# ethz-asl/voxgraph

Hardware: AMD Instinct MI355X
Metric: Mresiduals+Jacobians/s per GPU; full pose-graph solve ms (200 submaps) (higher is better)
Workload: dtype f32

## Files before the change

voxgraph_amd/csrc/vgx_context.hip:

```cpp
#include <algorithm>
#include <atomic>
#include <cmath>
#include <cstring>
#include <numeric>

#include <cstdlib>

#include "vgx_internal.h"

namespace vgx {

static std::mutex g_err_mu;
static std::string g_global_error = "no error";

void set_global_error(const std::string& msg) {
  std::lock_guard<std::mutex> lk(g_err_mu);
  g_global_error = msg;
}

int set_error(vgx_ctx ctx, int code, const std::string& msg) {
  if (ctx) {
    std::lock_guard<std::mutex> lk(ctx->err_mu);
    ctx->last_error = msg;
  } else {
// ... 29 lines not shown
    float v = __builtin_nanf("");
    if (slot >= 0) {
      int vx = ox ? 0 : cx, vy = oy ? 0 : cy, vz = oz ? 0 : cz;
      size_t at = (size_t)slot * VOX + vx + VPS * (vy + VPS * vz);
      bool ok = weight ? (weight[at] > 0.0f) : (observed[at] != 0);
      if (ok) v = distance[at];
    }
    out[cell] = v;
  }
}

int launch_brickify(vgx_submap sm, int which) {
  vgx_ctx ctx = sm->ctx;
  const float* dist = which == 0 ? sm->d_tsdf_distance : sm->d_esdf_distance;
  const float* w = which == 0 ? sm->d_tsdf_weight.get() : nullptr;
  const uint8_t* obs = which == 0 ? nullptr : sm->d_esdf_observed.get();
  const int layout = ctx->brick_layout;
  const size_t cells = brick_cells(sm->vps, layout);
  if ((unsigned long long)sm->n_blocks * cells >= (1ull << 32))
    return set_error(ctx, VGX_ERR_UNSUPPORTED,
                     "submap too large for 32-bit brick addressing: " + std::to_string(sm->n_blocks) + " blocks x " +
                         std::to_string(cells) + " cells per brick");
  size_t bytes = (size_t)sm->n_blocks * cells * sizeof(float);
  VGX_HIP(ctx, sm->grid[which].d_bricks.alloc(bytes));
  sm->grid[which].layout = layout;
  int3 mn = make_int3(sm->lut_min[0], sm->lut_min[1], sm->lut_min[2]);
  int3 dm = make_int3(sm->lut_dim[0], sm->lut_dim[1], sm->lut_dim[2]);
  dispatch_brick(sm->vps, layout, [&](auto V, auto L) {
    hipLaunchKernelGGL((brickify_kernel<V(), L()>), dim3(sm->n_blocks), dim3(256), 0, ctx->stream, sm->d_block_index, sm->d_lut, mn, dm,
                       dist, w, obs, sm->grid[which].d_bricks);
  });
  VGX_HIP(ctx, hipGetLastError());
  sm->grid[which].present = true;
  return VGX_OK;
}

template <int VPS>
__global__ __launch_bounds__(256) void requad_kernel(const float* __restrict__ apron, float* __restrict__ quad) {
  constexpr int CA = BrickLayout<VPS, 0>::cells, CQ = BrickLayout<VPS, 1>::cells, B = VPS + 1;
  const float* in = apron + (size_t)blockIdx.x * CA;
  float* out = quad + (size_t)blockIdx.x * CQ;
  for (int i = threadIdx.x; i < CQ; i += blockDim.x) {
    int cx, cy, cz;
    BrickLayout<VPS, 1>::decode(i, cx, cy, cz);
    out[i] = in[cx + B * (cy + B * cz)];
  }
}

__global__ __launch_bounds__(64) void chunk_bounds_kernel(const float4* __restrict__ xyzd, long long n,
                                                         float4* __restrict__ bounds,
                                                         float* __restrict__ chunk_minmax) {
  const long long first = (long long)blockIdx.x * kChunkPoints;
  float mn[3] = {INFINITY, INFINITY, INFINITY}, mx[3] = {-INFINITY, -INFINITY, -INFINITY};
  for (long long i = first + threadIdx.x; i < first + kChunkPoints && i < n; i += 64) {
    float4 p = xyzd[i];
    mn[0] = fminf(mn[0], p.x); mx[0] = fmaxf(mx[0], p.x);
    mn[1] = fminf(mn[1], p.y); mx[1] = fmaxf(mx[1], p.y);
    mn[2] = fminf(mn[2], p.z); mx[2] = fmaxf(mx[2], p.z);
  }
#pragma unroll
  for (int a = 0; a < 3; ++a)
#pragma unroll
    for (int off = 32; off >= 1; off >>= 1) {
      mn[a] = fminf(mn[a], __shfl_xor(mn[a], off, 64));
      mx[a] = fmaxf(mx[a], __shfl_xor(mx[a], off, 64));
    }
  if (threadIdx.x == 0) {
    float hx = 0.5f * (mx[0] - mn[0]), hy = 0.5f * (mx[1] - mn[1]), hz = 0.5f * (mx[2] - mn[2]);
    float r = sqrtf(hx * hx + hy * hy + hz * hz) * 1.0001f + 1e-4f;
    bounds[blockIdx.x] = make_float4(0.5f * (mx[0] + mn[0]), 0.5f * (mx[1] + mn[1]),
                                     0.5f * (mx[2] + mn[2]), r);
#pragma unroll
    for (int a = 0; a < 3; ++a) {
      chunk_minmax[6 * blockIdx.x + a] = mn[a];
      chunk_minmax[6 * blockIdx.x + 3 + a] = mx[a];
    }
  }
}

int build_chunk_bounds(vgx_ctx ctx, PointSet& ps) {
  ps.d_chunk_bounds.release();
  if (ps.n <= 0) return VGX_OK;
  const long long chunks = (ps.n + kChunkPoints - 1) / kChunkPoints;
  VGX_HIP(ctx, ps.d_chunk_bounds.alloc_n((size_t)chunks));
  DeviceBuffer s_minmax;
  VGX_HIP(ctx, s_minmax.alloc((size_t)chunks * 6 * sizeof(float)));
  float* d_minmax = s_minmax.as<float>();
  hipLaunchKernelGGL(chunk_bounds_kernel, dim3((unsigned)chunks), dim3(64), 0, ctx->stream, ps.d_xyzd,
                     (long long)ps.n, ps.d_chunk_bounds, d_minmax);
  std::vector<float> mm((size_t)chunks * 6);
  hipError_t e = hipGetLastError();
  if (e == hipSuccess) e = hipMemcpyAsync(mm.data(), d_minmax, mm.size() * sizeof(float), hipMemcpyDeviceToHost, ctx->stream);
  if (e == hipSuccess) e = hipStreamSynchronize(ctx->stream);
  if (e != hipSuccess) return set_error(ctx, VGX_ERR_HIP, std::string("chunk bounds: ") + hipGetErrorString(e));
  for (int a = 0; a < 3; ++a) {
    ps.aabb_min[a] = mm[(size_t)a];
    ps.aabb_max[a] = mm[3 + (size_t)a];
  }
  for (long long c = 1; c < chunks; ++c)
    for (int a = 0; a < 3; ++a) {
      ps.aabb_min[a] = std::min(ps.aabb_min[a], mm[(size_t)c * 6 + a]);
      ps.aabb_max[a] = std::max(ps.aabb_max[a], mm[(size_t)c * 6 + 3 + a]);
    }
  return VGX_OK;
}

int build_block_lut(vgx_submap sm) {
  vgx_ctx ctx = sm->ctx;
  const int n_blocks = sm->n_blocks;
  const int32_t* block_index = sm->block_index.data();
  int32_t mn[3] = {0, 0, 0}, mx[3] = {-1, -1, -1};
  for (int b = 0; b < n_blocks; ++b)
    for (int a = 0; a < 3; ++a) {
      int32_t v = block_index[3 * b + a];
      if (b == 0 || v < mn[a]) mn[a] = v;
      if (b == 0 || v > mx[a]) mx[a] = v;
    }
  size_t total = 1;
  for (int a = 0; a < 3; ++a) {
    sm->lut_min[a] = mn[a];
    sm->lut_dim[a] = mx[a] - mn[a] + 1;
    total *= (size_t)sm->lut_dim[a];
    if (total > ((size_t)1 << 28))
      return set_error(ctx, VGX_ERR_UNSUPPORTED,
                       "submap block AABB exceeds 2^28 cells (dense lookup table)");
  }
  if (n_blocks == 0) return VGX_OK;
  std::vector<int32_t> lut(total, -1);
  for (int b = 0; b < n_blocks; ++b) {
    size_t ix = (size_t)(block_index[3 * b + 0] - mn[0]);
    size_t iy = (size_t)(block_index[3 * b + 1] - mn[1]);
    size_t iz = (size_t)(block_index[3 * b + 2] - mn[2]);
    lut[ix + (size_t)sm->lut_dim[0] * (iy + (size_t)sm->lut_dim[1] * iz)] = b;
  }
  VGX_HIP(ctx, sm->d_lut.alloc_n(total));
  VGX_HIP(ctx, hipMemcpy(sm->d_lut, lut.data(), total * sizeof(int32_t), hipMemcpyHostToDevice));
  return VGX_OK;
}

}

namespace vgx {
void reset_point_set(PointSet& ps) {
  static std::atomic<uint64_t> next_version{1};
  ps = PointSet();
  ps.version = next_version.fetch_add(1);
}

int engine_to_host(vgx_ctx ctx, SamplerEngine& e) {
  if (!e.on_device) return VGX_OK;
  VGX_HIP(ctx, hipStreamSynchronize(ctx->stream));
  VGX_HIP(ctx, hipMemcpy(&e.host, e.d_state, sizeof(Mt19937), hipMemcpyDeviceToHost));
  e.on_device = false;
  return VGX_OK;
}

int engine_to_device(vgx_ctx ctx, SamplerEngine& e) {
  if (e.on_device) return VGX_OK;
  if (!e.d_state) VGX_HIP(ctx, e.d_state.alloc(sizeof(Mt19937)));
  VGX_HIP(ctx, hipMemcpyAsync(e.d_state, &e.host, sizeof(Mt19937), hipMemcpyHostToDevice, ctx->stream));
  e.on_device = true;
  return VGX_OK;
}
}

using namespace vgx;

int vgx_submap_s::ensure_quad_grid(int which) {
  Grid& g = grid[which];
  if (!g.present || !g.d_bricks || g.layout != VGX_BRICKS_APRON || g.d_quad) return VGX_OK;
  const size_t cells = brick_cells(vps, VGX_BRICKS_QUAD);
  if ((unsigned long long)n_blocks * cells >= (1ull << 32))
    return set_error(ctx, VGX_ERR_UNSUPPORTED, "submap too large for 32-bit addressing of its quad bricks: " +
                                                   std::to_string(n_blocks) + " blocks");
  static const long fail_after = getenv("VGX_TEST_QUAD_ALLOC_FAILS_AFTER") ? atol(getenv("VGX_TEST_QUAD_ALLOC_FAILS_AFTER")) : -1;
  static long made_so_far = 0;
  const bool pretend_oom = fail_after >= 0 && made_so_far++ >= fail_after;
  if (pretend_oom || g.d_quad.alloc_n((size_t)n_blocks * cells) != hipSuccess) {
    (void)hipGetLastError();
    return set_error(ctx, VGX_ERR_NOMEM, "quad bricks for a sampling session: device allocation failed (" +
                                             std::to_string((size_t)n_blocks * cells * sizeof(float)) + " bytes; "
                                             "vgx_ctx_set_sampling_bricks(ctx, VGX_SAMPLING_BRICKS_SAME) does without)");
  }
  if (vps == 16)
    hipLaunchKernelGGL(requad_kernel<16>, dim3(n_blocks), dim3(256), 0, ctx->stream, g.d_bricks, g.d_quad);
  else
    hipLaunchKernelGGL(requad_kernel<8>, dim3(n_blocks), dim3(256), 0, ctx->stream, g.d_bricks, g.d_quad);
  VGX_HIP(ctx, hipGetLastError());
  return VGX_OK;
}

vgx::GridDev vgx_submap_s::grid_dev(int which) const {
  GridDev g;
  g.bricks = grid[which].d_bricks;
  g.layout = grid[which].layout;
  g.lut = d_lut;
  for (int a = 0; a < 3; ++a) {
    g.lut_min[a] = lut_min[a];
    g.lut_dim[a] = lut_dim[a];
  }
  g.voxel_size = voxel_size;
  g.voxel_size_inv = voxel_size_inv;
  g.block_size = block_size;
  g.block_size_inv = block_size_inv;
  return g;
}

namespace vgx {
std::mutex& lifetime_mu() {
  static std::mutex mu;
  return mu;
}
}

extern "C" {

int vgx_ctx_create(int device, vgx_ctx* out) {
  if (!out) return set_error(nullptr, VGX_ERR_INVALID, "vgx_ctx_create: out == NULL");
  *out = nullptr;
  int count = 0;
  hipError_t e = hipGetDeviceCount(&count);
  if (e != hipSuccess || count <= 0)
    return set_error(nullptr, VGX_ERR_NO_DEVICE,
                     std::string("vgx_ctx_create: no HIP device (") +
                         (e != hipSuccess ? hipGetErrorString(e) : "count == 0") +
                         "); libvoxgraph_amd has no CPU fallback");
  if (device < 0 || device >= count)
    return set_error(nullptr, VGX_ERR_INVALID, "vgx_ctx_create: device index out of range");
  hipDeviceProp_t prop;
  if (hipGetDeviceProperties(&prop, device) != hipSuccess)
    return set_error(nullptr, VGX_ERR_HIP, "vgx_ctx_create: hipGetDeviceProperties failed");
  if (std::string(prop.gcnArchName).rfind("gfx950", 0) != 0)
    return set_error(nullptr, VGX_ERR_NO_DEVICE,
                     std::string("vgx_ctx_create: device is ") + prop.gcnArchName +
                         ", this library is built for gfx950 only");
  vgx_ctx ctx = new (std::nothrow) vgx_ctx_s();
  if (!ctx) return set_error(nullptr, VGX_ERR_NOMEM, "vgx_ctx_create: out of host memory");
  ctx->device = device;
  ctx->cu_count = prop.multiProcessorCount;
  int prio_least = 0, prio_greatest = 0;
  const bool use_prio = hipSetDevice(device) == hipSuccess &&
                        hipDeviceGetStreamPriorityRange(&prio_least, &prio_greatest) == hipSuccess;
  ctx->stream_priorities = use_prio && prio_least != prio_greatest;
  if (hipSetDevice(device) != hipSuccess ||
      hipStreamCreateWithPriority(&ctx->own_stream, hipStreamNonBlocking, ctx->stream_priorities ? prio_least : 0) != hipSuccess ||
      hipStreamCreateWithPriority(&ctx->tsdf_own_stream, hipStreamNonBlocking, ctx->stream_priorities ? prio_greatest : 0) != hipSuccess ||
      hipEventCreate(&ctx->ev_start) != hipSuccess ||
      hipEventCreate(&ctx->ev_stop) != hipSuccess ||
      hipEventCreate(&ctx->ev_tsdf_start) != hipSuccess ||
      hipEventCreate(&ctx->ev_tsdf_stop) != hipSuccess ||
      hipEventCreateWithFlags(&ctx->ev_handover, hipEventDisableTiming) != hipSuccess) {
    if (ctx->own_stream) (void)hipStreamDestroy(ctx->own_stream);
    if (ctx->tsdf_own_stream) (void)hipStreamDestroy(ctx->tsdf_own_stream);
    for (hipEvent_t ev : {ctx->ev_start, ctx->ev_stop, ctx->ev_tsdf_start, ctx->ev_tsdf_stop, ctx->ev_handover})
      if (ev) (void)hipEventDestroy(ev);
    delete ctx;
    return set_error(nullptr, VGX_ERR_HIP, "vgx_ctx_create: stream/event creation failed");
  }
  ctx->stream = ctx->own_stream;
  ctx->tsdf_stream = ctx->tsdf_own_stream;
  ctx->last_error = "no error";
  *out = ctx;
  return VGX_OK;
}

int vgx_ctx_destroy(vgx_ctx ctx) {
  if (!ctx) return VGX_ERR_INVALID;
  (void)hipSetDevice(ctx->device);
  (void)hipStreamSynchronize(ctx->stream);
  (void)hipStreamSynchronize(ctx->tsdf_stream);
  for (hipEvent_t ev : {ctx->ev_start, ctx->ev_stop, ctx->ev_tsdf_start, ctx->ev_tsdf_stop, ctx->ev_handover})
    if (ev) (void)hipEventDestroy(ev);
  for (int k = 0; k < Context::kEvalSlots; ++k) {
    Context::EvalSlot& sl = ctx->eval_slot[k];
    if (sl.stream) {
      (void)hipStreamSynchronize(sl.stream);
      (void)hipStreamDestroy(sl.stream);
    }
    if (sl.order) (void)hipEventDestroy(sl.order);
    sl.d_out.release();
    sl.d_raw.release();
    sl.h_raw.release();
    sl.h_out.release();
  }
  if (ctx->own_stream) (void)hipStreamDestroy(ctx->own_stream);
  if (ctx->tsdf_own_stream) (void)hipStreamDestroy(ctx->tsdf_own_stream);
  delete ctx;
  return VGX_OK;
}

const char* vgx_last_error(vgx_ctx ctx) {
  static thread_local std::string copy;
  if (ctx) {
    std::lock_guard<std::mutex> lk(ctx->err_mu);
    copy = ctx->last_error;
  } else {
    std::lock_guard<std::mutex> lk(g_err_mu);
    copy = g_global_error;
  }
  return copy.c_str();
}

int vgx_ctx_set_stream(vgx_ctx ctx, void* hip_stream) {
  if (!ctx) return VGX_ERR_INVALID;
  std::lock_guard<std::mutex> lk(ctx->mu);
  ctx->stream = hip_stream ? (hipStream_t)hip_stream : ctx->own_stream;
  return VGX_OK;
}

void* vgx_ctx_get_stream(vgx_ctx ctx) { return ctx ? (void*)ctx->stream : nullptr; }

int vgx_ctx_set_tsdf_stream(vgx_ctx ctx, void* hip_stream) {
  if (!ctx) return VGX_ERR_INVALID;
  std::lock_guard<std::mutex> lk(ctx->tsdf_mu);
  (void)hipSetDevice(ctx->device);
  (void)hipStreamSynchronize(ctx->tsdf_stream);
  ctx->tsdf_stream = hip_stream ? (hipStream_t)hip_stream : ctx->tsdf_own_stream;
  return VGX_OK;
}

void* vgx_ctx_get_tsdf_stream(vgx_ctx ctx) { return ctx ? (void*)ctx->tsdf_stream : nullptr; }

int vgx_ctx_set_brick_layout(vgx_ctx ctx, int32_t layout) {
  if (!ctx) return VGX_ERR_INVALID;
  if (layout != VGX_BRICKS_APRON && layout != VGX_BRICKS_QUAD)
    return set_error(ctx, VGX_ERR_INVALID, "vgx_ctx_set_brick_layout: unknown layout");
  std::lock_guard<std::mutex> lk(ctx->mu);
  ctx->brick_layout = layout;
  return VGX_OK;
}

int vgx_ctx_set_sampling_bricks(vgx_ctx ctx, int32_t mode) {
  if (!ctx) return VGX_ERR_INVALID;
  if (mode != VGX_SAMPLING_BRICKS_SAME && mode != VGX_SAMPLING_BRICKS_QUAD)
    return set_error(ctx, VGX_ERR_INVALID, "vgx_ctx_set_sampling_bricks: unknown mode");
  std::lock_guard<std::mutex> lk(ctx->mu);
  ctx->sampling_bricks = mode;
  return VGX_OK;
}

int vgx_ctx_synchronize(vgx_ctx ctx) {
  if (!ctx) return VGX_ERR_INVALID;
  VGX_HIP(ctx, hipStreamSynchronize(ctx->stream));
  VGX_HIP(ctx, hipStreamSynchronize(ctx->tsdf_stream));
  return VGX_OK;
}

int vgx_ctx_synchronize_tsdf(vgx_ctx ctx) {
  if (!ctx) return VGX_ERR_INVALID;
  hipStream_t st;
  {
    std::lock_guard<std::mutex> lk(ctx->tsdf_mu);
    st = ctx->tsdf_stream;
  }
  VGX_HIP(ctx, hipStreamSynchronize(st));
  return VGX_OK;
}

int vgx_ctx_tsdf_wait_for_stream(vgx_ctx ctx, void* producer_stream) {
  if (!ctx) return VGX_ERR_INVALID;
  hipStream_t producer = (hipStream_t)producer_stream;
  if (!producer) {
    std::lock_guard<std::mutex> lk(ctx->mu);
    producer = ctx->stream;
  }
  std::lock_guard<std::mutex> lk(ctx->tsdf_mu);
  VGX_HIP(ctx, hipSetDevice(ctx->device));
  hipEvent_t ev = nullptr;
  VGX_HIP(ctx, hipEventCreateWithFlags(&ev, hipEventDisableTiming));
  hipError_t e = hipEventRecord(ev, producer);
  if (e == hipSuccess) e = hipStreamWaitEvent(ctx->tsdf_stream, ev, 0);
  (void)hipEventDestroy(ev);
  VGX_HIP(ctx, e);
  return VGX_OK;
}

int vgx_ctx_stream_priorities(vgx_ctx ctx) { return ctx && ctx->stream_priorities ? 1 : 0; }

int vgx_ctx_timer_start(vgx_ctx ctx) {
  if (!ctx) return VGX_ERR_INVALID;
  VGX_HIP(ctx, hipEventRecord(ctx->ev_start, ctx->stream));
  {
    std::lock_guard<std::mutex> lk(ctx->tsdf_mu);
    VGX_HIP(ctx, hipEventRecord(ctx->ev_tsdf_start, ctx->tsdf_stream));
  }
  return VGX_OK;
}

int vgx_ctx_timer_stop(vgx_ctx ctx, float* elapsed_ms) {
  if (!ctx || !elapsed_ms) return VGX_ERR_INVALID;
  VGX_HIP(ctx, hipEventRecord(ctx->ev_stop, ctx->stream));
  {
    std::lock_guard<std::mutex> lk(ctx->tsdf_mu);
    VGX_HIP(ctx, hipEventRecord(ctx->ev_tsdf_stop, ctx->tsdf_stream));
  }
  VGX_HIP(ctx, hipEventSynchronize(ctx->ev_stop));
  VGX_HIP(ctx, hipEventSynchronize(ctx->ev_tsdf_stop));
  float a = 0.0f, b = 0.0f;
  VGX_HIP(ctx, hipEventElapsedTime(&a, ctx->ev_start, ctx->ev_stop));
  VGX_HIP(ctx, hipEventElapsedTime(&b, ctx->ev_tsdf_start, ctx->ev_tsdf_stop));
  *elapsed_ms = a > b ? a : b;
  return VGX_OK;
}

static int upload(vgx_ctx ctx, const void* src, size_t bytes, DeviceBuffer& dst) {
  if (!src || bytes == 0) return VGX_OK;
  VGX_HIP(ctx, dst.alloc(bytes));
  VGX_HIP(ctx, hipMemcpyAsync(dst.p, src, bytes, hipMemcpyHostToDevice, ctx->stream));
  return VGX_OK;
}

int vgx_submap_create(vgx_ctx ctx, int32_t submap_id, float voxel_size, int32_t vps,
                      int32_t n_blocks, const int32_t* block_index, const float* tsdf_distance,
                      const float* tsdf_weight, const float* esdf_distance,
                      const uint8_t* esdf_observed, vgx_submap* out) {
  if (!ctx || !out) return VGX_ERR_INVALID;
  *out = nullptr;
  std::lock_guard<std::mutex> lk(ctx->mu);
  if (!(voxel_size > 0) || n_blocks < 0 || (n_blocks > 0 && !block_index))
    return set_error(ctx, VGX_ERR_INVALID, "vgx_submap_create: bad voxel_size / n_blocks / block_index");
  if (vps != 16 && vps != 8)
    return set_error(ctx, VGX_ERR_UNSUPPORTED, "vgx_submap_create: voxels_per_side must be 8 or 16");
  if ((tsdf_distance == nullptr) != (tsdf_weight == nullptr) ||
      (esdf_observed != nullptr && esdf_distance == nullptr))
    return set_error(ctx, VGX_ERR_INVALID,
                     "vgx_submap_create: tsdf_distance/tsdf_weight come together; esdf_observed needs esdf_distance");
  VGX_HIP(ctx, hipSetDevice(ctx->device));
  vgx_submap sm = new (std::nothrow) vgx_submap_s();
  if (!sm) return set_error(ctx, VGX_ERR_NOMEM, "vgx_submap_create: out of host memory");
  sm->ctx = ctx;
  sm->id = submap_id;
  sm->vps = vps;
  sm->n_blocks = n_blocks;
  sm->voxel_size = voxel_size;
  sm->voxel_size_inv = 1.0f / voxel_size;
  sm->block_size = (float)vps * voxel_size;
  sm->block_size_inv = 1.0f / sm->block_size;
  sm->block_index.assign(block_index, block_index + 3 * (size_t)n_blocks);

  int rc = build_block_lut(sm);
  if (rc == VGX_OK && n_blocks > 0) {
    const size_t nvox = (size_t)n_blocks * vps * vps * vps;
    rc = upload(ctx, block_index, 3 * (size_t)n_blocks * sizeof(int32_t), sm->d_block_index);
    if (rc == VGX_OK) rc = upload(ctx, tsdf_distance, nvox * sizeof(float), sm->d_tsdf_distance);
    if (rc == VGX_OK) rc = upload(ctx, tsdf_weight, nvox * sizeof(float), sm->d_tsdf_weight);
    if (rc == VGX_OK) rc = upload(ctx, esdf_distance, nvox * sizeof(float), sm->d_esdf_distance);
    if (rc == VGX_OK) rc = upload(ctx, esdf_observed, nvox * sizeof(uint8_t), sm->d_esdf_observed);
    if (rc == VGX_OK && hipStreamSynchronize(ctx->stream) != hipSuccess)
      rc = set_error(ctx, VGX_ERR_HIP, "vgx_submap_create: H2D upload failed");
    if (rc == VGX_OK && sm->d_tsdf_distance) rc = launch_brickify(sm, 0);
    if (rc == VGX_OK && sm->d_esdf_distance && sm->d_esdf_observed) rc = launch_brickify(sm, 1);
  }
  if (rc != VGX_OK) {
    vgx_submap_destroy(sm);
    return rc;
  }
  *out = sm;
  return VGX_OK;
}


int vgx_submap_release_raw_layers(vgx_submap sm) {
  if (!sm) return VGX_ERR_INVALID;
  (void)hipStreamSynchronize(sm->ctx->stream);
  sm->d_tsdf_distance.release();
  sm->d_tsdf_weight.release();
  sm->d_esdf_distance.release();
  sm->d_esdf_observed.release();
  sm->d_tsdf_rgba.release();
  return VGX_OK;
}

int vgx_submap_set_colors(vgx_submap sm, const uint8_t* rgba) {
  if (!sm) return VGX_ERR_INVALID;
  vgx_ctx ctx = sm->ctx;
  if (!rgba) return set_error(ctx, VGX_ERR_INVALID, "vgx_submap_set_colors: NULL rgba");
  std::lock_guard<std::mutex> lk(ctx->mu);
  if (sm->n_blocks > 0 && (!sm->d_tsdf_distance || !sm->d_tsdf_weight))
    return set_error(ctx, VGX_ERR_INVALID, "vgx_submap_set_colors: raw TSDF layer not resident (released?)");
  VGX_HIP(ctx, hipSetDevice(ctx->device));
  const size_t bytes = std::max<size_t>((size_t)sm->n_blocks * sm->vps * sm->vps * sm->vps * 4, 4);
  DeviceArray<uint32_t> fresh;
  hipError_t e = fresh.alloc(bytes);
  if (e != hipSuccess) return vgx::alloc_error(ctx, e, "vgx_submap_set_colors: allocating colours");
  if (sm->n_blocks > 0) e = hipMemcpyAsync(fresh, rgba, bytes, hipMemcpyHostToDevice, ctx->stream);
  if (e == hipSuccess) e = hipStreamSynchronize(ctx->stream);
  VGX_HIP(ctx, e);
  sm->d_tsdf_rgba.swap(fresh);
  return VGX_OK;
}

int vgx_submap_has_colors(vgx_submap sm, int32_t* has) {
  if (!sm || !has) return VGX_ERR_INVALID;
  std::lock_guard<std::mutex> lk(sm->ctx->mu);
  *has = sm->d_tsdf_rgba ? 1 : 0;
  return VGX_OK;
}

int vgx_submap_download_colors(vgx_submap sm, uint8_t* rgba) {
  if (!sm) return VGX_ERR_INVALID;
  vgx_ctx ctx = sm->ctx;
  if (!rgba) return set_error(ctx, VGX_ERR_INVALID, "vgx_submap_download_colors: NULL rgba");
  std::lock_guard<std::mutex> lk(ctx->mu);
  if (!sm->d_tsdf_rgba) return set_error(ctx, VGX_ERR_INVALID, "vgx_submap_download_colors: the submap has no colours");
  VGX_HIP(ctx, hipSetDevice(ctx->device));
  VGX_HIP(ctx, hipStreamSynchronize(ctx->stream));
  const size_t bytes = (size_t)sm->n_blocks * sm->vps * sm->vps * sm->vps * 4;
  if (bytes) VGX_HIP(ctx, hipMemcpy(rgba, sm->d_tsdf_rgba, bytes, hipMemcpyDeviceToHost));
  return VGX_OK;
}

int vgx_submap_download_layers(vgx_submap sm, float* tsdf_distance, float* tsdf_weight,
                               float* esdf_distance, uint8_t* esdf_observed) {
  if (!sm) return VGX_ERR_INVALID;
  vgx_ctx ctx = sm->ctx;
  VGX_HIP(ctx, hipSetDevice(ctx->device));
  VGX_HIP(ctx, hipStreamSynchronize(ctx->stream));
  const size_t nvox = (size_t)sm->n_blocks * sm->vps * sm->vps * sm->vps;
  struct { void* dst; const void* src; size_t bytes; } jobs[4] = {
      {tsdf_distance, sm->d_tsdf_distance, nvox * sizeof(float)},
      {tsdf_weight, sm->d_tsdf_weight, nvox * sizeof(float)},
      {esdf_distance, sm->d_esdf_distance, nvox * sizeof(float)},
      {esdf_observed, sm->d_esdf_observed, nvox * sizeof(uint8_t)}};
  for (auto& j : jobs) {
    if (!j.dst) continue;
    if (!j.src) return set_error(ctx, VGX_ERR_INVALID, "vgx_submap_download_layers: layer not resident");
    if (j.bytes) VGX_HIP(ctx, hipMemcpy(j.dst, j.src, j.bytes, hipMemcpyDeviceToHost));
  }
  return VGX_OK;
}

int vgx_submap_block_index(vgx_submap sm, int32_t* block_index) {
  if (!sm || !block_index) return VGX_ERR_INVALID;
  std::copy(sm->block_index.begin(), sm->block_index.end(), block_index);
  return VGX_OK;
}

int vgx_submap_destroy(vgx_submap sm) {
  if (!sm) return VGX_ERR_INVALID;
  {
    std::lock_guard<std::mutex> lk(vgx::lifetime_mu());
    if (sm->users > 0) {
      sm->destroy_requested = true;
      return VGX_OK;
    }
  }
  (void)hipSetDevice(sm->ctx->device);
  (void)hipStreamSynchronize(sm->ctx->stream);
  delete sm;
  return VGX_OK;
}

int32_t vgx_submap_id(vgx_submap sm) { return sm ? sm->id : -1; }
int32_t vgx_submap_num_blocks(vgx_submap sm) { return sm ? sm->n_blocks : -1; }

static inline uint64_t spread3(uint64_t v) {
  v &= 0x1fffff;
  v = (v | v << 32) & 0x1f00000000ffffULL;
  v = (v | v << 16) & 0x1f0000ff0000ffULL;
  v = (v | v << 8) & 0x100f00f00f00f00fULL;
  v = (v | v << 4) & 0x10c30c30c30c30c3ULL;
  v = (v | v << 2) & 0x1249249249249249ULL;
  return v;
}

int vgx_submap_set_points(vgx_submap sm, int32_t point_type, int64_t n, const float* xyz,
                          const float* distance, const float* weight, uint32_t flags) {
  if (!sm) return VGX_ERR_INVALID;
  vgx_ctx ctx = sm->ctx;
  std::lock_guard<std::mutex> lk(ctx->mu);
  if (point_type != VGX_POINTS_ISOSURFACE && point_type != VGX_POINTS_VOXELS)
    return set_error(ctx, VGX_ERR_INVALID, "vgx_submap_set_points: bad point_type");
  if (n < 0 || n > INT32_MAX || (n > 0 && (!xyz || !distance || !weight)))
    return set_error(ctx, VGX_ERR_INVALID, "vgx_submap_set_points: bad n or NULL arrays");
  VGX_HIP(ctx, hipSetDevice(ctx->device));
  PointSet& ps = sm->points[point_type];
  (void)hipStreamSynchronize(ctx->stream);
  reset_point_set(ps);
  ps.n = n;
  ps.cumulative_weight.resize((size_t)n);
  double acc = 0;
  for (int64_t i = 0; i < n; ++i) {
    acc = (i == 0) ? (double)weight[i] : acc + (double)weight[i];
    ps.cumulative_weight[(size_t)i] = acc;
  }
  std::vector<int64_t> order;
  if ((flags & VGX_POINTS_SORT_MORTON) && n > 1) {
    std::vector<uint64_t> key((size_t)n);
    float mnv[3] = {xyz[0], xyz[1], xyz[2]};
    for (int64_t i = 0; i < n; ++i)
      for (int a = 0; a < 3; ++a) mnv[a] = std::min(mnv[a], xyz[3 * i + a]);
    float base[3];
    for (int a = 0; a < 3; ++a) base[a] = std::floor(mnv[a] * sm->block_size_inv) * sm->block_size;
    for (int64_t i = 0; i < n; ++i) {
      uint64_t c[3];
      for (int a = 0; a < 3; ++a) {
        double v = std::floor(((double)xyz[3 * i + a] - (double)base[a]) * (double)sm->voxel_size_inv);
        c[a] = (uint64_t)std::min(std::max(v, 0.0), 2097151.0);
      }
      key[(size_t)i] = spread3(c[0]) | (spread3(c[1]) << 1) | (spread3(c[2]) << 2);
    }
    order.resize((size_t)n);
    std::iota(order.begin(), order.end(), (int64_t)0);
    std::stable_sort(order.begin(), order.end(),
                     [&](int64_t a, int64_t b) { return key[(size_t)a] < key[(size_t)b]; });
  }
  std::vector<float4> h_xyzd((size_t)n);
  std::vector<float> h_w((size_t)n);
  double sum_w = 0;
  for (int64_t i = 0; i < n; ++i) {
    int64_t s = order.empty() ? i : order[(size_t)i];
    h_xyzd[(size_t)i] = make_float4(xyz[3 * s], xyz[3 * s + 1], xyz[3 * s + 2], distance[s]);
    h_w[(size_t)i] = weight[s];
    sum_w += (double)weight[s];
  }
  ps.sum_weight = sum_w;
  ps.order = order;
  if (!order.empty()) {
    ps.inv_order.resize((size_t)n);
    for (int64_t i = 0; i < n; ++i) ps.inv_order[(size_t)order[(size_t)i]] = (int32_t)i;
  }
  if (n > 0) {
    VGX_HIP(ctx, ps.d_xyzd.alloc_n((size_t)n));
    VGX_HIP(ctx, ps.d_weight.alloc_n((size_t)n));
    VGX_HIP(ctx, hipMemcpy(ps.d_xyzd, h_xyzd.data(), (size_t)n * sizeof(float4), hipMemcpyHostToDevice));
    VGX_HIP(ctx, hipMemcpy(ps.d_weight, h_w.data(), (size_t)n * sizeof(float), hipMemcpyHostToDevice));
  }
  const int rc = build_chunk_bounds(ctx, ps);
  ps.present = rc == VGX_OK;
  return rc;
}

int64_t vgx_submap_num_points(vgx_submap sm, int32_t point_type) {
  if (!sm || point_type < 0 || point_type > 1 || !sm->points[point_type].present) return -1;
  return sm->points[point_type].n;
}

int vgx_submap_point_order(vgx_submap sm, int32_t point_type, int64_t* order) {
  if (!sm || point_type < 0 || point_type > 1 || !order) return VGX_ERR_INVALID;
  const PointSet& ps = sm->points[point_type];
  if (!ps.present) return set_error(sm->ctx, VGX_ERR_INVALID, "vgx_submap_point_order: no such point set");
  for (int64_t i = 0; i < ps.n; ++i) order[i] = ps.order.empty() ? i : ps.order[(size_t)i];
  return VGX_OK;
}

int vgx_submap_download_points(vgx_submap sm, int32_t point_type, float* xyz, float* distance,
                               float* weight) {
  if (!sm || point_type < 0 || point_type > 1) return VGX_ERR_INVALID;
  vgx_ctx ctx = sm->ctx;
  const PointSet& ps = sm->points[point_type];
  if (!ps.present) return set_error(ctx, VGX_ERR_INVALID, "vgx_submap_download_points: no such point set");
  if (ps.n == 0) return VGX_OK;
  VGX_HIP(ctx, hipSetDevice(ctx->device));
  VGX_HIP(ctx, hipStreamSynchronize(ctx->stream));
  std::vector<float4> h((size_t)ps.n);
  VGX_HIP(ctx, hipMemcpy(h.data(), ps.d_xyzd, (size_t)ps.n * sizeof(float4), hipMemcpyDeviceToHost));
  for (int64_t i = 0; i < ps.n; ++i) {
    if (xyz) {
      xyz[3 * i] = h[(size_t)i].x;
      xyz[3 * i + 1] = h[(size_t)i].y;
      xyz[3 * i + 2] = h[(size_t)i].z;
    }
    if (distance) distance[i] = h[(size_t)i].w;
  }
  if (weight) VGX_HIP(ctx, hipMemcpy(weight, ps.d_weight, (size_t)ps.n * sizeof(float), hipMemcpyDeviceToHost));
  return VGX_OK;
}

}

extern "C" {
int vgx_internal_set_error(vgx_ctx ctx, int code, const char* msg) { return vgx::set_error(ctx, code, msg ? msg : ""); }
int vgx_internal_launch_brickify(vgx_submap sm, int which) { return vgx::launch_brickify(sm, which); }
int vgx_internal_build_block_lut(vgx_submap sm) { return vgx::build_block_lut(sm); }
}
```

voxgraph_amd/csrc/vgx_extract.hip:

```cpp
#include <vector>

#include "vgx_internal.h"

#pragma clang fp contract(off)

namespace vgx {

__device__ __forceinline__ bool keep_voxel(float td, float tw, double min_w, double max_d) {
  return (double)tw > min_w && (double)fabsf(td) < max_d;
}

template <int VPS>
__global__ __launch_bounds__(256) void extract_count_kernel(const float* __restrict__ tsdf_d,
                                                            const float* __restrict__ tsdf_w,
                                                            double min_w, double max_d,
                                                            int32_t* __restrict__ counts,
                                                            double* __restrict__ wsum) {
  constexpr int VOX = VPS * VPS * VPS;
  const size_t base = (size_t)blockIdx.x * VOX;
  int cnt = 0;
  double sw = 0.0;
  for (int v = threadIdx.x; v < VOX; v += 256) {
    float td = tsdf_d[base + v], tw = tsdf_w[base + v];
    if (keep_voxel(td, tw, min_w, max_d)) {
      ++cnt;
      sw += (double)tw;
    }
  }
#pragma unroll
  for (int off = 32; off >= 1; off >>= 1) {
    cnt += __shfl_xor(cnt, off, 64);
    sw += __shfl_xor(sw, off, 64);
  }
  __shared__ int s_cnt[4];
  __shared__ double s_sw[4];
  if ((threadIdx.x & 63) == 0) {
    s_cnt[threadIdx.x >> 6] = cnt;
    s_sw[threadIdx.x >> 6] = sw;
  }
  __syncthreads();
  if (threadIdx.x == 0) {
    counts[blockIdx.x] = (s_cnt[0] + s_cnt[1]) + (s_cnt[2] + s_cnt[3]);
    wsum[blockIdx.x] = (s_sw[0] + s_sw[1]) + (s_sw[2] + s_sw[3]);
  }
}

template <int VPS>
__global__ __launch_bounds__(256) void extract_write_kernel(
    const int32_t* __restrict__ block_index, const float* __restrict__ tsdf_d,
    const float* __restrict__ tsdf_w, const float* __restrict__ esdf_d, double min_w,
    double max_d, float voxel_size, float block_size, const int64_t* __restrict__ offsets,
    float4* __restrict__ xyzd, float* __restrict__ weight) {
  constexpr int VOX = VPS * VPS * VPS;
  const int b = blockIdx.x;
  const size_t base = (size_t)b * VOX;
  const float ox = (float)block_index[3 * b + 0] * block_size;
  const float oy = (float)block_index[3 * b + 1] * block_size;
  const float oz = (float)block_index[3 * b + 2] * block_size;
  __shared__ int s_wave[4];
  int64_t running = offsets[b];
  const int lane = threadIdx.x & 63, wave = threadIdx.x >> 6;
  for (int round = 0; round < VOX; round += 256) {
    int v = round + (int)threadIdx.x;
    float td = 0.0f, tw = 0.0f;
    bool keep = false;
    if (v < VOX) {
      td = tsdf_d[base + v];
      tw = tsdf_w[base + v];
      keep = keep_voxel(td, tw, min_w, max_d);
    }
    unsigned long long mask = __ballot(keep);
    int before = __popcll(mask & ((1ull << lane) - 1ull));
    if (lane == 0) s_wave[wave] = __popcll(mask);
    __syncthreads();
    int wave_off = 0, total = 0;
#pragma unroll
    for (int w = 0; w < 4; ++w) {
      if (w < wave) wave_off += s_wave[w];
      total += s_wave[w];
    }
    if (keep) {
      int64_t at = running + wave_off + before;
      int ix = v % VPS, iy = (v / VPS) % VPS, iz = v / (VPS * VPS);
      float x = voxel_centre(ox, ix, voxel_size);
      float y = voxel_centre(oy, iy, voxel_size);
      float z = voxel_centre(oz, iz, voxel_size);
      float d = esdf_d ? esdf_d[base + v] : td;
      xyzd[at] = make_float4(x, y, z, d);
      weight[at] = tw;
    }
    running += total;
    __syncthreads();
  }
}

}

using namespace vgx;

extern "C" int vgx_submap_extract_voxel_points(vgx_submap sm, double min_voxel_weight,
                                               double max_voxel_distance,
                                               int32_t use_esdf_distance, int64_t* n_points_out) {
  if (!sm) return VGX_ERR_INVALID;
  vgx_ctx ctx = sm->ctx;
  std::lock_guard<std::mutex> lk(ctx->mu);
  if (sm->n_blocks > 0 && (!sm->d_tsdf_distance || !sm->d_tsdf_weight))
    return set_error(ctx, VGX_ERR_INVALID, "vgx_submap_extract_voxel_points: TSDF layer not resident");
  if (sm->n_blocks > 0 && use_esdf_distance && !sm->d_esdf_distance)
    return set_error(ctx, VGX_ERR_INVALID, "vgx_submap_extract_voxel_points: ESDF layer not resident");
  VGX_HIP(ctx, hipSetDevice(ctx->device));
  PointSet& ps = sm->points[VGX_POINTS_VOXELS];
  VGX_HIP(ctx, hipStreamSynchronize(ctx->stream));
  reset_point_set(ps);
  const int nb = sm->n_blocks;
  if (nb == 0) {
    ps.present = true;
    if (n_points_out) *n_points_out = 0;
    return VGX_OK;
  }
  DeviceBuffer s_counts, s_wsum, s_offsets;
  VGX_HIP(ctx, s_counts.alloc((size_t)nb * sizeof(int32_t)));
  VGX_HIP(ctx, s_wsum.alloc((size_t)nb * sizeof(double)));
  VGX_HIP(ctx, s_offsets.alloc(((size_t)nb + 1) * sizeof(int64_t)));
  int32_t* d_counts = s_counts.as<int32_t>();
  double* d_wsum = s_wsum.as<double>();
  int64_t* d_offsets = s_offsets.as<int64_t>();
  if (sm->vps == 16)
    hipLaunchKernelGGL(extract_count_kernel<16>, dim3(nb), dim3(256), 0, ctx->stream,
                       sm->d_tsdf_distance, sm->d_tsdf_weight, min_voxel_weight,
                       max_voxel_distance, d_counts, d_wsum);
  else
    hipLaunchKernelGGL(extract_count_kernel<8>, dim3(nb), dim3(256), 0, ctx->stream,
                       sm->d_tsdf_distance, sm->d_tsdf_weight, min_voxel_weight,
                       max_voxel_distance, d_counts, d_wsum);
  std::vector<int32_t> counts((size_t)nb);
  std::vector<double> wsum((size_t)nb);
  std::vector<int64_t> offsets((size_t)nb + 1, 0);
  hipError_t e = hipMemcpyAsync(counts.data(), d_counts, (size_t)nb * sizeof(int32_t), hipMemcpyDeviceToHost, ctx->stream);
  if (e == hipSuccess) e = hipMemcpyAsync(wsum.data(), d_wsum, (size_t)nb * sizeof(double), hipMemcpyDeviceToHost, ctx->stream);
  if (e == hipSuccess) e = hipStreamSynchronize(ctx->stream);
  int rc = VGX_OK;
  if (e != hipSuccess) rc = set_error(ctx, VGX_ERR_HIP, std::string("extract: ") + hipGetErrorString(e));
  double sum_w = 0;
  if (rc == VGX_OK) {
    for (int b = 0; b < nb; ++b) {
      offsets[(size_t)b + 1] = offsets[(size_t)b] + counts[(size_t)b];
      sum_w += wsum[(size_t)b];
    }
    const int64_t n = offsets[(size_t)nb];
    if (n > INT32_MAX) rc = set_error(ctx, VGX_ERR_UNSUPPORTED, "extract: more than 2^31 points");
    ps.n = n;
    ps.sum_weight = sum_w;
    if (rc == VGX_OK && n > 0) {
      if (ps.d_xyzd.alloc_n((size_t)n) != hipSuccess || ps.d_weight.alloc_n((size_t)n) != hipSuccess)
        rc = set_error(ctx, VGX_ERR_NOMEM, "extract: device allocation failed");
    }
    if (rc == VGX_OK && n > 0) {
      e = hipMemcpyAsync(d_offsets, offsets.data(), ((size_t)nb + 1) * sizeof(int64_t), hipMemcpyHostToDevice, ctx->stream);
      if (e == hipSuccess) {
        const float* esdf = use_esdf_distance ? sm->d_esdf_distance.get() : nullptr;
        if (sm->vps == 16)
          hipLaunchKernelGGL(extract_write_kernel<16>, dim3(nb), dim3(256), 0, ctx->stream,
                             sm->d_block_index, sm->d_tsdf_distance, sm->d_tsdf_weight, esdf,
                             min_voxel_weight, max_voxel_distance, sm->voxel_size, sm->block_size,
                             d_offsets, ps.d_xyzd, ps.d_weight);
        else
          hipLaunchKernelGGL(extract_write_kernel<8>, dim3(nb), dim3(256), 0, ctx->stream,
                             sm->d_block_index, sm->d_tsdf_distance, sm->d_tsdf_weight, esdf,
                             min_voxel_weight, max_voxel_distance, sm->voxel_size, sm->block_size,
                             d_offsets, ps.d_xyzd, ps.d_weight);
        e = hipGetLastError();
      }
      if (e == hipSuccess) e = hipStreamSynchronize(ctx->stream);
      if (e != hipSuccess) rc = set_error(ctx, VGX_ERR_HIP, std::string("extract: ") + hipGetErrorString(e));
    }
  }
  if (rc == VGX_OK) rc = build_chunk_bounds(ctx, ps);
  if (rc == VGX_OK && n_points_out) *n_points_out = ps.n;
  if (rc == VGX_OK) ps.present = true; else reset_point_set(ps);
  return rc;
}
```

voxgraph_amd/csrc/vgx_internal.h:

```cpp
#ifndef VGX_INTERNAL_H_
#define VGX_INTERNAL_H_

#include <hip/hip_runtime.h>

#include <algorithm>
#include <atomic>
#include <cstdint>
#include <mutex>
#include <condition_variable>
#include <initializer_list>
#include <random>
#include <string>
#include <type_traits>
#include <utility>
#include <vector>

#include "voxgraph_amd.h"

namespace vgx {


template <int VPS, int LAYOUT>
struct BrickLayout {
  static_assert(LAYOUT == 0 || LAYOUT == 1, "apron (0) or quad (1) bricks");
  static constexpr int B = VPS + 1;
  static constexpr int cells = LAYOUT == 0 ? B * B * B : B * VPS * VPS * 4;
  __host__ __device__ static int anchor(int vx, int vy, int vz) {
    if (LAYOUT == 0) return vx + B * (vy + B * vz);
    return 4 * (vx + B * (vy + VPS * vz));
  }
  __host__ __device__ static void decode(int i, int& cx, int& cy, int& cz) {
    if (LAYOUT == 0) {
      cx = i % B; cy = (i / B) % B; cz = i / (B * B);
      return;
    }
    const int comp = i & 3, e = i >> 2;
    cx = e % B; cy = (e / B) % VPS + (comp & 1); cz = e / (B * VPS) + (comp >> 1);
  }
};
template <class F>
inline auto dispatch_brick(int vps, int layout, F&& f) {
  using std::integral_constant;
  if (vps == 16) {
    if (layout == VGX_BRICKS_QUAD) return f(integral_constant<int, 16>{}, integral_constant<int, 1>{});
    return f(integral_constant<int, 16>{}, integral_constant<int, 0>{});
  }
  if (layout == VGX_BRICKS_QUAD) return f(integral_constant<int, 8>{}, integral_constant<int, 1>{});
  return f(integral_constant<int, 8>{}, integral_constant<int, 0>{});
}
inline size_t brick_cells(int vps, int layout) {
  return dispatch_brick(vps, layout, [](auto V, auto L) { return (size_t)BrickLayout<V(), L()>::cells; });
}

struct GridDev {
  const float* bricks;
  const int32_t* lut;
  int32_t lut_min[3];
  int32_t lut_dim[3];
  float voxel_size, voxel_size_inv, block_size, block_size_inv;
  int32_t layout;
};

struct alignas(16) PosePack {
  float qw, qz;
  float tx, ty, tz;
  float cos_e, sin_e;
  float cos_emo, sin_emo;
  float dxs, dxc;
  float dys, dyc;
  float k1, k2;
  float pad;
};
static_assert(sizeof(PosePack) == 64, "PosePack must stay one 64-byte line");

struct alignas(16) ConstraintDev {
  GridDev grid;
  const float4* xyzd;
  const float* weight;
  const uint32_t* sample_raw;
  const double* cumulative;
  const int32_t* search_lut;
  int32_t search_buckets;
  const float4* sample_pts;
  const int32_t* inv_order;
  int64_t n_points;
  const float4* chunk_bounds;
  int64_t n;
  int64_t row0;
  int64_t prow0;
  int32_t tile_points;
  double factor;
  double no_corr_cost;
};

struct Tile {
  int32_t constraint;
  int32_t count;
  int64_t start;
};

constexpr int kMinSearchBuckets = 4096;
constexpr int kMaxSearchBuckets = 1 << 24;
constexpr int kChunkPoints = 512;
constexpr int kNormalSize = 45;
constexpr int kPartialSize = 22;

struct DeviceBuffer {
  void* p = nullptr;
  size_t bytes = 0;
  DeviceBuffer() = default;
  DeviceBuffer(const DeviceBuffer&) = delete;
  DeviceBuffer& operator=(const DeviceBuffer&) = delete;
  DeviceBuffer(DeviceBuffer&& o) noexcept { swap(o); }
  DeviceBuffer& operator=(DeviceBuffer&& o) noexcept {
    swap(o);
    return *this;
  }
  ~DeviceBuffer() { release(); }
  void swap(DeviceBuffer& o) {
    std::swap(p, o.p);
    std::swap(bytes, o.bytes);
  }
  void release() {
    if (p) (void)hipFree(p);
    p = nullptr;
    bytes = 0;
  }
  hipError_t alloc(size_t n) {
    release();
    const hipError_t e = hipMalloc(&p, n);
    if (e == hipSuccess) bytes = n;
    else p = nullptr;
    return e;
  }
  hipError_t reserve(size_t n, size_t min_bytes = 0, bool slack = false) {
    if (n <= bytes) return hipSuccess;
    return alloc(std::max(slack ? n + n / 4 : n, min_bytes));
  }
  void* detach() {
    void* q = p;
    p = nullptr;
    bytes = 0;
    return q;
  }
  template <typename T>
  T* as() const {
    return static_cast<T*>(p);
  }
};
template <class T>
struct DeviceArray : DeviceBuffer {
  T* get() const { return static_cast<T*>(p); }
  operator T*() const { return get(); }
  hipError_t alloc_n(size_t count) { return alloc(count * sizeof(T)); }
};
struct PinnedBuffer {
  void* p = nullptr;
  size_t bytes = 0;
  PinnedBuffer() = default;
  PinnedBuffer(const PinnedBuffer&) = delete;
  PinnedBuffer& operator=(const PinnedBuffer&) = delete;
  PinnedBuffer(PinnedBuffer&& o) noexcept { swap(o); }
  PinnedBuffer& operator=(PinnedBuffer&& o) noexcept {
    swap(o);
    return *this;
  }
  ~PinnedBuffer() { release(); }
  void swap(PinnedBuffer& o) {
    std::swap(p, o.p);
    std::swap(bytes, o.bytes);
  }
  void release() {
    if (p) (void)hipHostFree(p);
    p = nullptr;
    bytes = 0;
  }
  hipError_t alloc(size_t n, unsigned flags = hipHostMallocDefault) {
    release();
    const hipError_t e = hipHostMalloc(&p, n, flags);
    if (e == hipSuccess) bytes = n;
    else p = nullptr;
    return e;
  }
  hipError_t reserve(size_t n) { return n <= bytes ? hipSuccess : alloc(n); }
  template <typename T>
  T* as() const {
    return static_cast<T*>(p);
  }
};
struct UploadStage {
  PinnedBuffer half[2];
  hipEvent_t copied[2] = {nullptr, nullptr};
  int turn = 0;
  UploadStage() = default;
  UploadStage(const UploadStage&) = delete;
  UploadStage& operator=(const UploadStage&) = delete;
  ~UploadStage() {
    for (hipEvent_t e : copied)
      if (e) (void)hipEventDestroy(e);
  }
  size_t bytes() const { return half[0].bytes; }
  hipError_t reserve(size_t n) {
    hipError_t e = hipSuccess;
    for (int k = 0; k < 2 && e == hipSuccess; ++k)
      if (!copied[k]) e = hipEventCreateWithFlags(&copied[k], hipEventDisableTiming);
    if (e == hipSuccess && n > bytes()) {
      half[0].release();
      half[1].release();
      e = half[0].alloc(n);
      if (e == hipSuccess) e = half[1].alloc(n);
    }
    if (e != hipSuccess) {
      half[0].release();
      half[1].release();
    }
    return e;
  }
  void* next(int* k, hipError_t* err = nullptr) {
    *k = turn;
    turn ^= 1;
    const hipError_t e = hipEventSynchronize(copied[*k]);
    if (err) *err = e;
    return e == hipSuccess ? half[*k].p : nullptr;
  }
  hipError_t record(int k, hipStream_t stream) { return hipEventRecord(copied[k], stream); }
};
struct DeviceBufferSize {
  DeviceBuffer* buffer;
  size_t bytes;
};
inline hipError_t alloc_group(std::initializer_list<DeviceBufferSize> group) {
  for (const DeviceBufferSize& g : group) g.buffer->release();
  hipError_t e = hipSuccess;
  for (const DeviceBufferSize& g : group)
    if (e == hipSuccess) e = g.buffer->alloc(g.bytes);
  if (e != hipSuccess)
    for (const DeviceBufferSize& g : group) g.buffer->release();
  return e;
}

template <class Call>
hipError_t temp_bytes(Call& call, size_t* bytes) {
  *bytes = 0;
  return call(nullptr, *bytes);
}
template <class Call>
hipError_t run_with_temp(DeviceBuffer& tmp, Call& call) {
  size_t bytes = 0;
  hipError_t e = temp_bytes(call, &bytes);
  if (e == hipSuccess) e = tmp.reserve(bytes, 8);
  if (e == hipSuccess) e = call(tmp.p, bytes);
  return e;
}

struct Context {
  int device = 0;
  hipStream_t own_stream = nullptr;
  hipStream_t stream = nullptr;
  hipEvent_t ev_start = nullptr, ev_stop = nullptr;
  std::mutex mu;
  hipStream_t tsdf_own_stream = nullptr;
  hipStream_t tsdf_stream = nullptr;
  bool stream_priorities = false;
  std::atomic<int> tsdf_integrators{0};
  hipEvent_t ev_tsdf_start = nullptr, ev_tsdf_stop = nullptr, ev_handover = nullptr;
  std::mutex tsdf_mu;
  std::mutex err_mu;
  std::string last_error;
  int cu_count = 256;
  int brick_layout = 0;
  int sampling_bricks = 1;
  struct EvalSlot {
    hipStream_t stream = nullptr;
    hipEvent_t order = nullptr;
    DeviceBuffer d_out;
    DeviceBuffer d_raw;
    PinnedBuffer h_raw;
    PinnedBuffer h_out;
    bool busy = false;
  };
  static constexpr int kEvalSlots = 8;
  static constexpr size_t kSmallOutputBytes = 1u << 20;
  EvalSlot eval_slot[kEvalSlots];
  std::condition_variable slot_free;
};

struct Mt19937 {
  static constexpr int kN = 624;
  uint32_t mt[kN];
  uint32_t idx = kN;
  Mt19937() { seed(5489u); }
  void seed(uint32_t s) {
    mt[0] = s;
    for (int i = 1; i < kN; ++i) mt[i] = 1812433253u * (mt[i - 1] ^ (mt[i - 1] >> 30)) + (uint32_t)i;
    idx = kN;
  }
  void twist() {
    for (int k = 0; k < kN; ++k) {
      uint32_t y = (mt[k] & 0x80000000u) | (mt[(k + 1) % kN] & 0x7fffffffu);
      mt[k] = mt[(k + 397) % kN] ^ (y >> 1) ^ ((y & 1u) ? 0x9908b0dfu : 0u);
    }
    idx = 0;
  }
  uint32_t operator()() {
    if (idx >= (uint32_t)kN) twist();
    uint32_t y = mt[idx++];
    y ^= y >> 11;
    y ^= (y << 7) & 0x9d2c5680u;
    y ^= (y << 15) & 0xefc60000u;
    y ^= y >> 18;
    return y;
  }
};
static_assert(sizeof(Mt19937) == 625 * 4, "Mt19937 is copied to the device as 625 words");

struct SamplerEngine {
  Mt19937 host;
  DeviceArray<uint32_t> d_state;
  bool on_device = false;
};

struct PointSet {
  int64_t n = 0;
  uint64_t version = 0;
  DeviceArray<float4> d_xyzd;
  DeviceArray<float> d_weight;
  DeviceArray<float4> d_chunk_bounds;
  float aabb_min[3] = {0, 0, 0}, aabb_max[3] = {0, 0, 0};
  double sum_weight = 0;
  bool present = false;
  std::vector<int64_t> order;
  std::vector<int32_t> inv_order;
  std::vector<double> cumulative_weight;
  DeviceArray<double> d_cumulative;
  int32_t search_buckets = 0;
  DeviceArray<int32_t> d_search_lut;
  DeviceArray<int32_t> d_inv_order;
  SamplerEngine rng;
};

struct Grid {
  DeviceArray<float> d_bricks;
  bool present = false;
  int layout = 0;
  DeviceArray<float> d_quad;
};

}

struct vgx_ctx_s : vgx::Context {};

struct vgx_submap_s {
  vgx_ctx ctx = nullptr;
  int32_t id = 0;
  float voxel_size = 0, voxel_size_inv = 0, block_size = 0, block_size_inv = 0;
  int32_t vps = 0;
  int32_t n_blocks = 0;
  std::vector<int32_t> block_index;
  vgx::DeviceArray<int32_t> d_block_index;
  vgx::DeviceArray<int32_t> d_lut;
  int32_t lut_min[3] = {0, 0, 0};
  int32_t lut_dim[3] = {0, 0, 0};
  vgx::DeviceArray<float> d_tsdf_distance;
  vgx::DeviceArray<float> d_tsdf_weight;
  vgx::DeviceArray<uint32_t> d_tsdf_rgba;
  vgx::DeviceArray<float> d_esdf_distance;
  vgx::DeviceArray<uint8_t> d_esdf_observed;
  vgx::Grid grid[2];
  vgx::PointSet points[2];
  std::vector<int32_t> isosurface_blocks;
  vgx::DeviceArray<int32_t> d_iso_block_index;
  vgx::DeviceArray<uint8_t> d_block_has_data;
  vgx::GridDev grid_dev(int which) const;
  int ensure_quad_grid(int which);
  int users = 0;
  bool destroy_requested = false;
};

struct vgx_reg_s {
  vgx_ctx ctx = nullptr;
  vgx_submap reference = nullptr;
  vgx_submap reading = nullptr;
  vgx_reg_config cfg{};
  int64_t num_residuals = 0;
  uint64_t points_version = 0;
  vgx::SamplerEngine rng;
  vgx::DeviceBuffer d_sample_raw;
  vgx::PinnedBuffer h_sample_raw;
  std::mutex mu;
  int draw_raw(uint32_t* out);
  vgx::SamplerEngine& engine();
  bool sampling() const { return cfg.sampling_ratio != -1.0f; }
  bool points_current() const;
  vgx::ConstraintDev describe() const;
  int users = 0;
  bool destroy_requested = false;
};

struct vgx_reg_batch_s {
  vgx_ctx ctx = nullptr;
  int32_t n = 0;
  int32_t n_global = 0;
  int layout = 0;
  std::vector<vgx_reg> regs;
  std::vector<int32_t> node_pair;
  std::vector<int32_t> global_index;
  std::vector<int64_t> row_offset;
  std::vector<vgx::Tile> tiles;
  vgx::DeviceBuffer d_desc;
  vgx::DeviceBuffer d_pack;
  vgx::UploadStage pack_stage;
  vgx::DeviceBuffer d_tiles;
  vgx::DeviceBuffer d_draw_tiles;
  int32_t n_draw_tiles = 0;
  vgx::DeviceBuffer d_drawn;
  vgx::DeviceBuffer d_drawn_idx;
  vgx::DeviceBuffer d_tile_dead;
  vgx::DeviceBuffer d_tile_first;
  vgx::DeviceBuffer d_partials;
  vgx::DeviceBuffer d_normal;
  vgx::PinnedBuffer h_normal;
  vgx::DeviceBuffer d_node_pair;
  vgx::DeviceBuffer d_global_index;
  std::vector<vgx::Tile> reduce_tiles;
  std::vector<vgx::ConstraintDev> host_desc;
  std::vector<int32_t> host_tile_first;
  bool launch_order_made = false;
  bool launch_order_grouped = false, points_order_grouped = false;
  bool points_order_made = false;
  std::vector<int32_t> host_points_tile_first;
  vgx::DeviceBuffer d_reduce_tiles;
  int32_t csr_nodes = 0;
  vgx::DeviceBuffer d_node_first;
  vgx::DeviceBuffer d_node_items;
  struct StreamJob {
    vgx::SamplerEngine* engine;
    int64_t offset;
    int64_t count;
  };
  std::vector<StreamJob> stream_jobs;
  vgx::DeviceBuffer d_raw;
  vgx::DeviceBuffer d_stream_jobs;
  bool any_sampling = false;
  bool holds_regs = false;
  vgx::DeviceBuffer d_rows[3];
  vgx::PinnedBuffer h_rows;
  bool rows_have[3] = {false, false, false};
  bool rows_mirrored = false;
  int users = 0;
  bool destroy_requested = false;
};

namespace vgx {
#ifndef VGX_TOOLING_LIBRARY
int set_error(vgx_ctx ctx, int code, const std::string& msg);
#else
inline int set_error(vgx_ctx ctx, int code, const std::string& msg);
#endif

std::mutex& lifetime_mu();

void set_global_error(const std::string& msg);

__host__ __device__ __forceinline__ float voxel_centre(float origin, int idx, float voxel_size) {
  return origin + ((float)idx + 0.5f) * voxel_size;
}

#define VGX_HIP(ctx, call)                                                      \
  do {                                                                          \
    hipError_t e__ = (call);                                                    \
    if (e__ != hipSuccess)                                                      \
      return vgx::set_error((ctx), VGX_ERR_HIP,                                 \
                            std::string(#call) + ": " + hipGetErrorString(e__)); \
  } while (0)

inline int alloc_error(vgx_ctx ctx, hipError_t e, const char* what) {
  (void)hipGetLastError();
  return set_error(ctx, e == hipErrorOutOfMemory ? VGX_ERR_NOMEM : VGX_ERR_HIP, std::string(what) + ": " + hipGetErrorString(e));
}

inline int upload_new(vgx_ctx ctx, DeviceBuffer& buffer, const void* src, size_t bytes) {
  buffer.release();
  if (bytes == 0) return VGX_OK;
  VGX_HIP(ctx, buffer.alloc(bytes));
  VGX_HIP(ctx, hipMemcpy(buffer.p, src, bytes, hipMemcpyHostToDevice));
  return VGX_OK;
}

struct MeshView {
  vgx_ctx ctx;
  bool holds_mesh;
  bool has_colors;
  bool per_vertex;
  int64_t n_tris;
  const float* vertices;
  const float* normals;
  const uint32_t* colors;
};
std::mutex& mesh_mutex(vgx_mesh M);
MeshView mesh_view(vgx_mesh M);

struct EvalTotals {
  double sum;
  float max_abs, min_abs;
  long long n_eval, n_ign, n_non, n_err_blocks;
};
struct EvalDevice {
  DeviceBuffer slot, has, pos, part, tot, tmp, ed, es, ebi;
};
int eval_check(const char* fn, vgx_submap gt, vgx_submap test, int32_t layer, int32_t mode, const void* details);
int eval_enqueue(vgx_submap gt, vgx_submap test, int32_t layer, int32_t mode, bool want_index, bool want_distance, bool want_set,
                 EvalDevice& D);
void eval_details(const EvalTotals& tot, vgx_voxel_evaluation_details* details);

#ifndef VGX_TOOLING_LIBRARY
int launch_brickify(vgx_submap sm, int which);
int build_block_lut(vgx_submap sm);
#else
inline int launch_brickify(vgx_submap sm, int which);
inline int build_block_lut(vgx_submap sm);
#endif
int build_chunk_bounds(vgx_ctx ctx, PointSet& ps);
void reset_point_set(PointSet& ps);
int engine_to_host(vgx_ctx ctx, SamplerEngine& e);
int engine_to_device(vgx_ctx ctx, SamplerEngine& e);
void make_pose_pack(const double ref_pose[4], const double read_pose[4], PosePack* out);
std::vector<Tile> make_tiles(int32_t constraint, int64_t n, int tile_points);
constexpr int kBlockThreads = 256;
constexpr int kPointsPerThread = 4;
constexpr int kTilePoints = kBlockThreads * kPointsPerThread;
}

extern "C" {
VGX_API int vgx_internal_set_error(vgx_ctx ctx, int code, const char* msg);
VGX_API int vgx_internal_launch_brickify(vgx_submap sm, int which);
VGX_API int vgx_internal_build_block_lut(vgx_submap sm);
}
#ifdef VGX_TOOLING_LIBRARY
namespace vgx {
inline int set_error(vgx_ctx ctx, int code, const std::string& msg) { return vgx_internal_set_error(ctx, code, msg.c_str()); }
inline int launch_brickify(vgx_submap sm, int which) { return vgx_internal_launch_brickify(sm, which); }
inline int build_block_lut(vgx_submap sm) { return vgx_internal_build_block_lut(sm); }
}
#endif

#endif
```

voxgraph_amd/csrc/vgx_iso.hip:

```cpp
#include <cmath>
#include <vector>

#include "vgx_internal.h"
#include "vgx_interp.h"

#pragma clang fp contract(off)

namespace vgx {

constexpr unsigned long long kEmptyKey = ~0ull;

struct IsoParams {
  const int32_t* block_index;
  const int32_t* lut;
  int3 lut_min, lut_dim;
  const float* tsdf_d;
  const float* tsdf_w;
  float voxel_size, voxel_size_inv, block_size, block_size_inv;
  float min_weight;
  double threshold_inv;
  unsigned long long* keys;
  unsigned long long* ids;
  unsigned long long mask;
};
// ... 124 lines not shown
    const int e = round_ + (int)threadIdx.x;
    float vert[3] = {0, 0, 0};
    bool cand = e < EDGES && iso_candidate<VPS>(p, tile, b, e, vert);
    bool keep = cand;
    float dist = 0.0f, wgt = 0.0f;
    if (MODE >= 1 && cand) {
      const unsigned long long key = iso_cell_key(p, vert);
      const unsigned long long id = (unsigned long long)b * EDGES + (unsigned long long)e;
      unsigned long long h = hash64(key) & p.mask;
      if (MODE == 1) {
        while (true) {
          unsigned long long prev = atomicCAS(&p.keys[h], kEmptyKey, key);
          if (prev == kEmptyKey || prev == key) {
            atomicMin(&p.ids[h], id);
            break;
          }
          h = (h + 1) & p.mask;
        }
      } else {
        while (p.keys[h] != key) h = (h + 1) & p.mask;
        keep = p.ids[h] == id && tsdf_interp<VPS>(p, vert, dist, wgt);
      }
    }
    if (MODE == 0 || MODE == 2) my_count += keep ? 1 : 0;
    if (MODE == 3) {
      unsigned long long m = __ballot(keep);
      int before = __popcll(m & ((1ull << lane) - 1ull));
      if (lane == 0) s_wave[wave] = __popcll(m);
      __syncthreads();
      int wave_off = 0, total = 0;
#pragma unroll
      for (int w = 0; w < 4; ++w) {
        if (w < wave) wave_off += s_wave[w];
        total += s_wave[w];
      }
      if (keep) {
        int64_t at = running + wave_off + before;
        xyzd[at] = make_float4(vert[0], vert[1], vert[2], dist);
        weight[at] = wgt;
        int rx = (int)floorf(vert[0] * p.block_size_inv + 1e-6f) - p.lut_min.x;
        int ry = (int)floorf(vert[1] * p.block_size_inv + 1e-6f) - p.lut_min.y;
        int rz = (int)floorf(vert[2] * p.block_size_inv + 1e-6f) - p.lut_min.z;
        if ((unsigned)rx < (unsigned)p.lut_dim.x && (unsigned)ry < (unsigned)p.lut_dim.y &&
            (unsigned)rz < (unsigned)p.lut_dim.z) {
          int slot = p.lut[rx + p.lut_dim.x * (ry + p.lut_dim.y * rz)];
          if (slot >= 0) block_has_vertex[slot] = 1;
        }
      }
      running += total;
      __syncthreads();
    }
  }
  if (MODE == 0 || MODE == 2) {
#pragma unroll
    for (int off = 32; off >= 1; off >>= 1) my_count += __shfl_xor(my_count, off, 64);
    if (lane == 0) s_wave[wave] = my_count;
    __syncthreads();
    if (threadIdx.x == 0) counts[b] = (s_wave[0] + s_wave[1]) + (s_wave[2] + s_wave[3]);
  }
}

template <int MODE>
static void launch_iso(vgx_submap sm, const IsoParams& p, int32_t* counts, const int64_t* offsets,
                       float4* xyzd, float* weight, unsigned char* has, const int32_t* block_list = nullptr, int n_list = 0) {
  hipStream_t st = sm->ctx->stream;
  const int grid = block_list ? n_list : sm->n_blocks;
  if (grid <= 0) return;
  if (sm->vps == 16)
    hipLaunchKernelGGL((iso_pass_kernel<16, MODE>), dim3(grid), dim3(256), 0, st, p, counts,
                       offsets, xyzd, weight, has, block_list);
  else
    hipLaunchKernelGGL((iso_pass_kernel<8, MODE>), dim3(grid), dim3(256), 0, st, p, counts,
                       offsets, xyzd, weight, has, block_list);
}

static int extract_isosurface(vgx_submap sm, IsoParams p, PointSet& ps) {
  static const std::string kFn = "vgx_submap_extract_isosurface_points: ";
  vgx_ctx ctx = sm->ctx;
  hipStream_t st = ctx->stream;
  const int nb = sm->n_blocks;
  DeviceBuffer d_counts, d_offsets, d_has, d_keys, d_ids, d_active;
  if (d_counts.alloc((size_t)nb * 4) != hipSuccess || d_offsets.alloc(((size_t)nb + 1) * 8) != hipSuccess ||
      d_has.alloc((size_t)nb) != hipSuccess)
    return set_error(ctx, VGX_ERR_NOMEM, kFn + "device allocation failed");
  std::vector<int32_t> counts((size_t)nb);
  auto fetch_counts = [&]() {
    hipError_t e = hipGetLastError();
    if (e == hipSuccess) e = hipMemcpyAsync(counts.data(), d_counts.p, (size_t)nb * 4, hipMemcpyDeviceToHost, st);
    if (e == hipSuccess) e = hipStreamSynchronize(st);
    return e;
  };
  launch_iso<0>(sm, p, d_counts.as<int32_t>(), nullptr, nullptr, nullptr, nullptr);
  VGX_HIP(ctx, fetch_counts());
  int64_t candidates = 0;
  std::vector<int32_t> active;
  for (int b = 0; b < nb; ++b) {
    candidates += counts[(size_t)b];
    if (counts[(size_t)b] > 0) active.push_back(b);
  }
  if (candidates == 0) return VGX_OK;
  unsigned long long cap = 1024;
  while (cap < 2ull * (unsigned long long)candidates) cap <<= 1;
  p.mask = cap - 1;
  if (d_keys.alloc(cap * 8) != hipSuccess || d_ids.alloc(cap * 8) != hipSuccess)
    return set_error(ctx, VGX_ERR_NOMEM, kFn + "dedup table allocation failed");
  p.keys = d_keys.as<unsigned long long>();
  p.ids = d_ids.as<unsigned long long>();
  VGX_HIP(ctx, hipMemsetAsync(p.keys, 0xff, cap * 8, st));
  VGX_HIP(ctx, hipMemsetAsync(p.ids, 0xff, cap * 8, st));
  VGX_HIP(ctx, hipMemsetAsync(d_has.p, 0, (size_t)nb, st));
  VGX_HIP(ctx, hipMemsetAsync(d_counts.p, 0, (size_t)nb * 4, st));
  VGX_HIP(ctx, d_active.alloc(active.size() * 4));
  VGX_HIP(ctx, hipMemcpyAsync(d_active.p, active.data(), active.size() * 4, hipMemcpyHostToDevice, st));
  launch_iso<1>(sm, p, d_counts.as<int32_t>(), nullptr, nullptr, nullptr, nullptr, d_active.as<int32_t>(), (int)active.size());
  launch_iso<2>(sm, p, d_counts.as<int32_t>(), nullptr, nullptr, nullptr, nullptr, d_active.as<int32_t>(), (int)active.size());
  VGX_HIP(ctx, fetch_counts());
  std::vector<int64_t> offsets((size_t)nb + 1, 0);
  for (int b = 0; b < nb; ++b) offsets[(size_t)b + 1] = offsets[(size_t)b] + counts[(size_t)b];
  const int64_t n = offsets[(size_t)nb];
  ps.n = n;
  if (n == 0) return VGX_OK;
  if (ps.d_xyzd.alloc_n((size_t)n) != hipSuccess || ps.d_weight.alloc_n((size_t)n) != hipSuccess)
    return set_error(ctx, VGX_ERR_NOMEM, kFn + "point allocation failed");
  VGX_HIP(ctx, hipMemcpyAsync(d_offsets.p, offsets.data(), ((size_t)nb + 1) * 8, hipMemcpyHostToDevice, st));
  launch_iso<3>(sm, p, d_counts.as<int32_t>(), d_offsets.as<int64_t>(), ps.d_xyzd, ps.d_weight, d_has.as<unsigned char>(),
                d_active.as<int32_t>(), (int)active.size());
  VGX_HIP(ctx, hipGetLastError());
  std::vector<float> w((size_t)n);
  std::vector<unsigned char> has((size_t)nb);
  VGX_HIP(ctx, hipMemcpyAsync(w.data(), ps.d_weight, (size_t)n * 4, hipMemcpyDeviceToHost, st));
  VGX_HIP(ctx, hipMemcpyAsync(has.data(), d_has.p, (size_t)nb, hipMemcpyDeviceToHost, st));
  VGX_HIP(ctx, hipStreamSynchronize(st));
  double sw = 0;
  for (int64_t i = 0; i < n; ++i) sw += (double)w[(size_t)i];
  ps.sum_weight = sw;
  for (int b = 0; b < nb; ++b)
    if (has[(size_t)b]) sm->isosurface_blocks.push_back(b);
  return VGX_OK;
}

}

using namespace vgx;

extern "C" int vgx_submap_extract_isosurface_points(vgx_submap sm, double min_voxel_weight,
                                                    int64_t* n_points_out) {
  if (!sm) return VGX_ERR_INVALID;
  vgx_ctx ctx = sm->ctx;
  std::lock_guard<std::mutex> lk(ctx->mu);
  if (sm->n_blocks > 0 && (!sm->d_tsdf_distance || !sm->d_tsdf_weight))
    return set_error(ctx, VGX_ERR_INVALID, "vgx_submap_extract_isosurface_points: TSDF layer not resident");
  VGX_HIP(ctx, hipSetDevice(ctx->device));
  VGX_HIP(ctx, hipStreamSynchronize(ctx->stream));
  PointSet& ps = sm->points[VGX_POINTS_ISOSURFACE];
  reset_point_set(ps);
  sm->isosurface_blocks.clear();
  sm->d_iso_block_index.release();
  if (n_points_out) *n_points_out = 0;
  if (sm->n_blocks == 0) {
    ps.present = true;
    return VGX_OK;
  }

  IsoParams p{};
  p.block_index = sm->d_block_index;
  p.lut = sm->d_lut;
  p.lut_min = make_int3(sm->lut_min[0], sm->lut_min[1], sm->lut_min[2]);
  p.lut_dim = make_int3(sm->lut_dim[0], sm->lut_dim[1], sm->lut_dim[2]);
  p.tsdf_d = sm->d_tsdf_distance;
  p.tsdf_w = sm->d_tsdf_weight;
  p.voxel_size = sm->voxel_size;
  p.voxel_size_inv = sm->voxel_size_inv;
  p.block_size = sm->block_size;
  p.block_size_inv = sm->block_size_inv;
  p.min_weight = (float)min_voxel_weight;
  const float threshold = (float)(0.5 * (double)sm->voxel_size);
  p.threshold_inv = 1.0 / (double)threshold;

  int rc = extract_isosurface(sm, p, ps);
  if (rc == VGX_OK) rc = build_chunk_bounds(ctx, ps);
  if (rc == VGX_OK && !sm->isosurface_blocks.empty()) {
    std::vector<int32_t> ib(3 * sm->isosurface_blocks.size());
    for (size_t k = 0; k < sm->isosurface_blocks.size(); ++k)
      for (int a = 0; a < 3; ++a) ib[3 * k + a] = sm->block_index[3 * (size_t)sm->isosurface_blocks[k] + a];
    if (sm->d_iso_block_index.alloc_n(ib.size()) != hipSuccess ||
        hipMemcpy(sm->d_iso_block_index, ib.data(), ib.size() * 4, hipMemcpyHostToDevice) != hipSuccess)
      rc = set_error(ctx, VGX_ERR_NOMEM, "vgx_submap_extract_isosurface_points: block list upload failed");
  }
  if (rc == VGX_OK && n_points_out) *n_points_out = ps.n;
  if (rc == VGX_OK) ps.present = true; else reset_point_set(ps);
  return rc;
}
```

voxgraph_amd/csrc/vgx_reg.hip:

```cpp
#include <algorithm>
#include <cmath>
#include <cstdio>
#include <cstdlib>
#include <cstring>
#include <numeric>

#include "vgx_internal.h"

#pragma clang fp contract(off)

namespace vgx {

namespace {
struct YawQuat {
  float w, z;
};

YawQuat yaw_exp(float psi) {
  float nrm = std::sqrt(0.0f * 0.0f + 0.0f * 0.0f + psi * psi);
  double theta = (double)nrm;
  double na = theta < std::pow(2.220446049250313e-16, 0.25)
                  ? 0.5 + (theta * theta) * (1.0 / 48.0)
                  : std::sin(theta * 0.5) / theta;
  double ct = std::cos(theta * 0.5);
// ... 709 lines not shown
  const bool count_misses = C.no_corr_cost != 0.0;
  const bool sampled = C.sample_raw != nullptr;
  const float4* bounds = (!count_misses && !sampled && C.chunk_bounds) ? C.chunk_bounds : nullptr;
  const long long chunk0 = tile.start / kChunkPoints;
  const int n_chunks = (tile.count + kChunkPoints - 1) / kChunkPoints;
  const int wlane = (int)(threadIdx.x & 63);
  const unsigned long long live =
      __ballot(wlane < n_chunks && !(bounds && chunk_outside(g, P, bounds[chunk0 + wlane])));
  auto chunk_live = [&](int k) { return ((live >> k) & 1ull) != 0ull; };
  constexpr int kAcc = COST_ONLY ? 1 : 21;
  float acc[kAcc];
#pragma unroll
  for (int k = 0; k < kAcc; ++k) acc[k] = 0.0f;
  const float nc = (float)C.no_corr_cost;
  const bool grid_empty = g.bricks == nullptr;

  f32x4 pt_next[PPT];
  float w_next[PPT];
  bool live_next = chunk_live(0);
  if (live_next) {
#pragma unroll
    for (int j = 0; j < PPT; ++j) {
      int local = j * kBlockThreads + (int)threadIdx.x;
      int64_t i = tile.start + (local < tile.count ? local : 0);
      if (sampled) {
        pt_next[j] = as_global(reinterpret_cast<const f32x4*>(C.sample_pts))[C.row0 + i];
        w_next[j] = 1.0f;
      } else {
        pt_next[j] = as_global(reinterpret_cast<const f32x4*>(C.xyzd))[i];
        w_next[j] = as_global(C.weight)[i];
      }
    }
  }
  for (int base = 0; base < tile.count; base += kIterPoints) {
    f32x4 pt[PPT];
    float w[PPT];
    const bool live = live_next;
#pragma unroll
    for (int j = 0; j < PPT; ++j) {
      pt[j] = pt_next[j];
      w[j] = w_next[j];
    }
    live_next = false;
    if (base + kIterPoints < tile.count) {
      live_next = chunk_live((base + kIterPoints) / kChunkPoints);
      if (live_next) {
#pragma unroll
        for (int j = 0; j < PPT; ++j) {
          int local = base + kIterPoints + j * kBlockThreads + (int)threadIdx.x;
          int64_t i = tile.start + (local < tile.count ? local : 0);
          if (sampled) {
            pt_next[j] = as_global(reinterpret_cast<const f32x4*>(C.sample_pts))[C.row0 + i];
            w_next[j] = 1.0f;
          } else {
            pt_next[j] = as_global(reinterpret_cast<const f32x4*>(C.xyzd))[i];
            w_next[j] = as_global(C.weight)[i];
          }
        }
      }
    }
    if (!live) continue;
    Located loc[PPT];
    bool have[PPT];
    float d[PPT][8];
#pragma unroll
    for (int j = 0; j < PPT; ++j) {
      loc[j] = locate_stage1<VPS, LAYOUT>(g, P, pt[j].x, pt[j].y, pt[j].z);
      have[j] = false;
    }
    if (!grid_empty) {
      int slot[PPT];
#pragma unroll
      for (int j = 0; j < PPT; ++j) slot[j] = as_global(g.lut)[loc[j].lut_index];
      constexpr int CELLS = BrickLayout<VPS, LAYOUT>::cells;
      bool any = false;
#pragma unroll
      for (int j = 0; j < PPT; ++j) {
        have[j] = loc[j].inside && slot[j] >= 0;
        any |= have[j];
      }
      if (kBallotSkip && !count_misses && __builtin_amdgcn_ballot_w64(any) == 0ull) continue;
#pragma unroll
      for (int j = 0; j < PPT; ++j) {
        const unsigned off = (unsigned)(have[j] ? slot[j] : 0) * (unsigned)CELLS + (unsigned)loc[j].cell_off;
        load_neighbours<VPS, LAYOUT>(g.bricks + off, d[j]);
      }
    } else {
#pragma unroll
      for (int j = 0; j < PPT; ++j)
#pragma unroll
        for (int k = 0; k < 8; ++k) d[j][k] = 0.0f;
    }
#pragma unroll
    for (int j = 0; j < PPT; ++j) {
      const int local = base + j * kBlockThreads + (int)threadIdx.x;
      float u[6];
      const bool in_range = local < tile.count;
      float c_[8];
      const float value = interpolated_value(d[j], loc[j].Dx, loc[j].Dy, loc[j].Dz, c_[0], c_[1], c_[2], c_[3], c_[4],
                                             c_[5], c_[6], c_[7]);
      const bool ok = eval_point_lean(c_, have[j] && in_range, loc[j].Dx, loc[j].Dy, loc[j].Dz, value, g.voxel_size_inv, P,
                                      pt[j].x, pt[j].y, pt[j].w, w[j], u);
      u[5] = ok ? u[5] : ((count_misses && in_range) ? w[j] * nc : 0.0f);
      if (COST_ONLY) accumulate_square(acc[0], u[5]);
      else accumulate21(acc, u);
    }
  }
  const size_t row = ((size_t)tile_first[tile.constraint] + (size_t)(tile.start / C.tile_points)) * (kBlockThreads / 64) +
                     (threadIdx.x >> 6);
  if (COST_ONLY) {
    double v = (double)acc[0];
#pragma unroll
    for (int off = 32; off >= 1; off >>= 1) v += __shfl_xor(v, off, 64);
    if ((threadIdx.x & 63) == 0) partials[row * kPartialSize + 20] = v;
    return;
  }
  const int lane = threadIdx.x & 63;
  {
    const bool b5 = (lane & 32) != 0, b4 = (lane & 16) != 0, b3 = (lane & 8) != 0, b2 = (lane & 4) != 0, b1 = (lane & 2) != 0;
    double r16[16];
#pragma unroll
    for (int i = 0; i < 16; ++i) {
      const double lo = (double)acc[i], up = 16 + i < 21 ? (double)acc[16 + i < 21 ? 16 + i : 0] : 0.0;
      const double keep = b5 ? up : lo, send = b5 ? lo : up;
      r16[i] = keep + __shfl_xor(send, 32, 64);
    }
    double r8[8];
#pragma unroll
    for (int i = 0; i < 8; ++i) {
      const double keep = b4 ? r16[8 + i] : r16[i], send = b4 ? r16[i] : r16[8 + i];
      r8[i] = keep + __shfl_xor(send, 16, 64);
    }
    double r4[4];
#pragma unroll
    for (int i = 0; i < 4; ++i) {
      const double keep = b3 ? r8[4 + i] : r8[i], send = b3 ? r8[i] : r8[4 + i];
      r4[i] = keep + __shfl_xor(send, 8, 64);
    }
    double r2[2];
#pragma unroll
    for (int i = 0; i < 2; ++i) {
      const double keep = b2 ? r4[2 + i] : r4[i], send = b2 ? r4[i] : r4[2 + i];
      r2[i] = keep + __shfl_xor(send, 4, 64);
    }
    const double keep = b1 ? r2[1] : r2[0], send = b1 ? r2[0] : r2[1];
    double v = keep + __shfl_xor(send, 2, 64);
    v += __shfl_xor(v, 1, 64);
    const int s = lane >> 1;
    if ((lane & 1) == 0 && s < 21) partials[row * kPartialSize + s] = v;
  }
}

struct StreamJobDev {
  uint32_t* state;
  uint32_t* out;
  long long count;
};

__device__ __forceinline__ uint32_t mt_twist_word(uint32_t cur, uint32_t next, uint32_t far) {
  const uint32_t y = (cur & 0x80000000u) | (next & 0x7fffffffu);
  return far ^ (y >> 1) ^ ((y & 1u) ? 0x9908b0dfu : 0u);
}

constexpr int kMtThreads = 227;
__device__ __forceinline__ void lds_barrier() {
  __builtin_amdgcn_fence(__ATOMIC_RELEASE, "workgroup", "local");
  __builtin_amdgcn_s_barrier();
  __builtin_amdgcn_fence(__ATOMIC_ACQUIRE, "workgroup", "local");
}
__device__ __forceinline__ uint32_t mt_temper(uint32_t y) {
  y ^= y >> 11;
  y ^= (y << 7) & 0x9d2c5680u;
  y ^= (y << 15) & 0xefc60000u;
  y ^= y >> 18;
  return y;
}

__global__ __launch_bounds__(kMtThreads) void mt_generate_kernel(const StreamJobDev* __restrict__ jobs) {
  constexpr int N = Mt19937::kN, M = 397, H = N - M;
  constexpr int kLastOwner = N - 1 - 2 * H;
  constexpr int kStride = 3 * H + 3;
  static_assert(kMtThreads == H, "one thread per word of a range");
  const StreamJobDev job = jobs[blockIdx.x];
  VGX_GLOBAL uint32_t* const g_out = (VGX_GLOBAL uint32_t*)job.out;
  VGX_GLOBAL uint32_t* const g_state = (VGX_GLOBAL uint32_t*)job.state;
  __shared__ uint32_t buf[2][kStride];
  const int t = threadIdx.x;
  for (int k = t; k < N; k += kMtThreads) buf[0][k] = g_state[k];
  for (int k = N + t; k < kStride; k += kMtThreads) buf[0][k] = buf[1][k] = 0u;
  int idx = (int)g_state[N];
  int cur = 0;
  __syncthreads();
  const bool third = t <= kLastOwner;
  uint32_t a = buf[0][t], b = buf[0][H + t], c = buf[0][2 * H + t];
  auto twist = [&]() {
    const uint32_t* o = buf[cur];
    uint32_t* w = buf[cur ^ 1];
    const uint32_t a1 = o[t + 1], b1 = o[H + t + 1], far = o[t + M], c1 = o[2 * H + t + 1];
    const uint32_t new0 = mt_twist_word(o[0], o[1], o[M]);
    a = mt_twist_word(a, a1, far);
    b = mt_twist_word(b, b1, a);
    c = mt_twist_word(c, t == kLastOwner ? new0 : c1, b);
    w[t] = a;
    w[H + t] = b;
    w[2 * H + t] = c;
    lds_barrier();
    cur ^= 1;
  };
  auto store_part = [&](long long produced, int take) {
    const int pa = t - idx, pb = H + t - idx, pc = 2 * H + t - idx;
    if (pa >= 0 && pa < take) g_out[produced + pa] = mt_temper(a);
    if (pb >= 0 && pb < take) g_out[produced + pb] = mt_temper(b);
    if (third && pc >= 0 && pc < take) g_out[produced + pc] = mt_temper(c);
  };
  long long produced = 0;
  if (idx < N && produced < job.count) {
    const long long left = job.count - produced;
    const int take = (int)(left < (long long)(N - idx) ? left : (long long)(N - idx));
    store_part(produced, take);
    idx += take;
    produced += take;
  }
  {
    VGX_GLOBAL uint32_t* p = g_out + produced + t;
    const long long blocks = (job.count - produced) / N;
    for (long long k = 0; k < blocks; ++k) {
      twist();
      p[0] = mt_temper(a);
      p[H] = mt_temper(b);
      if (third) p[2 * H] = mt_temper(c);
      p += N;
    }
    if (blocks > 0) idx = N;
    produced += blocks * N;
  }
  if (produced < job.count) {
    twist();
    idx = 0;
    const int take = (int)(job.count - produced);
    store_part(produced, take);
    idx += take;
    produced += take;
  }
  __syncthreads();
  for (int k = t; k < N; k += kMtThreads) g_state[k] = buf[cur][k];
  if (t == 0) g_state[N] = (uint32_t)idx;
}

__global__ __launch_bounds__(64) void reg_tile_live_kernel(const ConstraintDev* __restrict__ cons,
                                                          const PosePack* __restrict__ packs,
                                                          const Tile* __restrict__ tiles, int n_tiles,
                                                          int32_t* __restrict__ live) {
  const int t = blockIdx.x;
  if (t >= n_tiles) return;
  const Tile tile = tiles[t];
  const ConstraintDev& C = cons[tile.constraint];
  const PosePack P = packs[tile.constraint];
  const bool cull = C.no_corr_cost == 0.0 && C.chunk_bounds && C.sample_raw == nullptr;
  const long long chunk0 = tile.start / kChunkPoints;
  const int n_chunks = (tile.count + kChunkPoints - 1) / kChunkPoints;
  int mine = 0;
  for (int k = threadIdx.x; k < n_chunks; k += 64) {
    const int pts = (k + 1) * kChunkPoints <= tile.count ? kChunkPoints : tile.count - k * kChunkPoints;
    if (!cull || !chunk_outside(C.grid, P, C.chunk_bounds[chunk0 + k])) mine += pts;
  }
#pragma unroll
  for (int off = 32; off >= 1; off >>= 1) mine += __shfl_xor(mine, off, 64);
  if (threadIdx.x == 0) live[t] = mine;
}

__global__ void reg_count_live_kernel(const ConstraintDev* __restrict__ cons, const PosePack* __restrict__ packs,
                                      int n_cons, unsigned long long* __restrict__ live ) {
  const int c = blockIdx.x;
  if (c >= n_cons) return;
  const ConstraintDev& C = cons[c];
  const PosePack P = packs[c];
  const long long n_chunks = (C.n + kChunkPoints - 1) / kChunkPoints;
  unsigned long long mine = 0;
  const bool cull = C.no_corr_cost == 0.0 && C.chunk_bounds && C.sample_raw == nullptr;
  for (long long k = threadIdx.x; k < n_chunks; k += blockDim.x) {
    const long long pts = (k + 1) * kChunkPoints <= C.n ? kChunkPoints : C.n - k * kChunkPoints;
    if (!cull || !chunk_outside(C.grid, P, C.chunk_bounds[k])) mine += (unsigned long long)pts;
  }
#pragma unroll
  for (int off = 32; off >= 1; off >>= 1) mine += __shfl_xor(mine, off, 64);
  if ((threadIdx.x & 63) == 0 && mine) atomicAdd(live + c, mine);
}

static std::vector<Tile> deal_to_xcds(const std::vector<std::vector<Tile>>& group_tiles,
                                      const std::vector<int64_t>& group_work, size_t n_tiles) {
  constexpr int kXcds = 8;
  std::vector<size_t> order(group_tiles.size());
  for (size_t g = 0; g < order.size(); ++g) order[g] = g;
  std::stable_sort(order.begin(), order.end(), [&](size_t a, size_t b) { return group_work[a] > group_work[b]; });
  std::vector<std::vector<Tile>> stream(kXcds);
  std::vector<int64_t> load(kXcds, 0);
  for (size_t g : order) {
    int best = 0;
    for (int x = 1; x < kXcds; ++x)
      if (load[(size_t)x] < load[(size_t)best]) best = x;
    stream[(size_t)best].insert(stream[(size_t)best].end(), group_tiles[g].begin(), group_tiles[g].end());
    load[(size_t)best] += group_work[g];
  }
  std::vector<size_t> next(kXcds, 0);
  std::vector<Tile> out;
  out.reserve(n_tiles);
  while (out.size() < n_tiles)
    for (int x = 0; x < kXcds && out.size() < n_tiles; ++x) {
      int src = x;
      if (next[(size_t)src] >= stream[(size_t)src].size()) {
        size_t left = 0;
        for (int y = 0; y < kXcds; ++y) {
          const size_t l = stream[(size_t)y].size() - next[(size_t)y];
          if (l > left) {
            left = l;
            src = y;
          }
        }
      }
      out.push_back(stream[(size_t)src][next[(size_t)src]++]);
    }
  return out;
}

static std::vector<Tile> make_draw_order(const std::vector<ConstraintDev>& desc,
                                         const std::vector<int32_t>& tile_first, const std::vector<Tile>& tiles) {
  std::vector<const void*> key;
  std::vector<std::vector<Tile>> group_tiles;
  std::vector<int64_t> group_work;
  size_t n = 0;
  for (size_t c = 0; c < desc.size(); ++c) {
    if (!desc[c].sample_raw) continue;
    size_t g = 0;
    while (g < key.size() && key[g] != (const void*)desc[c].cumulative) ++g;
    if (g == key.size()) {
      key.push_back((const void*)desc[c].cumulative);
      group_tiles.emplace_back();
      group_work.push_back(0);
    }
    for (int32_t t = tile_first[c]; t < tile_first[c + 1]; ++t) {
      group_tiles[g].push_back(tiles[(size_t)t]);
      group_work[g] += tiles[(size_t)t].count;
      ++n;
    }
  }
  return deal_to_xcds(group_tiles, group_work, n);
}

static bool make_xcd_order(const std::vector<ConstraintDev>& desc, const std::vector<int32_t>& tile_first,
                           const std::vector<int32_t>& tile_work, std::vector<Tile>& tiles, bool points_pass) {
  if (points_pass) {
    const char* e = getenv("VGX_POINTS_TILE_ORDER");
    if (e && atoi(e) == 0) return false;
  }
  const int n = (int)desc.size();
  if (n < 2 || tiles.size() < 16) return false;
  std::vector<std::vector<int>> groups;
  {
    std::vector<std::pair<const void*, int>> key;
    for (int c = 0; c < n; ++c) {
      int g = -1;
      if (!desc[(size_t)c].sample_raw)
        for (auto& k : key)
          if (k.first == (const void*)desc[(size_t)c].xyzd) g = k.second;
      if (g < 0) {
        g = (int)groups.size();
        groups.emplace_back();
        if (!desc[(size_t)c].sample_raw) key.emplace_back((const void*)desc[(size_t)c].xyzd, g);
      }
      groups[(size_t)g].push_back(c);
    }
  }
  std::vector<std::vector<Tile>> group_tiles(groups.size());
  std::vector<int64_t> group_work(groups.size(), 0);
  for (size_t g = 0; g < groups.size(); ++g) {
    int most = 0;
    for (int c : groups[g]) most = std::max(most, tile_first[(size_t)c + 1] - tile_first[(size_t)c]);
    for (int r = 0; r < most; ++r)
      for (int c : groups[g])
        if (r < tile_first[(size_t)c + 1] - tile_first[(size_t)c]) {
          const size_t t = (size_t)tile_first[(size_t)c] + (size_t)r;
          group_tiles[g].push_back(tiles[t]);
          group_work[g] += points_pass ? (int64_t)tiles[t].count * 36 + (int64_t)tile_work[t] * 52
                                       : (int64_t)tile_work[t] + 256;
        }
  }
  constexpr double kOrderShareMin = 0.3;
  constexpr double kOrderLiveMin = 0.75;
  {
    int64_t total = 0, shareable = 0;
    for (size_t g = 0; g < groups.size(); ++g) {
      int most = 0;
      for (int c : groups[g]) most = std::max(most, tile_first[(size_t)c + 1] - tile_first[(size_t)c]);
      for (int r = 0; r < most; ++r) {
        int64_t sum = 0, mx = 0;
        for (int c : groups[g])
          if (r < tile_first[(size_t)c + 1] - tile_first[(size_t)c]) {
            const int64_t w = tile_work[(size_t)tile_first[(size_t)c] + (size_t)r];
            sum += w;
// ... 135 lines not shown
    double v = 0.0;
    for (int c = threadIdx.x; c < n; c += 256) v += normal[(size_t)c * kNormalSize];
    part[threadIdx.x] = v;
    __syncthreads();
    for (int off = 128; off >= 1; off >>= 1) {
      if ((int)threadIdx.x < off) part[threadIdx.x] += part[threadIdx.x + off];
      __syncthreads();
    }
    if (threadIdx.x == 0) fused[0] = accumulate ? fused[0] + part[0] : part[0];
    return;
  }
  int64_t tid = (int64_t)blockIdx.x * blockDim.x + threadIdx.x;
  if (tid < n_node_elems) {
    int node = (int)(tid / 20), e = (int)(tid % 20);
    double v = 0.0;
    for (int it = node_first[node]; it < node_first[node + 1]; ++it) {
      int item = node_items[it];
      int c = item >> 1, side = item & 1;
      const double* nb = normal + (size_t)c * kNormalSize;
      if (e < 4) {
        v += nb[1 + 4 * side + e];
      } else {
        int k = (e - 4) / 4, l = (e - 4) % 4;
        v += H(nb, 4 * side + k, 4 * side + l);
      }
    }
    double* dst = e < 4 ? &fused[1 + 4 * (int64_t)node + e]
                        : &fused[1 + 4 * (int64_t)n_nodes + 16 * (int64_t)node + (e - 4)];
    *dst = accumulate ? *dst + v : v;
  } else if (tid < n_node_elems + n_off) {
    int64_t o = tid - n_node_elems;
    int c = (int)(o / 16), e = (int)(o % 16);
    const double* nb = normal + (size_t)c * kNormalSize;
    int gidx = global_index[c];
    double* dst = &fused[1 + 20 * (int64_t)n_nodes + 16 * (int64_t)gidx + e];
    double v = H(nb, e / 4, 4 + e % 4);
    *dst = accumulate ? *dst + v : v;
  }
}

__global__ void reg_scatter_normal_kernel(const double* __restrict__ normal, int n, const int32_t* __restrict__ global_index,
                                          double* __restrict__ all) {
  const int64_t tid = (int64_t)blockIdx.x * blockDim.x + threadIdx.x;
  if (tid >= (int64_t)n * kNormalSize) return;
  const int c = (int)(tid / kNormalSize), e = (int)(tid % kNormalSize);
  all[(size_t)global_index[c] * kNormalSize + e] = normal[tid];
}

template <typename OUT>
static void launch_points(vgx_ctx ctx, int vps, int layout, const ConstraintDev* d_desc, const PosePack* d_pack,
                          const Tile* d_tiles, unsigned char* d_tile_dead, int n_tiles, void* res, void* jr,
                          void* je, bool blocked = false) {
  if (n_tiles <= 0) return;
  hipLaunchKernelGGL(reg_points_tile_dead_kernel<kPointsPerThread>, dim3((n_tiles + 255) / 256), dim3(256), 0,
                     ctx->stream, d_desc, d_pack, d_tiles, n_tiles, d_tile_dead);
  dim3 grid(((n_tiles + 7) / 8) * 8), block(kBlockThreads);
  using O4 = typename Out4<OUT>::type;
  dispatch_brick(vps, layout, [&](auto V, auto L) {
    hipLaunchKernelGGL((reg_eval_points_kernel<V(), L(), OUT, kPointsPerThread>), grid, block, 0, ctx->stream, d_desc, d_pack, d_tiles,
                       d_tile_dead, n_tiles, (OUT*)res, (O4*)jr, (O4*)je, blocked ? 1 : 0);
  });
}

template <typename OUT>
static void launch_points_single(hipStream_t stream, int vps, const ConstraintDev& desc, const PosePack& pack,
                                 void* res, void* jr, void* je) {
  const int n_tiles = (int)((desc.n + kTilePoints - 1) / kTilePoints);
  if (n_tiles <= 0) return;
  dim3 grid(((n_tiles + 7) / 8) * 8), block(kBlockThreads);
  using O4 = typename Out4<OUT>::type;
  dispatch_brick(vps, desc.grid.layout, [&](auto V, auto L) {
    hipLaunchKernelGGL((reg_eval_points_single_kernel<V(), L(), OUT, kPointsPerThread>), grid, block, 0, stream, desc, pack, n_tiles,
                       (OUT*)res, (O4*)jr, (O4*)je);
  });
}

static void launch_visuals_single(hipStream_t stream, int vps, const ConstraintDev& desc, const PosePack& pack,
                                  const VisualsPose& mission, void* cloud, double* arrows, double* origins) {
  const int n_tiles = (int)((desc.n + kTilePoints - 1) / kTilePoints);
  if (n_tiles <= 0 || (!cloud && !arrows)) return;
  dim3 grid(n_tiles), block(kBlockThreads);
  dispatch_brick(vps, desc.grid.layout, [&](auto V, auto L) {
    if (arrows)
      hipLaunchKernelGGL((reg_visuals_single_kernel<V(), L(), kPointsPerThread, true>), grid, block, 0, stream, desc, pack, mission,
                         n_tiles, (f32x4*)cloud, arrows, origins);
    else
      hipLaunchKernelGGL((reg_visuals_single_kernel<V(), L(), kPointsPerThread, false>), grid, block, 0, stream, desc, pack, mission,
                         n_tiles, (f32x4*)cloud, arrows, origins);
  });
}

static VisualsPose make_visuals_pose(const double read_pose[4]) {
  const YawQuat q = yaw_exp((float)read_pose[3]);
  return {q.w, q.z, (float)read_pose[0], (float)read_pose[1], (float)read_pose[2]};
}

}

struct vgx_reg_visuals_s {
  vgx_ctx ctx = nullptr;
  std::mutex mu;
  int64_t n_residual_points = 0, n_jacobians = 0;
  double factor = 0;
  vgx::DeviceBuffer d_cloud;
  vgx::DeviceBuffer d_arrows;
  vgx::DeviceBuffer d_origins;
};

using namespace vgx;

vgx::ConstraintDev vgx_reg_s::describe() const {
  ConstraintDev c;
  std::memset(&c, 0, sizeof(c));
  c.grid = reading->grid_dev(cfg.use_esdf_distance ? 1 : 0);
  const PointSet& ps = reference->points[cfg.registration_point_type];
  c.xyzd = ps.d_xyzd;
  c.weight = ps.d_weight;
  if (cfg.sampling_ratio != -1.0f) {
    c.sample_raw = d_sample_raw.as<uint32_t>();
    c.cumulative = ps.d_cumulative;
    c.search_lut = ps.d_search_lut;
    c.search_buckets = ps.search_buckets;
    c.inv_order = ps.d_inv_order;
    c.n_points = ps.n;
  }
  c.chunk_bounds = ps.d_chunk_bounds;
  c.n = num_residuals;
  c.row0 = 0;
  c.prow0 = 0;
  if (cfg.sampling_ratio != -1.0f) {
    c.factor = 1.0;
  } else {
    c.factor = ps.sum_weight != 0 ? (double)num_residuals / ps.sum_weight : 0.0;
  }
  c.no_corr_cost = cfg.no_correspondence_cost;
  return c;
}

vgx::SamplerEngine& vgx_reg_s::engine() {
  return cfg.sampler_seed != 0u ? rng : reference->points[cfg.registration_point_type].rng;
}

bool vgx_reg_s::points_current() const {
  const PointSet& ps = reference->points[cfg.registration_point_type];
  return ps.present && ps.version == points_version;
}

int vgx_reg_s::draw_raw(uint32_t* out) {
  SamplerEngine& e = engine();
  int rc = engine_to_host(ctx, e);
  if (rc != VGX_OK) return rc;
  const int64_t m = 2 * num_residuals;
  for (int64_t k = 0; k < m; ++k) out[k] = e.host();
  return VGX_OK;
}

static void build_node_csr(int n, const int32_t* node_pair, int csr_nodes, std::vector<int32_t>& first,
                           std::vector<int32_t>& items) {
  first.assign((size_t)csr_nodes + 1, 0);
  items.assign(2 * (size_t)n, 0);
  for (int c = 0; c < n; ++c)
    for (int s = 0; s < 2; ++s) first[(size_t)node_pair[2 * c + s] + 1]++;
  for (int i = 0; i < csr_nodes; ++i) first[(size_t)i + 1] += first[(size_t)i];
  std::vector<int32_t> cur(first.begin(), first.end() - 1);
  for (int c = 0; c < n; ++c)
    for (int s = 0; s < 2; ++s) items[(size_t)cur[(size_t)node_pair[2 * c + s]]++] = (c << 1) | s;
}

extern "C" {

void vgx_reg_config_default(vgx_reg_config* cfg) {
  if (!cfg) return;
  cfg->registration_point_type = VGX_POINTS_ISOSURFACE;
  cfg->sampling_ratio = -1.0f;
  cfg->no_correspondence_cost = 0.0;
  cfg->use_esdf_distance = 1;
  cfg->sampler_seed = 0u;
}

int vgx_reg_create(vgx_ctx ctx, vgx_submap reference, vgx_submap reading, const vgx_reg_config* cfg,
                   vgx_reg* out) {
  if (!ctx || !out) return VGX_ERR_INVALID;
  *out = nullptr;
  std::lock_guard<std::mutex> lk(ctx->mu);
  if (!reference || !reading || !cfg)
    return set_error(ctx, VGX_ERR_INVALID, "vgx_reg_create: NULL submap or config");
  if (reference->ctx != ctx || reading->ctx != ctx)
    return set_error(ctx, VGX_ERR_INVALID, "vgx_reg_create: submaps belong to another context");
  if (cfg->registration_point_type != VGX_POINTS_ISOSURFACE &&
      cfg->registration_point_type != VGX_POINTS_VOXELS)
    return set_error(ctx, VGX_ERR_INVALID, "vgx_reg_create: bad registration_point_type");
  const PointSet& ps = reference->points[cfg->registration_point_type];
  if (!ps.present)
    return set_error(ctx, VGX_ERR_INVALID,
                     "vgx_reg_create: reference submap has no registration points of that type "
                     "(submap not finished)");
  const int which = cfg->use_esdf_distance ? 1 : 0;
  if (reading->n_blocks > 0 && !reading->grid[which].present)
    return set_error(ctx, VGX_ERR_INVALID,
                     which ? "vgx_reg_create: reading submap has no ESDF layer"
                           : "vgx_reg_create: reading submap has no TSDF layer");
  if (reference->vps != reading->vps)
    return set_error(ctx, VGX_ERR_UNSUPPORTED, "vgx_reg_create: submaps differ in voxels_per_side");
  vgx_reg r = new (std::nothrow) vgx_reg_s();
  if (!r) return set_error(ctx, VGX_ERR_NOMEM, "vgx_reg_create: out of host memory");
  r->ctx = ctx;
  r->reference = reference;
  r->reading = reading;
  r->cfg = *cfg;
  r->points_version = ps.version;
  if (cfg->sampling_ratio != -1.0f) {
    r->num_residuals = (int64_t)(int)(cfg->sampling_ratio * (float)ps.n);
    if (r->num_residuals < 0) r->num_residuals = 0;
  } else {
    r->num_residuals = ps.n;
  }
  if (cfg->sampler_seed != 0u) r->rng.host.seed(cfg->sampler_seed);
  if (cfg->sampling_ratio != -1.0f && (int64_t)ps.cumulative_weight.size() != ps.n) {
    PointSet& mps = reference->points[cfg->registration_point_type];
    std::vector<float> w((size_t)mps.n);
    if (mps.n > 0 && (hipStreamSynchronize(ctx->stream) != hipSuccess ||
                      hipMemcpy(w.data(), mps.d_weight, (size_t)mps.n * sizeof(float),
                                hipMemcpyDeviceToHost) != hipSuccess)) {
      delete r;
      return set_error(ctx, VGX_ERR_HIP, "vgx_reg_create: weight download failed");
    }
    mps.cumulative_weight.resize((size_t)mps.n);
    double acc = 0;
    for (int64_t i = 0; i < mps.n; ++i) {
      acc = (i == 0) ? (double)w[0] : acc + (double)w[(size_t)i];
      mps.cumulative_weight[(size_t)i] = acc;
    }
  }
  if (cfg->sampling_ratio != -1.0f && ps.n == 0) r->num_residuals = 0;
  if (cfg->sampling_ratio != -1.0f && ps.n > 0) {
    PointSet& mps = reference->points[cfg->registration_point_type];
    hipError_t e = hipSuccess;
    if (!mps.d_cumulative) {
      std::vector<double> padded(mps.cumulative_weight);
      padded.insert(padded.end(), 3, INFINITY);
      e = mps.d_cumulative.alloc_n(padded.size());
      if (e == hipSuccess)
        e = hipMemcpy(mps.d_cumulative, padded.data(), padded.size() * sizeof(double), hipMemcpyHostToDevice);
    }
    if (e == hipSuccess && !mps.d_search_lut) {
      int64_t K = kMinSearchBuckets;
      while (K < mps.n && K < kMaxSearchBuckets) K <<= 1;
      std::vector<int32_t> lut((size_t)K + 1);
      const std::vector<double>& cum = mps.cumulative_weight;
      const double total = cum.back();
      size_t pos = 0;
      for (int64_t k = 0; k <= K; ++k) {
        const double target = ((double)k / (double)K) * total;
        while (pos < cum.size() && !(target < cum[pos])) ++pos;
        lut[(size_t)k] = (int32_t)pos;
      }
      e = mps.d_search_lut.alloc_n(lut.size());
      if (e == hipSuccess)
        e = hipMemcpy(mps.d_search_lut, lut.data(), lut.size() * sizeof(int32_t), hipMemcpyHostToDevice);
      mps.search_buckets = (int32_t)K;
    }
    if (e == hipSuccess && !mps.inv_order.empty() && !mps.d_inv_order) {
      e = mps.d_inv_order.alloc_n((size_t)mps.n);
      if (e == hipSuccess)
        e = hipMemcpy(mps.d_inv_order, mps.inv_order.data(), (size_t)mps.n * sizeof(int32_t),
                      hipMemcpyHostToDevice);
    }
    if (e != hipSuccess) {
      delete r;
      return set_error(ctx, VGX_ERR_HIP, std::string("vgx_reg_create: sampler tables: ") + hipGetErrorString(e));
    }
  }
  {
    std::lock_guard<std::mutex> lt(lifetime_mu());
    ++reference->users;
    ++reading->users;
  }
  *out = r;
  return VGX_OK;
}

int vgx_reg_destroy(vgx_reg r) {
  if (!r) return VGX_ERR_INVALID;
  {
    std::lock_guard<std::mutex> lt(lifetime_mu());
    if (r->users > 0) {
      r->destroy_requested = true;
      return VGX_OK;
    }
  }
  (void)hipSetDevice(r->ctx->device);
  (void)hipStreamSynchronize(r->ctx->stream);
  vgx_submap orphan[2] = {nullptr, nullptr};
  {
    std::lock_guard<std::mutex> lt(lifetime_mu());
    vgx_submap both[2] = {r->reference, r->reading};
    for (int k = 0; k < 2; ++k) {
      vgx_submap sm = both[k];
      if (--sm->users == 0 && sm->destroy_requested) orphan[k] = sm;
    }
    if (orphan[0] == orphan[1]) orphan[1] = nullptr;
  }
  delete r;
  for (int k = 0; k < 2; ++k)
    if (orphan[k]) (void)vgx_submap_destroy(orphan[k]);
  return VGX_OK;
// ... 213 lines not shown
  const int64_t n = r->num_residuals;
  if (r->cfg.sampling_ratio != -1.0f && n > 0) {
    VGX_HIP(ctx, hipStreamSynchronize(ctx->stream));
    VGX_HIP(ctx, r->d_sample_raw.reserve((size_t)n * 2 * sizeof(uint32_t)));
    VGX_HIP(ctx, r->h_sample_raw.reserve((size_t)n * 2 * sizeof(uint32_t)));
    const int rc_draw = r->draw_raw(r->h_sample_raw.as<uint32_t>());
    if (rc_draw != VGX_OK) return rc_draw;
    VGX_HIP(ctx, hipMemcpyAsync(r->d_sample_raw.p, r->h_sample_raw.p, (size_t)n * 2 * sizeof(uint32_t),
                                hipMemcpyHostToDevice, ctx->stream));
  }
  if (reg_status(r) == VGX_EVALUATE_FALSE) return VGX_EVALUATE_FALSE;
  PosePack pack;
  make_pose_pack(ref_pose, read_pose, &pack);
  launch_points_single<float>(ctx->stream, r->reading->vps, r->describe(), pack, d_residuals, d_jac_ref,
                              d_jac_read);
  VGX_HIP(ctx, hipGetLastError());
  return VGX_OK;
}

int vgx_reg_batch_create(vgx_ctx ctx, int32_t n, const vgx_reg* regs, const int32_t* node_pair,
                         const int32_t* global_index, int32_t n_global, vgx_reg_batch* out) {
  if (!ctx || !out) return VGX_ERR_INVALID;
  *out = nullptr;
  std::lock_guard<std::mutex> lk(ctx->mu);
  if (n < 0 || (n > 0 && (!regs || !node_pair)))
    return set_error(ctx, VGX_ERR_INVALID, "vgx_reg_batch_create: bad n / NULL arrays");
  if (!global_index && n_global < n) n_global = n;
  if (n_global < n) return set_error(ctx, VGX_ERR_INVALID, "vgx_reg_batch_create: n_global < n");
  VGX_HIP(ctx, hipSetDevice(ctx->device));
  int vps = 0, layout = 0;
  for (int c = 0; c < n; ++c) {
    if (!regs[c] || regs[c]->ctx != ctx)
      return set_error(ctx, VGX_ERR_INVALID, "vgx_reg_batch_create: NULL or foreign constraint");
    if (!regs[c]->points_current())
      return set_error(ctx, VGX_ERR_INVALID,
                       "vgx_reg_batch_create: a reference submap's registration points were replaced after "
                       "its cost function was created");
    if (node_pair[2 * c] < 0 || node_pair[2 * c + 1] < 0)
      return set_error(ctx, VGX_ERR_INVALID, "vgx_reg_batch_create: negative node index");
    if (global_index && (global_index[c] < 0 || global_index[c] >= n_global))
      return set_error(ctx, VGX_ERR_INVALID, "vgx_reg_batch_create: global_index out of range");
    if (vps == 0) vps = regs[c]->reading->vps;
    if (regs[c]->reading->vps != vps)
      return set_error(ctx, VGX_ERR_UNSUPPORTED, "vgx_reg_batch_create: mixed voxels_per_side");
    const int lay = regs[c]->reading->grid[regs[c]->cfg.use_esdf_distance ? 1 : 0].layout;
    if (c == 0) layout = lay;
    if (lay != layout)
      return set_error(ctx, VGX_ERR_UNSUPPORTED,
                       "vgx_reg_batch_create: submaps with different brick layouts (vgx_ctx_set_brick_layout was "
                       "changed between their creation)");
  }
  bool quad_on_demand = n > 0 && layout == VGX_BRICKS_APRON && ctx->sampling_bricks == VGX_SAMPLING_BRICKS_QUAD;
  for (int c = 0; c < n && quad_on_demand; ++c) quad_on_demand = regs[c]->sampling();
  if (quad_on_demand) {
    VGX_HIP(ctx, hipSetDevice(ctx->device));
    std::vector<std::pair<vgx_submap, int>> made;
    for (int c = 0; c < n && quad_on_demand; ++c) {
      const int which = regs[c]->cfg.use_esdf_distance ? 1 : 0;
      const bool had = regs[c]->reading->grid[which].d_quad != nullptr;
      const int rc_q = regs[c]->reading->ensure_quad_grid(which);
      if (rc_q == VGX_OK) {
        if (!had && regs[c]->reading->grid[which].d_quad) made.emplace_back(regs[c]->reading, which);
        continue;
      }
      if (rc_q != VGX_ERR_NOMEM) return rc_q;
      VGX_HIP(ctx, hipStreamSynchronize(ctx->stream));
      for (auto& m : made) m.first->grid[m.second].d_quad.release();
      static bool told = false;
      if (!told) {
        told = true;
        fprintf(stderr, "libvoxgraph_amd: no memory for the quad bricks of a sampling batch (%s); it reads the apron bricks "
                        "instead -- same results, slower scattered evaluations\n", vgx_last_error(ctx));
      }
      set_error(ctx, VGX_OK, "no error");
      quad_on_demand = false;
    }
    if (quad_on_demand) layout = VGX_BRICKS_QUAD;
  }
  vgx_reg_batch b = new (std::nothrow) vgx_reg_batch_s();
  if (!b) return set_error(ctx, VGX_ERR_NOMEM, "vgx_reg_batch_create: out of host memory");
  vgx_reg_batch ex = b;
  b->ctx = ctx;
  b->n = n;
  b->n_global = n_global;
  b->layout = layout;
  b->regs.assign(regs, regs + n);
  b->node_pair.assign(node_pair, node_pair + 2 * (size_t)n);
  b->global_index.resize((size_t)n);
  for (int c = 0; c < n; ++c) b->global_index[(size_t)c] = global_index ? global_index[c] : c;
  b->row_offset.assign((size_t)n + 1, 0);
  std::vector<ConstraintDev> desc((size_t)n);
  std::vector<int32_t> tile_first((size_t)n + 1, 0), points_tile_first((size_t)n + 1, 0);
  auto reduce_iters_of = [](int64_t n_residuals) {
    return (int)std::min<int64_t>(kReduceIters, std::max<int64_t>(1, n_residuals / ((int64_t)kTilePoints * 5)));
  };
  int max_node = -1;
  for (int c = 0; c < n; ++c) {
    desc[(size_t)c] = regs[c]->describe();
    if (quad_on_demand) {
      const Grid& gq = regs[c]->reading->grid[regs[c]->cfg.use_esdf_distance ? 1 : 0];
      if (gq.d_bricks) {
        desc[(size_t)c].grid.bricks = gq.d_quad;
        desc[(size_t)c].grid.layout = VGX_BRICKS_QUAD;
      }
    }
    desc[(size_t)c].row0 = b->row_offset[(size_t)c];
    desc[(size_t)c].prow0 = (int64_t)b->tiles.size() * kTilePoints;
    b->row_offset[(size_t)c + 1] = b->row_offset[(size_t)c] + regs[c]->num_residuals;
    std::vector<Tile> t = make_tiles(c, regs[c]->num_residuals, kTilePoints);
    points_tile_first[(size_t)c] = (int32_t)b->tiles.size();
    b->tiles.insert(b->tiles.end(), t.begin(), t.end());
    tile_first[(size_t)c] = (int32_t)ex->reduce_tiles.size();
    desc[(size_t)c].tile_points = kTilePoints * reduce_iters_of(regs[c]->num_residuals);
    std::vector<Tile> rt = make_tiles(c, regs[c]->num_residuals, desc[(size_t)c].tile_points);
    ex->reduce_tiles.insert(ex->reduce_tiles.end(), rt.begin(), rt.end());
    max_node = std::max(max_node, std::max(node_pair[2 * c], node_pair[2 * c + 1]));
  }
  tile_first[(size_t)n] = (int32_t)ex->reduce_tiles.size();
  points_tile_first[(size_t)n] = (int32_t)b->tiles.size();
  ex->host_desc = desc;
  ex->host_tile_first = tile_first;
  {
    std::vector<int> job_of((size_t)n, -1);
    for (int c = 0; c < n; ++c) {
      if (!regs[c]->sampling() || regs[c]->num_residuals == 0) continue;
      SamplerEngine* e = &regs[c]->engine();
      int j = 0;
      while (j < (int)b->stream_jobs.size() && b->stream_jobs[(size_t)j].engine != e) ++j;
      if (j == (int)b->stream_jobs.size()) b->stream_jobs.push_back({e, 0, 0});
      job_of[(size_t)c] = j;
      b->stream_jobs[(size_t)j].count += 2 * regs[c]->num_residuals;
    }
    int64_t total = 0;
    for (auto& j : b->stream_jobs) {
      j.offset = total;
      total += j.count;
    }
    b->any_sampling = total > 0;
    if (b->any_sampling) {
      if (b->d_raw.alloc((size_t)total * sizeof(uint32_t)) != hipSuccess ||
          b->d_drawn.alloc((size_t)b->row_offset[(size_t)n] * sizeof(float4)) != hipSuccess ||
          b->d_drawn_idx.alloc((size_t)b->row_offset[(size_t)n] * sizeof(int32_t)) != hipSuccess) {
        vgx_reg_batch_destroy(b);
        return set_error(ctx, VGX_ERR_NOMEM, "vgx_reg_batch_create: sampler stream buffer allocation failed");
      }
      std::vector<int64_t> used(b->stream_jobs.size(), 0);
      for (int c = 0; c < n; ++c) {
        const int j = job_of[(size_t)c];
        if (j < 0) continue;
        desc[(size_t)c].sample_raw = b->d_raw.as<uint32_t>() + b->stream_jobs[(size_t)j].offset + used[(size_t)j];
        desc[(size_t)c].sample_pts = b->d_drawn.as<float4>();
        used[(size_t)j] += 2 * regs[c]->num_residuals;
      }
      std::vector<StreamJobDev> jd(b->stream_jobs.size());
      for (size_t j = 0; j < jd.size(); ++j) {
        SamplerEngine* e = b->stream_jobs[j].engine;
        if (!e->d_state && e->d_state.alloc(sizeof(Mt19937)) != hipSuccess) {
          vgx_reg_batch_destroy(b);
          return set_error(ctx, VGX_ERR_NOMEM, "vgx_reg_batch_create: sampler state allocation failed");
        }
        jd[j] = {e->d_state, b->d_raw.as<uint32_t>() + b->stream_jobs[j].offset, (long long)b->stream_jobs[j].count};
      }
      if (b->d_stream_jobs.alloc(jd.size() * sizeof(StreamJobDev)) != hipSuccess ||
          hipMemcpy(b->d_stream_jobs.p, jd.data(), jd.size() * sizeof(StreamJobDev), hipMemcpyHostToDevice) != hipSuccess) {
        vgx_reg_batch_destroy(b);
        return set_error(ctx, VGX_ERR_NOMEM, "vgx_reg_batch_create: sampler job table upload failed");
      }
    }
  }
  ex->host_desc = desc;
  ex->host_points_tile_first = points_tile_first;
  ex->csr_nodes = max_node + 1;
  std::vector<int32_t> first, items;
  build_node_csr(n, node_pair, ex->csr_nodes, first, items);
  int rc = upload_new(ctx, b->d_desc, desc.data(), desc.size() * sizeof(ConstraintDev));
  if (rc == VGX_OK) rc = upload_new(ctx, b->d_tiles, b->tiles.data(), b->tiles.size() * sizeof(Tile));
  if (rc == VGX_OK && !b->tiles.empty() && b->d_tile_dead.alloc(b->tiles.size()) != hipSuccess) rc = VGX_ERR_NOMEM;
  if (rc == VGX_OK && b->any_sampling) {
    const std::vector<Tile> dt = make_draw_order(desc, points_tile_first, b->tiles);
    b->n_draw_tiles = (int32_t)dt.size();
    rc = upload_new(ctx, b->d_draw_tiles, dt.data(), dt.size() * sizeof(Tile));
  }
  if (rc == VGX_OK) rc = upload_new(ctx, ex->d_reduce_tiles, ex->reduce_tiles.data(), ex->reduce_tiles.size() * sizeof(Tile));
  if (rc == VGX_OK) rc = upload_new(ctx, b->d_tile_first, tile_first.data(), tile_first.size() * sizeof(int32_t));
  if (rc == VGX_OK) rc = upload_new(ctx, b->d_node_pair, b->node_pair.data(), b->node_pair.size() * sizeof(int32_t));
  if (rc == VGX_OK) rc = upload_new(ctx, b->d_global_index, b->global_index.data(), b->global_index.size() * sizeof(int32_t));
  if (rc == VGX_OK) rc = upload_new(ctx, ex->d_node_first, first.data(), first.size() * sizeof(int32_t));
  if (rc == VGX_OK) rc = upload_new(ctx, ex->d_node_items, items.data(), items.size() * sizeof(int32_t));
  if (rc == VGX_OK && n > 0) {
    if (b->d_pack.alloc((size_t)n * sizeof(PosePack)) != hipSuccess ||
        b->pack_stage.reserve((size_t)n * sizeof(PosePack)) != hipSuccess ||
        b->d_partials.alloc(std::max<size_t>(1, ex->reduce_tiles.size()) * (kBlockThreads / 64) * kPartialSize * sizeof(double)) != hipSuccess ||
        b->d_normal.alloc((size_t)n * kNormalSize * sizeof(double)) != hipSuccess ||
        b->h_normal.alloc((size_t)n * kNormalSize * sizeof(double)) != hipSuccess)
      rc = set_error(ctx, VGX_ERR_NOMEM, "vgx_reg_batch_create: device allocation failed");
  }
  if (rc != VGX_OK) {
    vgx_reg_batch_destroy(b);
    return rc;
  }
  {
    std::lock_guard<std::mutex> lt(lifetime_mu());
    for (vgx_reg r : b->regs) ++r->users;
    b->holds_regs = true;
  }
  *out = b;
  return VGX_OK;
}

int vgx_reg_batch_destroy(vgx_reg_batch b) {
  if (!b) return VGX_ERR_INVALID;
  {
    std::lock_guard<std::mutex> lt(lifetime_mu());
    if (b->users > 0) {
      b->destroy_requested = true;
      return VGX_OK;
    }
  }
  (void)hipSetDevice(b->ctx->device);
  (void)hipStreamSynchronize(b->ctx->stream);
  std::vector<vgx_reg> orphans;
  if (b->holds_regs) {
    std::lock_guard<std::mutex> lt(lifetime_mu());
    for (vgx_reg r : b->regs)
      if (--r->users == 0 && r->destroy_requested) orphans.push_back(r);
  }
  for (vgx_reg r : orphans) (void)vgx_reg_destroy(r);
  delete b;
  return VGX_OK;
}

int64_t vgx_reg_batch_num_residuals(vgx_reg_batch b) { return b ? b->row_offset.back() : -1; }

int vgx_reg_batch_row_offsets(vgx_reg_batch b, int64_t* row_offset) {
  if (!b || !row_offset) return VGX_ERR_INVALID;
  std::copy(b->row_offset.begin(), b->row_offset.end(), row_offset);
  return VGX_OK;
}

static int batch_points_current(vgx_reg_batch b) {
  for (vgx_reg r : b->regs)
    if (!r->points_current())
      return set_error(b->ctx, VGX_ERR_INVALID,
                       "vgx_reg_batch: a reference submap's registration points were replaced after the "
                       "batch was created");
  return VGX_OK;
}

static int batch_begin(vgx_reg_batch b) {
  vgx_ctx ctx = b->ctx;
  int rc0 = batch_points_current(b);
  if (rc0 != VGX_OK) return rc0;
  if (!b->any_sampling) return VGX_OK;
  for (auto& j : b->stream_jobs) {
    int rc = engine_to_device(ctx, *j.engine);
    if (rc != VGX_OK) return rc;
  }
  hipLaunchKernelGGL(mt_generate_kernel, dim3((unsigned)b->stream_jobs.size()), dim3(kMtThreads), 0, ctx->stream,
                     b->d_stream_jobs.as<StreamJobDev>());
  VGX_HIP(ctx, hipGetLastError());
  const int per_xcd = 8 * kDrawWgsPerXcdDefault < b->n_draw_tiles ? kDrawWgsPerXcdDefault : (b->n_draw_tiles + 7) / 8;
  const dim3 grid((unsigned)(8 * per_xcd));
  hipLaunchKernelGGL(reg_draw_kernel, grid, dim3(256), 0, ctx->stream, b->d_desc.as<ConstraintDev>(),
                     b->d_draw_tiles.as<Tile>(), (int)b->n_draw_tiles, per_xcd, b->d_drawn_idx.as<int32_t>());
  VGX_HIP(ctx, hipGetLastError());
  hipLaunchKernelGGL(reg_gather_points_kernel, grid, dim3(256), 0, ctx->stream, b->d_desc.as<ConstraintDev>(),
                     b->d_draw_tiles.as<Tile>(), (int)b->n_draw_tiles, per_xcd, b->d_drawn_idx.as<int32_t>(),
                     b->d_drawn.as<float4>());
  VGX_HIP(ctx, hipGetLastError());
  return VGX_OK;
}

static int batch_upload_packs(vgx_reg_batch b, const double* poses, int32_t n_nodes, int32_t* status) {
  vgx_ctx ctx = b->ctx;
  if (b->n == 0) return VGX_OK;
  int turn = 0;
  hipError_t waited = hipSuccess;
  PosePack* stage = static_cast<PosePack*>(b->pack_stage.next(&turn, &waited));
  VGX_HIP(ctx, waited);
  for (int c = 0; c < b->n; ++c) {
    int i = b->node_pair[2 * (size_t)c], j = b->node_pair[2 * (size_t)c + 1];
    if (i >= n_nodes || j >= n_nodes)
      return set_error(ctx, VGX_ERR_INVALID, "vgx_reg_batch: node index >= n_nodes");
    make_pose_pack(poses + 4 * (size_t)i, poses + 4 * (size_t)j, &stage[c]);
    if (status) status[c] = reg_status(b->regs[(size_t)c]);
  }
  VGX_HIP(ctx, hipMemcpyAsync(b->d_pack.as<PosePack>(), stage, (size_t)b->n * sizeof(PosePack),
                              hipMemcpyHostToDevice, ctx->stream));
  VGX_HIP(ctx, b->pack_stage.record(turn, ctx->stream));
  return VGX_OK;
}

static int apply_launch_order(vgx_reg_batch b, const std::vector<Tile>& tiles, Tile* d_tiles,
                              const std::vector<int32_t>& tile_first, bool points_pass) {
  vgx_ctx ctx = b->ctx;
  bool& grouped = points_pass ? b->points_order_grouped : b->launch_order_grouped;
  const int n_tiles = (int)tiles.size();
  DeviceBuffer s_live;
  VGX_HIP(ctx, s_live.alloc((size_t)n_tiles * sizeof(int32_t)));
  hipLaunchKernelGGL(reg_tile_live_kernel, dim3(n_tiles), dim3(64), 0, ctx->stream, b->d_desc.as<ConstraintDev>(), b->d_pack.as<PosePack>(),
                     d_tiles, n_tiles, s_live.as<int32_t>());
  VGX_HIP(ctx, hipGetLastError());
  std::vector<int32_t> work((size_t)n_tiles);
  VGX_HIP(ctx, hipMemcpyAsync(work.data(), s_live.p, work.size() * sizeof(int32_t), hipMemcpyDeviceToHost, ctx->stream));
  VGX_HIP(ctx, hipStreamSynchronize(ctx->stream));
  std::vector<Tile> ordered = tiles;
  grouped = make_xcd_order(b->host_desc, tile_first, work, ordered, points_pass);
  VGX_HIP(ctx, hipMemcpy(d_tiles, ordered.data(), ordered.size() * sizeof(Tile), hipMemcpyHostToDevice));
  return VGX_OK;
}

static int batch_evaluation_begin(vgx_reg_batch b, const double* poses, int32_t n_nodes, int32_t* status) {
  const int rc = batch_begin(b);
  return rc != VGX_OK ? rc : batch_upload_packs(b, poses, n_nodes, status);
}

}

template <typename OUT>
static int batch_points_pass(vgx_reg_batch b, const double* poses, int32_t n_nodes, void* res, void* jr, void* je, bool blocked,
                             int32_t* status) {
  vgx_ctx ctx = b->ctx;
  int rc = batch_evaluation_begin(b, poses, n_nodes, status);
  if (rc != VGX_OK) return rc;
  if (b->n == 0) return VGX_OK;
  if (!b->points_order_made && !b->tiles.empty()) {
    rc = apply_launch_order(b, b->tiles, b->d_tiles.as<Tile>(), b->host_points_tile_first, true);
    if (rc != VGX_OK) return rc;
    b->points_order_made = true;
  }
  launch_points<OUT>(ctx, b->regs[0]->reading->vps, b->layout, b->d_desc.as<ConstraintDev>(), b->d_pack.as<PosePack>(),
                     b->d_tiles.as<Tile>(), b->d_tile_dead.as<unsigned char>(), (int)b->tiles.size(), res, jr, je, blocked);
  VGX_HIP(ctx, hipGetLastError());
  return VGX_OK;
}

extern "C" {

int vgx_reg_batch_evaluate_points(vgx_reg_batch b, const double* poses, int32_t n_nodes,
                                  void* d_residuals, void* d_jac_ref, void* d_jac_read,
                                  int32_t* status) {
  if (!b || !poses) return VGX_ERR_INVALID;
  vgx_ctx ctx = b->ctx;
  std::lock_guard<std::mutex> lk(ctx->mu);
  if (!d_residuals) return set_error(ctx, VGX_ERR_INVALID, "vgx_reg_batch_evaluate_points: residuals == NULL");
  VGX_HIP(ctx, hipSetDevice(ctx->device));
  return batch_points_pass<float>(b, poses, n_nodes, d_residuals, d_jac_ref, d_jac_read, false, status);
}

int vgx_reg_batch_evaluate_points_f64(vgx_reg_batch b, const double* poses, int32_t n_nodes, void* d_residuals,
                                      void* d_jac_ref, void* d_jac_read, int32_t* status) {
  if (!b || !poses) return VGX_ERR_INVALID;
  vgx_ctx ctx = b->ctx;
  std::lock_guard<std::mutex> lk(ctx->mu);
  if (!d_residuals) return set_error(ctx, VGX_ERR_INVALID, "vgx_reg_batch_evaluate_points_f64: residuals == NULL");
  if (((uintptr_t)d_jac_ref | (uintptr_t)d_jac_read) & 31u)
    return set_error(ctx, VGX_ERR_INVALID, "vgx_reg_batch_evaluate_points_f64: Jacobian arrays must be 32-byte aligned (one row)");
  VGX_HIP(ctx, hipSetDevice(ctx->device));
  return batch_points_pass<double>(b, poses, n_nodes, d_residuals, d_jac_ref, d_jac_read, false, status);
}

constexpr int64_t kRowsMirrorLimit = (int64_t)2 << 30;

int vgx_reg_batch_evaluate_rows_f64(vgx_reg_batch b, const double* poses, int32_t n_nodes, int32_t want_jac_ref,
                                    int32_t want_jac_read, int32_t* status) {
  if (!b || !poses) return VGX_ERR_INVALID;
  vgx_ctx ctx = b->ctx;
  const int64_t R = b->row_offset.back();
  std::lock_guard<std::mutex> lk(ctx->mu);
  VGX_HIP(ctx, hipSetDevice(ctx->device));
  const size_t bytes[3] = {(size_t)std::max<int64_t>(R, 1) * 8, (size_t)std::max<int64_t>(R, 1) * 32, (size_t)std::max<int64_t>(R, 1) * 32};
  const bool want[3] = {true, want_jac_ref != 0, want_jac_read != 0};
  for (int a = 0; a < 3; ++a)
    if (want[a] && !b->d_rows[a].p && b->d_rows[a].alloc(bytes[a]) != hipSuccess) {
      (void)hipGetLastError();
      return set_error(ctx, VGX_ERR_NOMEM, "vgx_reg_batch_evaluate_rows_f64: no device memory for the batch's own rows");
    }
  if (!b->h_rows.p && R > 0 && R * 72 <= kRowsMirrorLimit && b->h_rows.alloc((size_t)R * 72) != hipSuccess)
    (void)hipGetLastError();
  b->rows_mirrored = false;
  const int rc = batch_points_pass<double>(b, poses, n_nodes, b->d_rows[0].p, want[1] ? b->d_rows[1].p : nullptr,
                                           want[2] ? b->d_rows[2].p : nullptr, false, status);
  if (rc != VGX_OK) return rc;
  b->rows_have[0] = true;
  b->rows_have[1] = want[1];
  b->rows_have[2] = want[2];
  if (b->h_rows.p && R > 0) {
    VGX_HIP(ctx, hipMemcpyAsync(b->h_rows.p, b->d_rows[0].p, (size_t)R * 8, hipMemcpyDeviceToHost, ctx->stream));
    if (b->rows_have[1])
      VGX_HIP(ctx, hipMemcpyAsync(b->h_rows.as<char>() + (size_t)R * 8, b->d_rows[1].p, (size_t)R * 32, hipMemcpyDeviceToHost, ctx->stream));
    if (b->rows_have[2])
      VGX_HIP(ctx, hipMemcpyAsync(b->h_rows.as<char>() + (size_t)R * 40, b->d_rows[2].p, (size_t)R * 32, hipMemcpyDeviceToHost, ctx->stream));
    b->rows_mirrored = true;
  }
  return VGX_OK;
}

int vgx_reg_batch_fetch_rows_f64(vgx_reg_batch b, int32_t c, double* residuals, double* jac_ref, double* jac_read) {
  if (!b || c < 0 || c >= b->n) return VGX_ERR_INVALID;
  vgx_ctx ctx = b->ctx;
  std::lock_guard<std::mutex> lk(ctx->mu);
  if (!b->rows_have[0]) return set_error(ctx, VGX_ERR_INVALID, "vgx_reg_batch_fetch_rows_f64: no rows evaluation to fetch from");
  if ((jac_ref && !b->rows_have[1]) || (jac_read && !b->rows_have[2]))
    return set_error(ctx, VGX_ERR_INVALID, "vgx_reg_batch_fetch_rows_f64: the last rows evaluation was asked for no such Jacobian block");
  VGX_HIP(ctx, hipSetDevice(ctx->device));
  VGX_HIP(ctx, hipStreamSynchronize(ctx->stream));
  const int64_t R = b->row_offset.back(), r0 = b->row_offset[(size_t)c], n = b->row_offset[(size_t)c + 1] - r0;
  if (n <= 0) return VGX_OK;
  if (b->rows_mirrored) {
    if (residuals) std::memcpy(residuals, b->h_rows.as<char>() + (size_t)r0 * 8, (size_t)n * 8);
    if (jac_ref) std::memcpy(jac_ref, b->h_rows.as<char>() + (size_t)R * 8 + (size_t)r0 * 32, (size_t)n * 32);
    if (jac_read) std::memcpy(jac_read, b->h_rows.as<char>() + (size_t)R * 40 + (size_t)r0 * 32, (size_t)n * 32);
    return VGX_OK;
  }
  if (residuals) VGX_HIP(ctx, hipMemcpy(residuals, b->d_rows[0].as<double>() + r0, (size_t)n * 8, hipMemcpyDeviceToHost));
  if (jac_ref) VGX_HIP(ctx, hipMemcpy(jac_ref, b->d_rows[1].as<double>() + 4 * r0, (size_t)n * 32, hipMemcpyDeviceToHost));
  if (jac_read) VGX_HIP(ctx, hipMemcpy(jac_read, b->d_rows[2].as<double>() + 4 * r0, (size_t)n * 32, hipMemcpyDeviceToHost));
  return VGX_OK;
}

int vgx_reg_batch_blocked_layout(vgx_reg_batch b, int64_t* bytes, int32_t* rows_per_block, int64_t* first_block) {
  if (!b) return VGX_ERR_INVALID;
  if (bytes) *bytes = (int64_t)b->tiles.size() * kTilePoints * 36;
  if (rows_per_block) *rows_per_block = kTilePoints;
  if (first_block) {
    int64_t blk = 0;
    for (int c = 0; c < b->n; ++c) {
      first_block[c] = blk;
      blk += (b->regs[(size_t)c]->num_residuals + kTilePoints - 1) / kTilePoints;
    }
    first_block[b->n] = blk;
  }
  return VGX_OK;
}

int vgx_reg_batch_evaluate_points_blocked(vgx_reg_batch b, const double* poses, int32_t n_nodes, void* d_blocks,
                                          int32_t* status) {
  if (!b || !poses) return VGX_ERR_INVALID;
  vgx_ctx ctx = b->ctx;
  std::lock_guard<std::mutex> lk(ctx->mu);
  if (!d_blocks) return set_error(ctx, VGX_ERR_INVALID, "vgx_reg_batch_evaluate_points_blocked: blocks == NULL");
  if (((uintptr_t)d_blocks & 15u) != 0)
    return set_error(ctx, VGX_ERR_INVALID, "vgx_reg_batch_evaluate_points_blocked: blocks must be 16-byte aligned");
  VGX_HIP(ctx, hipSetDevice(ctx->device));
  return batch_points_pass<float>(b, poses, n_nodes, d_blocks, d_blocks, d_blocks, true, status);
}

int vgx_reg_batch_choose_outputs(vgx_reg_batch b, const double* poses, int32_t n_nodes, int32_t n_candidates,
                                 void* const* d_residuals, void* const* d_jac_ref, void* const* d_jac_read, int32_t launches,
                                 int32_t chosen[3], float* ms_chosen, float* ms_trials) {
  if (!b || !poses || !d_residuals || !chosen || n_candidates <= 0 || launches <= 0) return VGX_ERR_INVALID;
  vgx_ctx ctx = b->ctx;
  if (b->any_sampling)
    return set_error(ctx, VGX_ERR_INVALID, "vgx_reg_batch_choose_outputs: a sampling batch (its trial evaluations would advance the "
                                           "sampling engines); choose the arrays with an all-points batch of the same sizes");
  for (int k = 0; k < n_candidates; ++k)
    if (!d_residuals[k] || (d_jac_ref && !d_jac_ref[k]) || (d_jac_read && !d_jac_read[k]))
      return set_error(ctx, VGX_ERR_INVALID, "vgx_reg_batch_choose_outputs: a candidate is NULL");
  hipEvent_t e0 = nullptr, e1 = nullptr;
  {
    std::lock_guard<std::mutex> lk(ctx->mu);
    VGX_HIP(ctx, hipSetDevice(ctx->device));
    if (hipEventCreate(&e0) != hipSuccess || hipEventCreate(&e1) != hipSuccess) {
      if (e0) (void)hipEventDestroy(e0);
      return set_error(ctx, VGX_ERR_HIP, "vgx_reg_batch_choose_outputs: hipEventCreate failed");
    }
  }
  int n_trials = 0;
  auto trial = [&](int i, int j, int k, float* ms) -> int {
    void* jr = d_jac_ref ? d_jac_ref[j] : nullptr;
    void* je = d_jac_read ? d_jac_read[k] : nullptr;
    int rc = vgx_reg_batch_evaluate_points(b, poses, n_nodes, d_residuals[i], jr, je, nullptr);
    if (rc != VGX_OK) return rc;
    {
      std::lock_guard<std::mutex> lk(ctx->mu);
      VGX_HIP(ctx, hipEventRecord(e0, ctx->stream));
    }
    for (int l = 0; l < launches && rc == VGX_OK; ++l)
      rc = vgx_reg_batch_evaluate_points(b, poses, n_nodes, d_residuals[i], jr, je, nullptr);
    if (rc != VGX_OK) return rc;
    {
      std::lock_guard<std::mutex> lk(ctx->mu);
      VGX_HIP(ctx, hipEventRecord(e1, ctx->stream));
    }
    VGX_HIP(ctx, hipEventSynchronize(e1));
    float t = 0.0f;
    VGX_HIP(ctx, hipEventElapsedTime(&t, e0, e1));
    *ms = t / (float)launches;
    if (ms_trials) ms_trials[n_trials] = *ms;
    ++n_trials;
    return VGX_OK;
  };
  int rc = VGX_OK;
  float best = 0.0f;
  int pick[3] = {0, 0, 0};
  for (int s_ = 0; s_ < n_candidates && rc == VGX_OK; ++s_) {
    float t = 0.0f;
    rc = trial(s_, s_, s_, &t);
    if (rc == VGX_OK && (s_ == 0 || t < best)) {
      best = t;
      pick[0] = pick[1] = pick[2] = s_;
    }
  }
  for (int which = 2; which >= 0 && rc == VGX_OK && n_candidates > 1; --which) {
    if ((which == 1 && !d_jac_ref) || (which == 2 && !d_jac_read)) continue;
    const int set_pick = pick[which];
    for (int c = 0; c < n_candidates && rc == VGX_OK; ++c) {
      if (c == set_pick) {
        if (ms_trials) ms_trials[n_trials] = -1.0f;
        ++n_trials;
        continue;
      }
      int q[3] = {pick[0], pick[1], pick[2]};
      q[which] = c;
      float t = 0.0f;
      rc = trial(q[0], q[1], q[2], &t);
      if (rc == VGX_OK && t < 0.995f * best) {
        best = t;
        pick[which] = c;
      }
    }
  }
  {
    std::lock_guard<std::mutex> lk(ctx->mu);
    (void)hipEventDestroy(e0);
    (void)hipEventDestroy(e1);
  }
  if (rc != VGX_OK) return rc;
  chosen[0] = pick[0];
  chosen[1] = pick[1];
  chosen[2] = pick[2];
  if (ms_chosen) *ms_chosen = best;
  return VGX_OK;
}

int vgx_reg_batch_alloc_outputs(vgx_reg_batch b, const double* poses, int32_t n_nodes, int32_t n_candidates, int32_t want_jac_ref,
                                int32_t want_jac_read, void** d_residuals, void** d_jac_ref, void** d_jac_read, float* ms_chosen) {
  if (!b || !poses || !d_residuals || n_candidates <= 0 || n_candidates > 16 || (want_jac_ref && !d_jac_ref) ||
      (want_jac_read && !d_jac_read))
    return VGX_ERR_INVALID;
  vgx_ctx ctx = b->ctx;
  *d_residuals = nullptr;
  if (d_jac_ref) *d_jac_ref = nullptr;
  if (d_jac_read) *d_jac_read = nullptr;
  const size_t rows = (size_t)std::max<int64_t>(b->row_offset.back(), 1);
  DeviceBuffer cand[3][16];
  void* cand_p[3][16] = {};
  const size_t bytes[3] = {rows * 4, rows * 16, rows * 16};
  const bool want[3] = {true, want_jac_ref != 0, want_jac_read != 0};
  int have = 0, rc = VGX_OK;
  {
    std::lock_guard<std::mutex> lk(ctx->mu);
    VGX_HIP(ctx, hipSetDevice(ctx->device));
    for (; have < n_candidates; ++have) {
      bool ok = true;
      for (int a = 0; a < 3 && ok; ++a)
        if (want[a]) ok = cand[a][have].alloc(bytes[a]) == hipSuccess;
      if (!ok) {
        (void)hipGetLastError();
        for (int a = 0; a < 3; ++a) cand[a][have].release();
        break;
      }
      for (int a = 0; a < 3; ++a) cand_p[a][have] = cand[a][have].p;
    }
  }
  if (have == 0) return set_error(ctx, VGX_ERR_NOMEM, "vgx_reg_batch_alloc_outputs: no memory for one set of row arrays");
  int32_t chosen[3] = {0, 0, 0};
  if (have > 1 && !b->any_sampling && b->row_offset.back() > 0)
    rc = vgx_reg_batch_choose_outputs(b, poses, n_nodes, have, cand_p[0], want[1] ? cand_p[1] : nullptr, want[2] ? cand_p[2] : nullptr, 3,
                                      chosen, ms_chosen, nullptr);
  else if (ms_chosen)
    *ms_chosen = 0.0f;
  {
    std::lock_guard<std::mutex> lk(ctx->mu);
    (void)hipSetDevice(ctx->device);
    (void)hipStreamSynchronize(ctx->stream);
    if (rc == VGX_OK) {
      *d_residuals = cand[0][chosen[0]].detach();
      if (want[1]) *d_jac_ref = cand[1][chosen[1]].detach();
      if (want[2]) *d_jac_read = cand[2][chosen[2]].detach();
    }
    for (int a = 0; a < 3; ++a)
      for (int k = 0; k < have; ++k) cand[a][k].release();
  }
  return rc;
}

int vgx_reg_batch_free_outputs(vgx_reg_batch b, void* d_residuals, void* d_jac_ref, void* d_jac_read) {
  if (!b) return VGX_ERR_INVALID;
  vgx_ctx ctx = b->ctx;
  std::lock_guard<std::mutex> lk(ctx->mu);
  (void)hipSetDevice(ctx->device);
  (void)hipStreamSynchronize(ctx->stream);
  for (void* p : {d_residuals, d_jac_ref, d_jac_read})
    if (p) (void)hipFree(p);
  return VGX_OK;
}

}

template <bool COST_ONLY>
static int launch_fused_tiles(vgx_reg_batch b) {
  vgx_ctx ctx = b->ctx;
  const int n_tiles = (int)b->reduce_tiles.size();
  if (!b->launch_order_made && n_tiles > 0) {
    int rc = apply_launch_order(b, b->reduce_tiles, b->d_reduce_tiles.as<Tile>(), b->host_tile_first, false);
    if (rc != VGX_OK) return rc;
    b->launch_order_made = true;
  }
  const unsigned occupancy_pad = ctx->tsdf_integrators.load() > 0 ? 27u * 1024u : 0u;
  if (n_tiles > 0) {
    dim3 grid(n_tiles), block(kBlockThreads);
    dispatch_brick(b->regs[0]->reading->vps, b->layout, [&](auto V, auto L) {
      hipLaunchKernelGGL((reg_eval_reduce_lean_kernel<V(), L(), COST_ONLY>), grid, block, occupancy_pad, ctx->stream,
                         b->d_desc.as<ConstraintDev>(), b->d_pack.as<PosePack>(), b->d_reduce_tiles.as<Tile>(), n_tiles,
                         b->d_tile_first.as<int32_t>(), b->d_partials.as<double>());
    });
    VGX_HIP(ctx, hipGetLastError());
  }
  return VGX_OK;
}

extern "C" {

int vgx_reg_batch_evaluate_normal(vgx_reg_batch b, const double* poses, int32_t n_nodes,
                                  void* d_normal, double* normal_host, int32_t* status) {
  if (!b || !poses) return VGX_ERR_INVALID;
  vgx_ctx ctx = b->ctx;
  std::lock_guard<std::mutex> lk(ctx->mu);
  VGX_HIP(ctx, hipSetDevice(ctx->device));
  int rc = batch_evaluation_begin(b, poses, n_nodes, status);
  if (rc != VGX_OK) return rc;
  if (b->n == 0) return VGX_OK;
  double* out = d_normal ? (double*)d_normal : b->d_normal.as<double>();
  rc = launch_fused_tiles<false>(b);
  if (rc != VGX_OK) return rc;
  hipLaunchKernelGGL(reg_finalize_kernel, dim3(b->n), dim3(256), 0, ctx->stream, b->d_desc.as<ConstraintDev>(), b->d_pack.as<PosePack>(),
                     b->d_tile_first.as<int32_t>(), b->d_partials.as<double>(), out);
  VGX_HIP(ctx, hipGetLastError());
  if (normal_host) {
    const size_t bytes = (size_t)b->n * kNormalSize * sizeof(double);
    VGX_HIP(ctx, hipMemcpyAsync(b->h_normal.as<double>(), out, bytes, hipMemcpyDeviceToHost, ctx->stream));
    VGX_HIP(ctx, hipStreamSynchronize(ctx->stream));
    std::memcpy(normal_host, b->h_normal.as<double>(), bytes);
  }
  return VGX_OK;
}

int vgx_reg_batch_evaluate_cost(vgx_reg_batch b, const double* poses, int32_t n_nodes, void* d_cost, double* cost_host,
                                int32_t* status) {
  if (!b || !poses) return VGX_ERR_INVALID;
  vgx_ctx ctx = b->ctx;
  std::lock_guard<std::mutex> lk(ctx->mu);
  VGX_HIP(ctx, hipSetDevice(ctx->device));
  int rc = batch_evaluation_begin(b, poses, n_nodes, status);
  if (rc != VGX_OK) return rc;
  if (b->n == 0) return VGX_OK;
  double* out = d_cost ? (double*)d_cost : b->d_normal.as<double>();
  rc = launch_fused_tiles<true>(b);
  if (rc != VGX_OK) return rc;
  hipLaunchKernelGGL(reg_finalize_cost_kernel, dim3((unsigned)((b->n + 3) / 4)), dim3(64), 0, ctx->stream, b->d_desc.as<ConstraintDev>(), (int)b->n,
                     b->d_tile_first.as<int32_t>(), b->d_partials.as<double>(), out);
  VGX_HIP(ctx, hipGetLastError());
  if (cost_host) {
    VGX_HIP(ctx, hipMemcpyAsync(b->h_normal.as<double>(), out, (size_t)b->n * sizeof(double), hipMemcpyDeviceToHost, ctx->stream));
    VGX_HIP(ctx, hipStreamSynchronize(ctx->stream));
    std::memcpy(cost_host, b->h_normal.as<double>(), (size_t)b->n * sizeof(double));
  }
  return VGX_OK;
}

int vgx_reg_batch_launch_order(vgx_reg_batch b, int32_t pass, int32_t* grouped) {
  if (!b || !grouped || (pass != 0 && pass != 1)) return VGX_ERR_INVALID;
  std::lock_guard<std::mutex> lk(b->ctx->mu);
  const bool made = pass ? b->points_order_made : b->launch_order_made;
  *grouped = !made ? -1 : (int32_t)(pass ? b->points_order_grouped : b->launch_order_grouped);
  return VGX_OK;
}

static int count_live_each(vgx_reg_batch b, std::vector<unsigned long long>& each) {
  vgx_ctx ctx = b->ctx;
  each.assign((size_t)b->n, 0);
  DeviceBuffer counter;
  VGX_HIP(ctx, counter.alloc((size_t)b->n * sizeof(unsigned long long)));
  VGX_HIP(ctx, hipMemsetAsync(counter.p, 0, (size_t)b->n * sizeof(unsigned long long), ctx->stream));
  hipLaunchKernelGGL(reg_count_live_kernel, dim3(b->n), dim3(256), 0, ctx->stream, b->d_desc.as<ConstraintDev>(), b->d_pack.as<PosePack>(), b->n,
                     counter.as<unsigned long long>());
  VGX_HIP(ctx, hipGetLastError());
  VGX_HIP(ctx, hipMemcpyAsync(each.data(), counter.p, each.size() * sizeof(unsigned long long), hipMemcpyDeviceToHost, ctx->stream));
  VGX_HIP(ctx, hipStreamSynchronize(ctx->stream));
  return VGX_OK;
}

int vgx_reg_batch_count_live_each(vgx_reg_batch b, const double* poses, int32_t n_nodes, int64_t* live_each) {
  if (!b || !poses || (b->n > 0 && !live_each)) return VGX_ERR_INVALID;
  vgx_ctx ctx = b->ctx;
  std::lock_guard<std::mutex> lk(ctx->mu);
  VGX_HIP(ctx, hipSetDevice(ctx->device));
  int rc = batch_points_current(b);
  if (rc == VGX_OK) rc = batch_upload_packs(b, poses, n_nodes, nullptr);
  if (rc != VGX_OK || b->n == 0) return rc;
  std::vector<unsigned long long> each;
  rc = count_live_each(b, each);
  if (rc != VGX_OK) return rc;
  for (int c = 0; c < b->n; ++c) live_each[c] = (int64_t)each[(size_t)c];
  return VGX_OK;
}

int vgx_reg_batch_count_live(vgx_reg_batch b, const double* poses, int32_t n_nodes, int64_t* live_residuals,
                             int64_t* unique_points) {
  if (!b || !poses || !live_residuals) return VGX_ERR_INVALID;
  vgx_ctx ctx = b->ctx;
  std::lock_guard<std::mutex> lk(ctx->mu);
  *live_residuals = 0;
  if (unique_points) *unique_points = 0;
  VGX_HIP(ctx, hipSetDevice(ctx->device));
  int rc = batch_points_current(b);
  if (rc == VGX_OK) rc = batch_upload_packs(b, poses, n_nodes, nullptr);
  if (rc != VGX_OK) return rc;
  if (b->n == 0) return VGX_OK;
  std::vector<unsigned long long> each;
  rc = count_live_each(b, each);
  if (rc != VGX_OK) return rc;
  unsigned long long v = 0;
  for (unsigned long long e : each) v += e;
  *live_residuals = (int64_t)v;
  if (!unique_points) return VGX_OK;
  std::vector<std::pair<const float4*, std::vector<float4>>> bounds;
  std::vector<std::pair<const float4*, std::vector<unsigned char>>> loaded;
  int64_t unique = 0;
  for (int c = 0; c < b->n; ++c) {
    const ConstraintDev& C = b->host_desc[(size_t)c];
    const int64_t n_chunks = (C.n + kChunkPoints - 1) / kChunkPoints;
    if (C.sample_raw) {
      unique += C.n;
      continue;
    }
    size_t k = 0;
    while (k < bounds.size() && bounds[k].first != C.xyzd) ++k;
    if (k == bounds.size()) {
      bounds.emplace_back(C.xyzd, std::vector<float4>((size_t)n_chunks));
      loaded.emplace_back(C.xyzd, std::vector<unsigned char>((size_t)n_chunks, 0));
      if (n_chunks > 0 && C.chunk_bounds)
        VGX_HIP(ctx, hipMemcpy(bounds[k].second.data(), C.chunk_bounds, (size_t)n_chunks * sizeof(float4), hipMemcpyDeviceToHost));
    }
    const bool cull = C.no_corr_cost == 0.0 && C.chunk_bounds;
    PosePack P;
    make_pose_pack(poses + 4 * (size_t)b->node_pair[2 * (size_t)c], poses + 4 * (size_t)b->node_pair[2 * (size_t)c + 1], &P);
    for (int64_t q = 0; q < n_chunks; ++q)
      if (!cull || !chunk_outside(C.grid, P, bounds[k].second[(size_t)q])) loaded[k].second[(size_t)q] = 1;
  }
  for (size_t k = 0; k < loaded.size(); ++k) {
    int64_t n_pts = 0;
    for (int c = 0; c < b->n; ++c)
      if (b->host_desc[(size_t)c].xyzd == loaded[k].first && !b->host_desc[(size_t)c].sample_raw)
        n_pts = std::max<int64_t>(n_pts, b->host_desc[(size_t)c].n);
    const int64_t n_chunks = (int64_t)loaded[k].second.size();
    for (int64_t q = 0; q < n_chunks; ++q)
      if (loaded[k].second[(size_t)q]) unique += (q + 1) * kChunkPoints <= n_pts ? kChunkPoints : n_pts - q * kChunkPoints;
  }
  *unique_points = unique;
  return VGX_OK;
}

int64_t vgx_reg_fused_size(int32_t n_nodes, int32_t n_global) {
  if (n_nodes < 0 || n_global < 0) return -1;
  return 1 + 20 * (int64_t)n_nodes + 16 * (int64_t)n_global;
}

int vgx_reg_batch_assemble(vgx_reg_batch b, const void* d_normal, int32_t n_nodes, void* d_fused,
                           int32_t zero_first) {
  if (!b || !d_fused) return VGX_ERR_INVALID;
  vgx_ctx ctx = b->ctx;
  std::lock_guard<std::mutex> lk(ctx->mu);
  vgx_reg_batch ex = b;
  if (n_nodes < ex->csr_nodes)
    return set_error(ctx, VGX_ERR_INVALID, "vgx_reg_batch_assemble: n_nodes smaller than the largest node index");
  VGX_HIP(ctx, hipSetDevice(ctx->device));
  const double* nb = d_normal ? (const double*)d_normal : b->d_normal.as<double>();
  if (zero_first)
    VGX_HIP(ctx, hipMemsetAsync(d_fused, 0, (size_t)vgx_reg_fused_size(n_nodes, b->n_global) * sizeof(double), ctx->stream));
  int64_t work = (int64_t)ex->csr_nodes * 20 + (int64_t)b->n * 16;
  if (work == 0) work = 1;
  int threads = 256;
  int blocks = (int)((work + threads - 1) / threads) + 1;
  hipLaunchKernelGGL(reg_assemble_kernel, dim3(blocks), dim3(threads), 0, ctx->stream, nb, b->n,
                     ex->csr_nodes, n_nodes, b->d_node_pair.as<int32_t>(), b->d_global_index.as<int32_t>(),
                     ex->d_node_first.as<int32_t>(), ex->d_node_items.as<int32_t>(),
                     (double*)d_fused, zero_first ? 0 : 1);
  VGX_HIP(ctx, hipGetLastError());
  return VGX_OK;
}

int32_t vgx_reg_batch_brick_layout(vgx_reg_batch b) { return b ? (int32_t)b->layout : -1; }

int vgx_reg_batch_scatter_normal(vgx_reg_batch b, const void* d_normal, void* d_normal_all, int32_t zero_first) {
  if (!b || !d_normal_all) return VGX_ERR_INVALID;
  vgx_ctx ctx = b->ctx;
  std::lock_guard<std::mutex> lk(ctx->mu);
  VGX_HIP(ctx, hipSetDevice(ctx->device));
  if (zero_first)
    VGX_HIP(ctx, hipMemsetAsync(d_normal_all, 0, (size_t)b->n_global * kNormalSize * sizeof(double), ctx->stream));
  if (b->n == 0) return VGX_OK;
  const double* nb = d_normal ? (const double*)d_normal : b->d_normal.as<double>();
  const int64_t work = (int64_t)b->n * kNormalSize;
  hipLaunchKernelGGL(reg_scatter_normal_kernel, dim3((unsigned)((work + 255) / 256)), dim3(256), 0, ctx->stream, nb, b->n,
                     b->d_global_index.as<int32_t>(), (double*)d_normal_all);
  VGX_HIP(ctx, hipGetLastError());
  return VGX_OK;
}

}

struct vgx_reg_assembler_s {
  vgx_ctx ctx = nullptr;
  int32_t n = 0, csr_nodes = 0;
  DeviceBuffer d_node_pair, d_identity, d_node_first, d_node_items;
};

extern "C" {

int vgx_reg_assembler_destroy(vgx_reg_assembler a) {
  if (!a) return VGX_ERR_INVALID;
  (void)hipSetDevice(a->ctx->device);
  (void)hipStreamSynchronize(a->ctx->stream);
  delete a;
  return VGX_OK;
}

int vgx_reg_assembler_create(vgx_ctx ctx, int32_t n, const int32_t* node_pair, vgx_reg_assembler* out) {
  if (!ctx || !out || n < 0 || (n > 0 && !node_pair)) return VGX_ERR_INVALID;
  *out = nullptr;
  int max_node = -1;
  for (int c = 0; c < 2 * n; ++c) {
    if (node_pair[c] < 0) return set_error(ctx, VGX_ERR_INVALID, "vgx_reg_assembler_create: negative node index");
    max_node = std::max(max_node, node_pair[c]);
  }
  std::lock_guard<std::mutex> lk(ctx->mu);
  VGX_HIP(ctx, hipSetDevice(ctx->device));
// ... 41 lines not shown
```

Measured before the change: 129,500.

## Prefetch next evaluation's random sampling on a side stream with double buffers

Adds a second sampling stream and double-buffered raw/drawn/descriptor buffers so the Mersenne Twister generation, draw and gather for the next evaluation are queued ahead while the current evaluation runs. On the next call, if the engine generation counters match, a small commit kernel copies the advanced RNG state instead of regenerating on the critical path; otherwise it falls back to inline sampling. Generation counters track host-side engine changes, and extra stream synchronisations are added wherever point sets are rebuilt. This costs extra device memory and speculative work that is discarded when poses or engines change between evaluations.

```diff
diff --git a/profiles/sampling_prefetch_bench.py b/profiles/sampling_prefetch_bench.py
--- /dev/null
+++ b/profiles/sampling_prefetch_bench.py
@@ -0,0 +1,74 @@
+import argparse
+import json
+import os
+import statistics
+import sys
+import time
+
+import numpy as np
+
+HERE_ROOT = os.path.dirname(os.path.dirname(os.path.abspath(__file__)))
+
+
+def main():
+    ap = argparse.ArgumentParser()
+    ap.add_argument("--root", default=HERE_ROOT, help="the tree whose library and bench.py scene are used")
+    ap.add_argument("--evals", type=int, default=40)
+    ap.add_argument("--loop", type=int, default=0)
+    ap.add_argument("--pauses-ms", type=float, nargs="*", default=[0.0, 0.3, 0.7, 2.0])
+    args = ap.parse_args()
+    sys.path.insert(0, os.path.abspath(args.root))
+    import bench
+    from voxgraph_amd import capi
+    scene = argparse.Namespace(grid=[20, 10], block_dims=[16, 16, 16], block_min=[-8, -8, -4], voxel_size=0.2, truncation=0.6,
+                               esdf_max=2.0, pose_sigma=0.3, yaw_sigma=0.05, seed=2)
+    true_poses, poses, pairs = bench.build_graph(scene)
+    ctx = capi.Context(0)
+    submaps = []
+    for k in range(len(true_poses)):
+        sm = capi.Submap.synth_city(ctx, k, scene.voxel_size, 16, scene.block_min, scene.block_dims, scene.truncation,
+                                    scene.esdf_max, 10.0, true_poses[k], scene.seed)
+        sm.extract_isosurface_points(1.0)
+        sm.release_raw_layers()
+        submaps.append(sm)
+    cfg = capi.default_config(registration_point_type=capi.POINTS_ISOSURFACE, sampling_ratio=0.05)
+    pairs_s = [(int(a), int(b)) for p in pairs for a, b in (p, p[::-1])]
+    cfs = [capi.RegistrationCostFunction(ctx, submaps[a], submaps[b], cfg) for a, b in pairs_s]
+    batch = capi.RegistrationBatch(ctx, cfs, pairs_s)
+    for _ in range(3):
+        batch.evaluate_normal(poses, to_host=False)
+    ctx.synchronize()
+    out = {"constraints": len(pairs_s), "residuals_per_evaluation": int(batch.num_residuals())}
+    if args.loop:
+        for _ in range(args.loop):
+            batch.evaluate_normal(poses, to_host=False)
+        ctx.synchronize()
+        out["evaluations"] = args.loop + 3
+    else:
+        out["evals_per_pause"] = args.evals
+        out["pauses"] = []
+        for pause_ms in args.pauses_ms:
+            stream_ms, wall_ms = [], []
+            for _ in range(args.evals):
+                t0 = time.perf_counter()
+                ctx.timer_start()
+                batch.evaluate_normal(poses, to_host=False)
+                stream_ms.append(ctx.timer_stop())
+                wall_ms.append((time.perf_counter() - t0) * 1e3)
+                t1 = time.perf_counter()
+                while (time.perf_counter() - t1) * 1e3 < pause_ms:
+                    pass
+            q = statistics.quantiles(stream_ms, n=10)
+            out["pauses"].append({"host_pause_ms": pause_ms, "stream_ms_per_evaluate_normal_median": round(statistics.median(stream_ms), 4),
+                                  "stream_ms_p10": round(q[0], 4), "stream_ms_p90": round(q[-1], 4),
+                                  "wall_ms_per_evaluate_normal_median": round(statistics.median(wall_ms), 4)})
+    status, normal = batch.evaluate_normal(poses)
+    out["cost_sum_after"] = float(normal[:, 0].sum())
+    print(json.dumps(out))
+    for o in [batch] + cfs + submaps:
+        o.destroy()
+    ctx.close()
+
+
+if __name__ == "__main__":
+    main()
diff --git a/profiles/sampling_prefetch_summary.py b/profiles/sampling_prefetch_summary.py
--- /dev/null
+++ b/profiles/sampling_prefetch_summary.py
@@ -0,0 +1,76 @@
+import csv
+import glob
+import json
+import os
+import sys
+
+SHORT = (("mt_generate", "mt_generate"), ("mt_commit", "mt_commit"), ("reg_draw", "reg_draw"), ("reg_gather_points", "reg_gather"),
+         ("reg_eval_reduce_lean", "fused_tiles"), ("reg_finalize", "finalize"), ("reg_assemble", "assemble"))
+
+
+def bench_runs(out, who):
+    rows = []
+    for f in sorted(glob.glob(os.path.join(out, who + "_*.json"))):
+        d = json.load(open(f))
+        s = d["shipped_config"]
+        rows.append({"run": os.path.basename(f), "shipped_ms_per_evaluation": round(s["ms_per_evaluation"], 4),
+                     "shipped_stream_ms": round(s["stream_ms_per_evaluation"], 4), "shipped_cost": repr(s["cost"]),
+                     "apron_ms": round(s["apron_bricks"]["ms_per_evaluation"], 4) if s.get("apron_bricks") else None,
+                     "apron_cost_equals_default": (s.get("apron_bricks") or {}).get("cost_equals_default"),
+                     "headline_value": round(d["value"], 1), "fused_ms_per_step": round(d["fused"]["ms_per_step"], 4)})
+    return rows
+
+
+def trim(out, who, evaluations=3):
+    files = glob.glob(os.path.join(out, "trace_" + who, "**", "*kernel_trace.csv"), recursive=True)
+    if not files:
+        return None
+    rows = []
+    for r in csv.DictReader(open(files[0])):
+        name = next((s for k, s in SHORT if k in r["Kernel_Name"]), None)
+        if name:
+            rows.append((int(r["Start_Timestamp"]), int(r["End_Timestamp"]), name, r.get("Queue_Id", ""), r.get("Stream_Id", "")))
+    rows.sort()
+    fused = [i for i, r in enumerate(rows) if r[2] == "fused_tiles"]
+    if len(fused) < evaluations + 1:
+        return None
+    first = fused[-evaluations - 1] + 1
+    while first < len(rows) and rows[first][2] in ("finalize", "assemble"):
+        first += 1
+    keep = rows[first:]
+    t0 = keep[0][0]
+    path = os.path.join(out, "trace_%s.trim.csv" % who)
+    with open(path, "w") as f:
+        f.write("kernel,queue,stream,start_us,end_us,duration_us\n")
+        for s, e, name, q, st in keep:
+            f.write("%s,%s,%s,%.1f,%.1f,%.1f\n" % (name, q, st, (s - t0) / 1e3, (e - t0) / 1e3, (e - s) / 1e3))
+    fk = [(s, e) for s, e, name, _, _ in keep if name == "fused_tiles"]
+    samp = [(s, e) for s, e, name, _, _ in keep if name in ("mt_generate", "reg_draw", "reg_gather")]
+    inside = sum(max(0, min(e, fe) - max(s, fs)) for s, e in samp for fs, fe in fk)
+    total = sum(e - s for s, e in samp)
+    return {"file": os.path.basename(path), "sampling_kernel_us": round(total / 1e3, 1),
+            "of_which_inside_a_fused_kernel_us": round(inside / 1e3, 1),
+            "fused_kernel_us": [round((e - s) / 1e3, 1) for s, e in fk],
+            "period_us": round((fk[-1][0] - fk[0][0]) / 1e3 / (len(fk) - 1), 1)}
+
+
+def main():
+    out = sys.argv[1]
+    for who in ("parent", "new"):
+        print("== bench.py shipped block alone, %s" % who)
+        for r in bench_runs(out, who):
+            print(json.dumps(r))
+    for who in ("parent", "new"):
+        p = os.path.join(out, "pause_%s.json" % who)
+        if os.path.exists(p):
+            print("== sampling_prefetch_bench.py, %s" % who)
+            d = json.loads(open(p).read().strip().splitlines()[-1])
+            for q in d.pop("pauses", []):
+                print(json.dumps(q))
+            print(json.dumps(d))
+    for who in ("parent", "new"):
+        print("== kernel trace of the back-to-back loop, %s: %s" % (who, json.dumps(trim(out, who))))
+
+
+if __name__ == "__main__":
+    main()
diff --git a/voxgraph_amd/csrc/vgx_context.hip b/voxgraph_amd/csrc/vgx_context.hip
--- a/voxgraph_amd/csrc/vgx_context.hip
+++ b/voxgraph_amd/csrc/vgx_context.hip
@@ -205,6 +205,7 @@
   VGX_HIP(ctx, hipStreamSynchronize(ctx->stream));
   VGX_HIP(ctx, hipMemcpy(&e.host, e.d_state, sizeof(Mt19937), hipMemcpyDeviceToHost));
   e.on_device = false;
+  ++e.generation;
   return VGX_OK;
 }
 
@@ -213,6 +214,7 @@
   if (!e.d_state) VGX_HIP(ctx, e.d_state.alloc(sizeof(Mt19937)));
   VGX_HIP(ctx, hipMemcpyAsync(e.d_state, &e.host, sizeof(Mt19937), hipMemcpyHostToDevice, ctx->stream));
   e.on_device = true;
+  ++e.generation;
   return VGX_OK;
 }
 }
@@ -297,6 +299,7 @@
   ctx->stream_priorities = use_prio && prio_least != prio_greatest;
   if (hipSetDevice(device) != hipSuccess ||
       hipStreamCreateWithPriority(&ctx->own_stream, hipStreamNonBlocking, ctx->stream_priorities ? prio_least : 0) != hipSuccess ||
+      hipStreamCreateWithPriority(&ctx->sample_stream, hipStreamNonBlocking, ctx->stream_priorities ? prio_least : 0) != hipSuccess ||
       hipStreamCreateWithPriority(&ctx->tsdf_own_stream, hipStreamNonBlocking, ctx->stream_priorities ? prio_greatest : 0) != hipSuccess ||
       hipEventCreate(&ctx->ev_start) != hipSuccess ||
       hipEventCreate(&ctx->ev_stop) != hipSuccess ||
@@ -304,6 +307,7 @@
       hipEventCreate(&ctx->ev_tsdf_stop) != hipSuccess ||
       hipEventCreateWithFlags(&ctx->ev_handover, hipEventDisableTiming) != hipSuccess) {
     if (ctx->own_stream) (void)hipStreamDestroy(ctx->own_stream);
+    if (ctx->sample_stream) (void)hipStreamDestroy(ctx->sample_stream);
     if (ctx->tsdf_own_stream) (void)hipStreamDestroy(ctx->tsdf_own_stream);
     for (hipEvent_t ev : {ctx->ev_start, ctx->ev_stop, ctx->ev_tsdf_start, ctx->ev_tsdf_stop, ctx->ev_handover})
       if (ev) (void)hipEventDestroy(ev);
@@ -321,6 +325,7 @@
   if (!ctx) return VGX_ERR_INVALID;
   (void)hipSetDevice(ctx->device);
   (void)hipStreamSynchronize(ctx->stream);
+  (void)hipStreamSynchronize(ctx->sample_stream);
   (void)hipStreamSynchronize(ctx->tsdf_stream);
   for (hipEvent_t ev : {ctx->ev_start, ctx->ev_stop, ctx->ev_tsdf_start, ctx->ev_tsdf_stop, ctx->ev_handover})
     if (ev) (void)hipEventDestroy(ev);
@@ -337,6 +342,7 @@
     sl.h_out.release();
   }
   if (ctx->own_stream) (void)hipStreamDestroy(ctx->own_stream);
+  if (ctx->sample_stream) (void)hipStreamDestroy(ctx->sample_stream);
   if (ctx->tsdf_own_stream) (void)hipStreamDestroy(ctx->tsdf_own_stream);
   delete ctx;
   return VGX_OK;
@@ -357,6 +363,8 @@
 int vgx_ctx_set_stream(vgx_ctx ctx, void* hip_stream) {
   if (!ctx) return VGX_ERR_INVALID;
   std::lock_guard<std::mutex> lk(ctx->mu);
+  (void)hipSetDevice(ctx->device);
+  (void)hipStreamSynchronize(ctx->sample_stream);
   ctx->stream = hip_stream ? (hipStream_t)hip_stream : ctx->own_stream;
   return VGX_OK;
 }
@@ -395,6 +403,7 @@
 int vgx_ctx_synchronize(vgx_ctx ctx) {
   if (!ctx) return VGX_ERR_INVALID;
   VGX_HIP(ctx, hipStreamSynchronize(ctx->stream));
+  VGX_HIP(ctx, hipStreamSynchronize(ctx->sample_stream));
   VGX_HIP(ctx, hipStreamSynchronize(ctx->tsdf_stream));
   return VGX_OK;
 }
@@ -629,6 +638,7 @@
   VGX_HIP(ctx, hipSetDevice(ctx->device));
   PointSet& ps = sm->points[point_type];
   (void)hipStreamSynchronize(ctx->stream);
+  (void)hipStreamSynchronize(ctx->sample_stream);
   reset_point_set(ps);
   ps.n = n;
   ps.cumulative_weight.resize((size_t)n);
diff --git a/voxgraph_amd/csrc/vgx_extract.hip b/voxgraph_amd/csrc/vgx_extract.hip
--- a/voxgraph_amd/csrc/vgx_extract.hip
+++ b/voxgraph_amd/csrc/vgx_extract.hip
@@ -111,6 +111,7 @@
   VGX_HIP(ctx, hipSetDevice(ctx->device));
   PointSet& ps = sm->points[VGX_POINTS_VOXELS];
   VGX_HIP(ctx, hipStreamSynchronize(ctx->stream));
+  VGX_HIP(ctx, hipStreamSynchronize(ctx->sample_stream));
   reset_point_set(ps);
   const int nb = sm->n_blocks;
   if (nb == 0) {
diff --git a/voxgraph_amd/csrc/vgx_internal.h b/voxgraph_amd/csrc/vgx_internal.h
--- a/voxgraph_amd/csrc/vgx_internal.h
+++ b/voxgraph_amd/csrc/vgx_internal.h
@@ -16,6 +16,7 @@
 #include <vector>
 
 #include "voxgraph_amd.h"
+#include "vgx_sampling_prefetch.h"
 
 namespace vgx {
 
@@ -257,6 +258,7 @@
   int device = 0;
   hipStream_t own_stream = nullptr;
   hipStream_t stream = nullptr;
+  hipStream_t sample_stream = nullptr;
   hipEvent_t ev_start = nullptr, ev_stop = nullptr;
   std::mutex mu;
   hipStream_t tsdf_own_stream = nullptr;
@@ -318,6 +320,7 @@
   Mt19937 host;
   DeviceArray<uint32_t> d_state;
   bool on_device = false;
+  uint64_t generation = 0;
 };
 
 struct PointSet {
@@ -442,6 +445,18 @@
   vgx::DeviceBuffer d_raw;
   vgx::DeviceBuffer d_stream_jobs;
   bool any_sampling = false;
+  bool draw_ahead = false;
+  vgx::DeviceBuffer d_raw_b, d_drawn_b, d_drawn_idx_b;
+  vgx::DeviceBuffer d_desc_b;
+  vgx::DeviceBuffer d_ahead_state;
+  hipEvent_t ev_order = nullptr;
+  hipEvent_t ev_ahead = nullptr;
+  vgx::PrefetchedBlock ahead;
+  bool ahead_begun = false;
+  int set = 0;
+  const vgx::ConstraintDev* desc_dev() const {
+    return (set ? d_desc_b : d_desc).as<vgx::ConstraintDev>();
+  }
   bool holds_regs = false;
   vgx::DeviceBuffer d_rows[3];
   vgx::PinnedBuffer h_rows;
diff --git a/voxgraph_amd/csrc/vgx_iso.hip b/voxgraph_amd/csrc/vgx_iso.hip
--- a/voxgraph_amd/csrc/vgx_iso.hip
+++ b/voxgraph_amd/csrc/vgx_iso.hip
@@ -300,6 +300,7 @@
     return set_error(ctx, VGX_ERR_INVALID, "vgx_submap_extract_isosurface_points: TSDF layer not resident");
   VGX_HIP(ctx, hipSetDevice(ctx->device));
   VGX_HIP(ctx, hipStreamSynchronize(ctx->stream));
+  VGX_HIP(ctx, hipStreamSynchronize(ctx->sample_stream));
   PointSet& ps = sm->points[VGX_POINTS_ISOSURFACE];
   reset_point_set(ps);
   sm->isosurface_blocks.clear();
diff --git a/voxgraph_amd/csrc/vgx_reg.hip b/voxgraph_amd/csrc/vgx_reg.hip
--- a/voxgraph_amd/csrc/vgx_reg.hip
+++ b/voxgraph_amd/csrc/vgx_reg.hip
@@ -885,7 +885,8 @@
 }
 
 struct StreamJobDev {
-  uint32_t* state;
+  const uint32_t* state_in;
+  uint32_t* state_out;
   uint32_t* out;
   long long count;
 };
@@ -916,7 +917,8 @@
   static_assert(kMtThreads == H, "one thread per word of a range");
   const StreamJobDev job = jobs[blockIdx.x];
   VGX_GLOBAL uint32_t* const g_out = (VGX_GLOBAL uint32_t*)job.out;
-  VGX_GLOBAL uint32_t* const g_state = (VGX_GLOBAL uint32_t*)job.state;
+  const VGX_GLOBAL uint32_t* const g_state = (const VGX_GLOBAL uint32_t*)job.state_in;
+  VGX_GLOBAL uint32_t* const g_state_out = (VGX_GLOBAL uint32_t*)job.state_out;
   __shared__ uint32_t buf[2][kStride];
   const int t = threadIdx.x;
   for (int k = t; k < N; k += kMtThreads) buf[0][k] = g_state[k];
@@ -976,8 +978,15 @@
     produced += take;
   }
   __syncthreads();
-  for (int k = t; k < N; k += kMtThreads) g_state[k] = buf[cur][k];
-  if (t == 0) g_state[N] = (uint32_t)idx;
+  for (int k = t; k < N; k += kMtThreads) g_state_out[k] = buf[cur][k];
+  if (t == 0) g_state_out[N] = (uint32_t)idx;
+}
+
+__global__ __launch_bounds__(kMtThreads) void mt_commit_kernel(const StreamJobDev* __restrict__ jobs) {
+  const StreamJobDev job = jobs[blockIdx.x];
+  const VGX_GLOBAL uint32_t* const from = (const VGX_GLOBAL uint32_t*)job.state_out;
+  VGX_GLOBAL uint32_t* const to = (VGX_GLOBAL uint32_t*)const_cast<uint32_t*>(job.state_in);
+  for (int k = threadIdx.x; k <= Mt19937::kN; k += kMtThreads) to[k] = from[k];
 }
 
 __global__ __launch_bounds__(64) void reg_tile_live_kernel(const ConstraintDev* __restrict__ cons,
@@ -1419,6 +1428,7 @@
   if (rc != VGX_OK) return rc;
   const int64_t m = 2 * num_residuals;
   for (int64_t k = 0; k < m; ++k) out[k] = e.host();
+  ++e.generation;
   return VGX_OK;
 }
 
@@ -1938,19 +1948,12 @@
         desc[(size_t)c].sample_pts = b->d_drawn.as<float4>();
         used[(size_t)j] += 2 * regs[c]->num_residuals;
       }
-      std::vector<StreamJobDev> jd(b->stream_jobs.size());
-      for (size_t j = 0; j < jd.size(); ++j) {
-        SamplerEngine* e = b->stream_jobs[j].engine;
+      for (auto& j : b->stream_jobs) {
+        SamplerEngine* e = j.engine;
         if (!e->d_state && e->d_state.alloc(sizeof(Mt19937)) != hipSuccess) {
           vgx_reg_batch_destroy(b);
           return set_error(ctx, VGX_ERR_NOMEM, "vgx_reg_batch_create: sampler state allocation failed");
         }
-        jd[j] = {e->d_state, b->d_raw.as<uint32_t>() + b->stream_jobs[j].offset, (long long)b->stream_jobs[j].count};
-      }
-      if (b->d_stream_jobs.alloc(jd.size() * sizeof(StreamJobDev)) != hipSuccess ||
-          hipMemcpy(b->d_stream_jobs.p, jd.data(), jd.size() * sizeof(StreamJobDev), hipMemcpyHostToDevice) != hipSuccess) {
-        vgx_reg_batch_destroy(b);
-        return set_error(ctx, VGX_ERR_NOMEM, "vgx_reg_batch_create: sampler job table upload failed");
       }
     }
   }
@@ -1981,6 +1984,39 @@
         b->h_normal.alloc((size_t)n * kNormalSize * sizeof(double)) != hipSuccess)
       rc = set_error(ctx, VGX_ERR_NOMEM, "vgx_reg_batch_create: device allocation failed");
   }
+  if (rc == VGX_OK && b->any_sampling) {
+    const size_t J = b->stream_jobs.size();
+    b->draw_ahead = b->d_raw_b.alloc(b->d_raw.bytes) == hipSuccess && b->d_drawn_b.alloc(b->d_drawn.bytes) == hipSuccess &&
+                    b->d_drawn_idx_b.alloc(b->d_drawn_idx.bytes) == hipSuccess &&
+                    b->d_desc_b.alloc(desc.size() * sizeof(ConstraintDev)) == hipSuccess &&
+                    b->d_ahead_state.alloc(J * sizeof(Mt19937)) == hipSuccess &&
+                    hipEventCreateWithFlags(&b->ev_order, hipEventDisableTiming) == hipSuccess &&
+                    hipEventCreateWithFlags(&b->ev_ahead, hipEventDisableTiming) == hipSuccess;
+    if (!b->draw_ahead) {
+      (void)hipGetLastError();
+      for (DeviceBuffer* d : {&b->d_raw_b, &b->d_drawn_b, &b->d_drawn_idx_b, &b->d_desc_b, &b->d_ahead_state}) d->release();
+    }
+    std::vector<StreamJobDev> jd((b->draw_ahead ? 4 : 1) * J);
+    for (int ahead = 0; ahead < (b->draw_ahead ? 2 : 1); ++ahead)
+      for (int set = 0; set < (b->draw_ahead ? 2 : 1); ++set)
+        for (size_t j = 0; j < J; ++j) {
+          uint32_t* const state = b->stream_jobs[j].engine->d_state;
+          jd[((size_t)ahead * 2 + set) * J + j] = {state, ahead ? b->d_ahead_state.as<uint32_t>() + j * (Mt19937::kN + 1) : state,
+                                                  (set ? b->d_raw_b : b->d_raw).as<uint32_t>() + b->stream_jobs[j].offset,
+                                                  (long long)b->stream_jobs[j].count};
+        }
+    rc = upload_new(ctx, b->d_stream_jobs, jd.data(), jd.size() * sizeof(StreamJobDev));
+    if (rc == VGX_OK && b->draw_ahead) {
+      std::vector<ConstraintDev> desc_b = desc;
+      for (auto& C : desc_b) {
+        if (!C.sample_pts) continue;
+        C.sample_raw = b->d_raw_b.as<uint32_t>() + (C.sample_raw - b->d_raw.as<uint32_t>());
+        C.sample_pts = b->d_drawn_b.as<float4>();
+      }
+      if (hipMemcpy(b->d_desc_b.p, desc_b.data(), desc_b.size() * sizeof(ConstraintDev), hipMemcpyHostToDevice) != hipSuccess)
+        rc = set_error(ctx, VGX_ERR_HIP, "vgx_reg_batch_create: descriptor upload failed");
+    }
+  }
   if (rc != VGX_OK) {
     vgx_reg_batch_destroy(b);
     return rc;
@@ -2005,6 +2041,9 @@
   }
   (void)hipSetDevice(b->ctx->device);
   (void)hipStreamSynchronize(b->ctx->stream);
+  if (b->any_sampling) (void)hipStreamSynchronize(b->ctx->sample_stream);
+  for (hipEvent_t ev : {b->ev_order, b->ev_ahead})
+    if (ev) (void)hipEventDestroy(ev);
   std::vector<vgx_reg> orphans;
   if (b->holds_regs) {
     std::lock_guard<std::mutex> lt(lifetime_mu());
@@ -2033,27 +2072,79 @@
   return VGX_OK;
 }
 
+static int queue_generate(vgx_reg_batch b, hipStream_t stream, int ahead, int set) {
+  const size_t J = b->stream_jobs.size();
+  hipLaunchKernelGGL(mt_generate_kernel, dim3((unsigned)J), dim3(kMtThreads), 0, stream,
+                     b->d_stream_jobs.as<StreamJobDev>() + ((size_t)ahead * 2 + set) * J);
+  VGX_HIP(b->ctx, hipGetLastError());
+  return VGX_OK;
+}
+
+static int queue_draw_gather(vgx_reg_batch b, hipStream_t stream, int set) {
+  vgx_ctx ctx = b->ctx;
+  const ConstraintDev* desc = (set ? b->d_desc_b : b->d_desc).as<ConstraintDev>();
+  int32_t* drawn_idx = (set ? b->d_drawn_idx_b : b->d_drawn_idx).as<int32_t>();
+  const int per_xcd = 8 * kDrawWgsPerXcdDefault < b->n_draw_tiles ? kDrawWgsPerXcdDefault : (b->n_draw_tiles + 7) / 8;
+  const dim3 grid((unsigned)(8 * per_xcd));
+  hipLaunchKernelGGL(reg_draw_kernel, grid, dim3(256), 0, stream, desc, b->d_draw_tiles.as<Tile>(), (int)b->n_draw_tiles,
+                     per_xcd, drawn_idx);
+  VGX_HIP(ctx, hipGetLastError());
+  hipLaunchKernelGGL(reg_gather_points_kernel, grid, dim3(256), 0, stream, desc, b->d_draw_tiles.as<Tile>(),
+                     (int)b->n_draw_tiles, per_xcd, drawn_idx, (set ? b->d_drawn_b : b->d_drawn).as<float4>());
+  VGX_HIP(ctx, hipGetLastError());
+  return VGX_OK;
+}
+
 static int batch_begin(vgx_reg_batch b) {
   vgx_ctx ctx = b->ctx;
+  const PrefetchedBlock ahead = std::move(b->ahead);
+  b->ahead = PrefetchedBlock();
+  b->ahead_begun = false;
   int rc0 = batch_points_current(b);
   if (rc0 != VGX_OK) return rc0;
   if (!b->any_sampling) return VGX_OK;
-  for (auto& j : b->stream_jobs) {
-    int rc = engine_to_device(ctx, *j.engine);
+  const size_t J = b->stream_jobs.size();
+  std::vector<uint64_t> generation(J);
+  for (size_t j = 0; j < J; ++j) generation[j] = b->stream_jobs[j].engine->generation;
+  const BlockPlan plan = plan_evaluation(ahead, generation.data(), J, b->set);
+  b->set = plan.set;
+  if (plan.commit) {
+    VGX_HIP(ctx, hipStreamWaitEvent(ctx->stream, b->ev_ahead, 0));
+    hipLaunchKernelGGL(mt_commit_kernel, dim3((unsigned)J), dim3(kMtThreads), 0, ctx->stream,
+                       b->d_stream_jobs.as<StreamJobDev>() + (size_t)(2 + plan.set) * J);
+    VGX_HIP(ctx, hipGetLastError());
+  } else {
+    for (auto& j : b->stream_jobs) {
+      int rc = engine_to_device(ctx, *j.engine);
+      if (rc != VGX_OK) return rc;
+    }
+    int rc = queue_generate(b, ctx->stream, 0, plan.set);
+    if (rc == VGX_OK) rc = queue_draw_gather(b, ctx->stream, plan.set);
     if (rc != VGX_OK) return rc;
   }
-  hipLaunchKernelGGL(mt_generate_kernel, dim3((unsigned)b->stream_jobs.size()), dim3(kMtThreads), 0, ctx->stream,
-                     b->d_stream_jobs.as<StreamJobDev>());
-  VGX_HIP(ctx, hipGetLastError());
-  const int per_xcd = 8 * kDrawWgsPerXcdDefault < b->n_draw_tiles ? kDrawWgsPerXcdDefault : (b->n_draw_tiles + 7) / 8;
-  const dim3 grid((unsigned)(8 * per_xcd));
-  hipLaunchKernelGGL(reg_draw_kernel, grid, dim3(256), 0, ctx->stream, b->d_desc.as<ConstraintDev>(),
-                     b->d_draw_tiles.as<Tile>(), (int)b->n_draw_tiles, per_xcd, b->d_drawn_idx.as<int32_t>());
-  VGX_HIP(ctx, hipGetLastError());
-  hipLaunchKernelGGL(reg_gather_points_kernel, grid, dim3(256), 0, ctx->stream, b->d_desc.as<ConstraintDev>(),
-                     b->d_draw_tiles.as<Tile>(), (int)b->n_draw_tiles, per_xcd, b->d_drawn_idx.as<int32_t>(),
-                     b->d_drawn.as<float4>());
-  VGX_HIP(ctx, hipGetLastError());
+  for (auto& j : b->stream_jobs) ++j.engine->generation;
+  if (!b->draw_ahead) return VGX_OK;
+  VGX_HIP(ctx, hipEventRecord(b->ev_order, ctx->stream));
+  VGX_HIP(ctx, hipStreamWaitEvent(ctx->sample_stream, b->ev_order, 0));
+  int rc = queue_generate(b, ctx->sample_stream, 1, plan.set ^ 1);
+  if (rc != VGX_OK) return rc;
+  b->ahead_begun = true;
+  return VGX_OK;
+}
+
+static int batch_evaluation_end(vgx_reg_batch b) {
+  vgx_ctx ctx = b->ctx;
+  if (!b->ahead_begun) return VGX_OK;
+  b->ahead_begun = false;
+  VGX_HIP(ctx, hipEventRecord(b->ev_order, ctx->stream));
+  VGX_HIP(ctx, hipStreamWaitEvent(ctx->sample_stream, b->ev_order, 0));
+  int rc = queue_draw_gather(b, ctx->sample_stream, b->set ^ 1);
+  if (rc != VGX_OK) return rc;
+  VGX_HIP(ctx, hipEventRecord(b->ev_ahead, ctx->sample_stream));
+  const size_t J = b->stream_jobs.size();
+  std::vector<uint64_t> generation(J);
+  for (size_t j = 0; j < J; ++j) generation[j] = b->stream_jobs[j].engine->generation;
+  note_queued(b->ahead, b->set, generation.data(), J);
   return VGX_OK;
 }
 
@@ -2084,7 +2175,7 @@
   const int n_tiles = (int)tiles.size();
   DeviceBuffer s_live;
   VGX_HIP(ctx, s_live.alloc((size_t)n_tiles * sizeof(int32_t)));
-  hipLaunchKernelGGL(reg_tile_live_kernel, dim3(n_tiles), dim3(64), 0, ctx->stream, b->d_desc.as<ConstraintDev>(), b->d_pack.as<PosePack>(),
+  hipLaunchKernelGGL(reg_tile_live_kernel, dim3(n_tiles), dim3(64), 0, ctx->stream, b->desc_dev(), b->d_pack.as<PosePack>(),
                      d_tiles, n_tiles, s_live.as<int32_t>());
   VGX_HIP(ctx, hipGetLastError());
   std::vector<int32_t> work((size_t)n_tiles);
@@ -2097,8 +2188,10 @@
 }
 
 static int batch_evaluation_begin(vgx_reg_batch b, const double* poses, int32_t n_nodes, int32_t* status) {
+  const int rc_points = batch_points_current(b);
+  const int rc_packs = rc_points == VGX_OK ? batch_upload_packs(b, poses, n_nodes, status) : VGX_OK;
   const int rc = batch_begin(b);
-  return rc != VGX_OK ? rc : batch_upload_packs(b, poses, n_nodes, status);
+  return rc != VGX_OK ? rc : rc_packs;
 }
 
 }
@@ -2115,10 +2208,10 @@
     if (rc != VGX_OK) return rc;
     b->points_order_made = true;
   }
-  launch_points<OUT>(ctx, b->regs[0]->reading->vps, b->layout, b->d_desc.as<ConstraintDev>(), b->d_pack.as<PosePack>(),
+  launch_points<OUT>(ctx, b->regs[0]->reading->vps, b->layout, b->desc_dev(), b->d_pack.as<PosePack>(),
                      b->d_tiles.as<Tile>(), b->d_tile_dead.as<unsigned char>(), (int)b->tiles.size(), res, jr, je, blocked);
   VGX_HIP(ctx, hipGetLastError());
-  return VGX_OK;
+  return batch_evaluation_end(b);
 }
 
 extern "C" {
@@ -2399,7 +2492,7 @@
     dim3 grid(n_tiles), block(kBlockThreads);
     dispatch_brick(b->regs[0]->reading->vps, b->layout, [&](auto V, auto L) {
       hipLaunchKernelGGL((reg_eval_reduce_lean_kernel<V(), L(), COST_ONLY>), grid, block, occupancy_pad, ctx->stream,
-                         b->d_desc.as<ConstraintDev>(), b->d_pack.as<PosePack>(), b->d_reduce_tiles.as<Tile>(), n_tiles,
+                         b->desc_dev(), b->d_pack.as<PosePack>(), b->d_reduce_tiles.as<Tile>(), n_tiles,
                          b->d_tile_first.as<int32_t>(), b->d_partials.as<double>());
     });
     VGX_HIP(ctx, hipGetLastError());
@@ -2421,9 +2514,11 @@
   double* out = d_normal ? (double*)d_normal : b->d_normal.as<double>();
   rc = launch_fused_tiles<false>(b);
   if (rc != VGX_OK) return rc;
-  hipLaunchKernelGGL(reg_finalize_kernel, dim3(b->n), dim3(256), 0, ctx->stream, b->d_desc.as<ConstraintDev>(), b->d_pack.as<PosePack>(),
+  hipLaunchKernelGGL(reg_finalize_kernel, dim3(b->n), dim3(256), 0, ctx->stream, b->desc_dev(), b->d_pack.as<PosePack>(),
                      b->d_tile_first.as<int32_t>(), b->d_partials.as<double>(), out);
   VGX_HIP(ctx, hipGetLastError());
+  rc = batch_evaluation_end(b);
+  if (rc != VGX_OK) return rc;
   if (normal_host) {
     const size_t bytes = (size_t)b->n * kNormalSize * sizeof(double);
     VGX_HIP(ctx, hipMemcpyAsync(b->h_normal.as<double>(), out, bytes, hipMemcpyDeviceToHost, ctx->stream));
@@ -2445,9 +2540,11 @@
   double* out = d_cost ? (double*)d_cost : b->d_normal.as<double>();
   rc = launch_fused_tiles<true>(b);
   if (rc != VGX_OK) return rc;
-  hipLaunchKernelGGL(reg_finalize_cost_kernel, dim3((unsigned)((b->n + 3) / 4)), dim3(64), 0, ctx->stream, b->d_desc.as<ConstraintDev>(), (int)b->n,
+  hipLaunchKernelGGL(reg_finalize_cost_kernel, dim3((unsigned)((b->n + 3) / 4)), dim3(64), 0, ctx->stream, b->desc_dev(), (int)b->n,
                      b->d_tile_first.as<int32_t>(), b->d_partials.as<double>(), out);
   VGX_HIP(ctx, hipGetLastError());
+  rc = batch_evaluation_end(b);
+  if (rc != VGX_OK) return rc;
   if (cost_host) {
     VGX_HIP(ctx, hipMemcpyAsync(b->h_normal.as<double>(), out, (size_t)b->n * sizeof(double), hipMemcpyDeviceToHost, ctx->stream));
     VGX_HIP(ctx, hipStreamSynchronize(ctx->stream));
@@ -2470,7 +2567,7 @@
   DeviceBuffer counter;
   VGX_HIP(ctx, counter.alloc((size_t)b->n * sizeof(unsigned long long)));
   VGX_HIP(ctx, hipMemsetAsync(counter.p, 0, (size_t)b->n * sizeof(unsigned long long), ctx->stream));
-  hipLaunchKernelGGL(reg_count_live_kernel, dim3(b->n), dim3(256), 0, ctx->stream, b->d_desc.as<ConstraintDev>(), b->d_pack.as<PosePack>(), b->n,
+  hipLaunchKernelGGL(reg_count_live_kernel, dim3(b->n), dim3(256), 0, ctx->stream, b->desc_dev(), b->d_pack.as<PosePack>(), b->n,
                      counter.as<unsigned long long>());
   VGX_HIP(ctx, hipGetLastError());
   VGX_HIP(ctx, hipMemcpyAsync(each.data(), counter.p, each.size() * sizeof(unsigned long long), hipMemcpyDeviceToHost, ctx->stream));
diff --git a/voxgraph_amd/csrc/vgx_sampling_prefetch.h b/voxgraph_amd/csrc/vgx_sampling_prefetch.h
--- /dev/null
+++ b/voxgraph_amd/csrc/vgx_sampling_prefetch.h
@@ -0,0 +1,32 @@
+#pragma once
+#include <cstddef>
+#include <cstdint>
+#include <vector>
+
+namespace vgx {
+
+struct PrefetchedBlock {
+  bool queued = false;
+  int set = 0;
+  std::vector<uint64_t> generation;
+};
+
+struct BlockPlan {
+  bool commit;
+  int set;
+};
+
+inline BlockPlan plan_evaluation(const PrefetchedBlock& p, const uint64_t* generation_now, size_t n_jobs, int last_set) {
+  if (!p.queued) return {false, last_set};
+  bool same = p.generation.size() == n_jobs;
+  for (size_t j = 0; same && j < n_jobs; ++j) same = p.generation[j] == generation_now[j];
+  return same ? BlockPlan{true, p.set} : BlockPlan{false, p.set ^ 1};
+}
+
+inline void note_queued(PrefetchedBlock& p, int evaluation_set, const uint64_t* generation_now, size_t n_jobs) {
+  p.queued = true;
+  p.set = evaluation_set ^ 1;
+  p.generation.assign(generation_now, generation_now + n_jobs);
+}
+
+}
```

New measurement: 128,400. No clear change (-0.9%).
